# Pixie8888/R3DFSSeg

Hardware: AMD Instinct MI355X
Metric: episodes/sec S3DIS 2-way 5-shot 2048-pt (MPTI+attention, train step: forward+backward+grad all-reduce+Adam) (higher is better)
Workload: dtype f32 (index-free GEMMs -- self-attention, 1x1 convolutions, weight gradients, the EdgeConv backward's edge GEMMs -- as bf16x3 split products on the bf16 MFMA with fp32 accumulate; every index-deciding result: fp32)

## Files before the change

### include/r3d.h

```cpp
#ifndef R3D_H
#define R3D_H
#include <stdint.h>

#ifdef __cplusplus
extern "C" {
#endif

const char* r3d_last_error_string(void);
int r3d_abi_version(void);
int r3d_debug_poison_lds(unsigned pattern, unsigned* sink , void* stream);
int r3d_debug_set_cg_spmv_lds_min_blocks(int min_blocks);
int r3d_set_matrix_arith(int mode);
int r3d_get_matrix_arith(void);
int r3d_debug_set_gemm_bx3(int mask);

int r3d_cm_to_pm(const float* in , int B, int C, int N, float* out , long ld, void* stream);
int r3d_pm_to_cm(const float* in , long ld, int B, int C, int N, float* out , void* stream);
int r3d_pm_to_cm_pitched(const float* in, long ld, int B, int C, int N, float* out , long pitch, void* stream);
long r3d_cm_pitch(int N);
int r3d_copy_cols(const float* src, long ld_src, float* dst, long ld_dst, long M, int C, void* stream);

int r3d_sqnorm(const float* x, long ldx, long rows, int C, float* out, void* stream);
long r3d_knn_norm_ws_words(int B, int N);
int r3d_knn_topk(const float* x, long ldx, const float* x_cm, int B, int N, int C, int k, int mode,
                 const int32_t* n_valid_dev, float* norm_ws, float* cm_ws, int32_t* idx_out, float* score_out,
                 int32_t* status, void* stream);
long r3d_knn_ws_words(int B, int N, int C, int k, int flags);
int r3d_knn_topk_batched(const float* x, long ldx, const float* x_cm, int B, int N, int C, int k, int mode,
                         const int32_t* n_valid_dev, int n_valid_stride, float* ws, long ws_words, int32_t* idx_out,
                         float* score_out, int32_t* status, void* stream);
int r3d_debug_set_knn_bf16_threshold(int on);
int r3d_debug_set_knn_bf16_filter(int on);
int r3d_set_wpack_in_capture(int on);

int r3d_pointwise_conv(const float* X, long ldx, const float* W , long M, int K, int Co,
                       const float* scale, const float* shift, int act, float* Out, long ldo, void* stream);

int r3d_edgeconv_fwd(const float* PQ, const int32_t* idx, const float* W2, const float* s2, const float* t2,
                     float* out, long ldo, int B, int N, int K, int32_t* argmax_out, void* stream);

long r3d_attention_ws_words(int B, int N);
int r3d_attention_fwd(const float* qkv, long ld, int B, int N, float* out, long ldo, float* lse_out, float* ws,
                      void* stream);

int r3d_head_desc_words(void);
int r3d_head_max_k(void);
int r3d_fps_sample_count_table(int k, int n_max, int32_t* out, void* stream);
long r3d_head_proto_ws_words(int n_way, int k_shot, int N);
int r3d_head_proto_ws_offsets(int n_way, int k_shot, int N, long* out6 );
#define R3D_HEAD_FPS_ONE_LAUNCH 1
int r3d_head_prototypes(const int32_t* support_y , const int32_t* shot_keep ,
                        const float* feat , long ldf, const float* featT ,
                        const float* qfeat , long ldq, int n_way, int k_shot, int N, int D,
                        int n_query_pts, int k, float* nodes, long ldn, float* node_labels ,
                        int32_t* desc, int32_t* assign_out , int32_t* cluster_count ,
                        int32_t* ws, long ws_words, int flags, void* stream);

int r3d_head_prototypes_batched(int n_ep, int fps_group, const int32_t* support_y, long sy_stride, const int32_t* shot_keep,
                                long keep_stride, const float* feat, long ldf, long feat_ep_rows, const float* qfeat, long ldq,
                                long qfeat_ep_rows, int n_way, int k_shot, int N, int D, int n_query_pts, int k, float* nodes,
                                long ldn, long nodes_ep_rows, float* node_labels, int32_t* desc, long desc_stride,
                                int32_t* assign_out, long assign_stride, int32_t* cluster_count, long ccount_stride,
                                int32_t* ws, long ws_words, long ws_stride, int flags, void* stream);

long r3d_lp_ws_words(int n_cap, int kp1);
int r3d_lp_ws_offsets(int n_cap, int kp1, long* out6);
int r3d_label_propagate(const float* nodes, long ldn, int D, const int32_t* nbr, int kp1, const float* Y,
                        const int32_t* n_dev, const int32_t* n_proto_dev, int n_cap, float sigma, float alpha,
                        int max_iter, float tol, float* Z, int32_t* ws, long ws_words, int32_t* stats_out, void* stream);

int r3d_label_propagate_batched(int n_ep, const float* nodes, long ldn, int D, const int32_t* nbr, int kp1, const float* Y,
                                const int32_t* n_dev, const int32_t* n_proto_dev, long desc_stride, int n_cap, float sigma,
                                float alpha, int max_iter, float tol, float* Z, int32_t* ws, long ws_words, long ws_stride,
                                int32_t* stats_out, long stats_stride, void* stream);
long r3d_graph_weights_verify_words(int n_cap, int kp1);
int r3d_graph_weights_verify(int n_ep, const float* nodes, long ldn, int D, const int32_t* n_dev, long desc_stride, int n_cap,
                             int kp1, float sigma, int32_t* ws, long ws_words, long ws_stride, float* scratch,
                             int32_t* mismatch_out, void* stream);

int r3d_label_propagate_solve_batched(int n_ep, const float* Y, const int32_t* n_dev, long desc_stride, int n_cap, int kp1,
                                      float alpha, int max_iter, float tol, float* Z, int32_t* ws, long ws_words,
                                      long ws_stride, int32_t* stats_out, long stats_stride, void* stream);

int r3d_graph_set_lp_budget(void* graph, void* graph_exec, int budget, int* n_cg);

int r3d_query_logits_ce(const float* Z, const int32_t* n_proto_dev, int n_q, int N, int n_classes,
                        const int64_t* labels , float* logits ,
                        float* loss_out , int32_t* pred_out , void* stream);

int r3d_query_logits_ce_batched(int n_ep, const float* Z, long z_ep_rows, const int32_t* n_proto_dev, long desc_stride, int n_q,
                                int N, int n_classes, const int64_t* labels, float* logits, float* loss_out, int32_t* pred_out,
                                void* stream);

int r3d_pointwise_conv_acc(const float* X, long ldx, const float* W, long M, int K, int Co, const float* scale,
                           const float* shift, int act, float* Out, long ldo, void* stream);
long r3d_pointwise_conv_stats_ws_words(long M, int Co);
int r3d_pointwise_conv_stats(const float* X, long ldx, const float* W, long M, int K, int Co, float* Out, long ldo,
                             float* sums_out , float* ws, void* stream);
int r3d_pointwise_conv_stats2(const float* X, long ldx, const float* W, long M, int K, int Co, float* Out, long ldo,
                              long M_first, float* sums_a , float* sums_b , float* ws, void* stream);
int r3d_pointwise_conv_stats_seg(const float* X, long ldx, const float* W, long M, int K, int Co, float* Out, long ldo,
                                 long rows_a, long rows_b, float* sums_out, float* ws, void* stream);
int r3d_colreduce(const float* part , int chunks, int C, float* sums_out , void* stream);
int r3d_colreduce_seg(const float* part, int count_a, int count_b, int n_seg, int C, float* sums_out , void* stream);
long r3d_colstats_ws_words(long M, int C);
int r3d_colstats(const float* X, long ldx, const float* DY, long lddy, long M, int C, int mode, const float* scale,
                 const float* shift, const float* mean, const float* invstd, int act, float* sums_out ,
                 float* ws, void* stream);
int r3d_bn_fold(const float* sums, double count, int C, const float* gamma, const float* beta, float eps,
                float momentum, float* running_mean , float* running_var , float* mean, float* invstd,
                float* scale, float* shift, float* rec , const int32_t* rec_index_dev , long rec_stride,
                void* stream);
long r3d_colstats_seg_ws_words(long M, int C, long rows_a, long rows_b);
int r3d_colstats_seg(const float* X, long ldx, const float* DY, long lddy, long M, int C, long rows_a, long rows_b, int mode,
                     const float* scale, const float* shift, const float* mean, const float* invstd, long bn_stride, int act,
                     float* sums_out , float* ws, void* stream);
int r3d_bn_fold_seg(const float* sums , int n_seg, double count_a, double count_b, int C, const float* gamma,
                    const float* beta, float eps, float momentum, float* running_mean , float* running_var ,
                    float* mean, float* invstd, float* scale, float* shift, long bn_stride, float* rec ,
                    const int32_t* rec_index_dev , long rec_stride, void* stream);
int r3d_affine_act_seg(const float* Z, long ldz, long M, int C, long rows_a, long rows_b, const float* scale, const float* shift,
                       long bn_stride, int act, float* Y, long ldy, void* stream);
int r3d_bn_bwd_apply_seg(const float* Z, long ldz, const float* DY, long lddy, long M, int C, long rows_a, long rows_b,
                         const float* scale, const float* shift, const float* mean, const float* invstd, long bn_stride, int act,
                         const float* sums , double count_a, double count_b, float* DZ, long lddz, void* stream);
int r3d_bn_running_update(const float* rec, int n_records, long rec_stride, int C, float momentum,
                          const float* bias , float* running_mean,
                          float* running_var, void* stream);
int r3d_affine_act(const float* Z, long ldz, long M, int C, const float* scale, const float* shift, int act, float* Y,
                   long ldy, void* stream);
int r3d_bn_bwd_apply(const float* Z, long ldz, const float* DY, long lddy, long M, int C, const float* scale,
                     const float* shift, const float* mean, const float* invstd, int act, const float* sums,
                     double count, float* DZ, long lddz, void* stream);
long r3d_gemm_tn_ws_words(long M, int Ca, int Cb);
int r3d_gemm_tn(const float* A, long lda, const float* B, long ldb, long M, int Ca, int Cb, float alpha, float* out,
                int accumulate, float* ws, void* stream);
int r3d_add_cols(const float* src, long ld_src, float* dst, long ld_dst, long M, int C, void* stream);

long r3d_edgeconv_train_ws_words(int B, int N);
int r3d_edge_stats1(const float* PQ, const int32_t* idx, int B, int N, int K, int clouds_a, int clouds_b,
                    float* sums_out , float* esum , float* ws,
                    void* stream);
int r3d_edgeconv_train_fwd_minmax(const float* PQ, const int32_t* idx, const float* s1, const float* t1, long bn_stride,
                                  const float* W2, int B, int N, int K, int clouds_a, int clouds_b, float* zmax, float* zmin,
                                  int32_t* argmax, int32_t* argmin, float* sums_out , float* ws, void* stream);
int r3d_edge_select(float* zmax , const float* zmin, int32_t* argmax ,
                    const int32_t* argmin, const float* s2, const float* t2, long bn_stride, long M, long rows_a, long rows_b,
                    float* out, long ldo, void* stream);
long r3d_edge_reverse_ws_words(int B, int N, int K);
int r3d_edge_reverse(const int32_t* idx, int B, int N, int K, int32_t* rev_ws, long ws_words, void* stream);
int r3d_edgeconv_bwd(const float* PQ, const int32_t* idx, const float* s1, const float* t1, const float* mean1,
                     const float* invstd1, const float* W2, const float* s2, const float* t2, const float* mean2,
                     const float* invstd2, long bn_stride, const float* bn2_sums, const float* dout, long lddo,
                     const int32_t* argmax, const float* zwin , const float* esum , int B, int N, int K,
                     int clouds_a, int clouds_b, float* DY1 , float* BE ,
                     const int32_t* rev_ws , float* dW2, float* bn1_sums, float* dPQ,
                     float* ws, void* stream);

int r3d_attention_fwd_train(const float* qkv, long ld, int B, int N, float* out, long ldo, float* lse_out, float p_drop,
                            unsigned seed, const unsigned* seed_dev, float* ws , void* stream);
int r3d_attention_bwd(const float* qkv, long ld, int B, int N, const float* O, long ldo, const float* dO, long lddo,
                      const float* lse, float p_drop, unsigned seed, const unsigned* seed_dev, float q_scale, float* dqkv,
                      long ldd, float* ws , void* stream);
int r3d_attention_bwd_ws(const float* qkv, long ld, int B, int N, const float* O, long ldo, const float* dO, long lddo,
                         const float* lse, float p_drop, unsigned seed, const unsigned* seed_dev, float q_scale,
                         float* dqkv, long ldd, float* ws, int ws_holds_packed_qkv, void* stream);

long r3d_attention_ws_words_ep(int B, int N, int seed_group);
int r3d_attention_fwd_train_ep(const float* qkv, long ld, int B, int N, float* out, long ldo, float* lse_out, float p_drop,
                               unsigned seed, const unsigned* seed_dev, int seed_group, float* ws, void* stream);
int r3d_attention_bwd_ep(const float* qkv, long ld, int B, int N, const float* O, long ldo, const float* dO, long lddo,
                         const float* lse, float p_drop, unsigned seed, const unsigned* seed_dev, int seed_group, float q_scale,
                         float* dqkv, long ldd, float* ws, int ws_holds_packed_qkv, void* stream);

long r3d_attention_ws_words_ep_d(int B, int N, int seed_group, int D);
int r3d_attention_fwd_train_ep_d(const float* qkv, long ld, int B, int N, float* out, long ldo, float* lse_out, float p_drop,
                                 unsigned seed, const unsigned* seed_dev, int seed_group, int D, float* ws, void* stream);
int r3d_attention_bwd_ep_d(const float* qkv, long ld, int B, int N, const float* O, long ldo, const float* dO, long lddo,
                           const float* lse, float p_drop, unsigned seed, const unsigned* seed_dev, int seed_group, int D,
                           float q_scale, float* dqkv, long ldd, float* ws, int ws_holds_packed_qkv, void* stream);

int r3d_ce_grad(const float* Z, const int32_t* n_proto_dev, int n_cap, int n_query_pts, int n_classes,
                const int64_t* labels, const float* gscale_dev, float* G, void* stream);
int r3d_label_propagate_bwd(const float* nodes, long ldn, int D, int kp1, const float* Z, const float* G,
                            const int32_t* n_dev, int n_cap, float sigma, float alpha, int max_iter, float tol, float* lam,
                            float* dnodes, long ldd, int32_t* ws, long ws_words, int32_t* stats_out, void* stream);
int r3d_head_prototypes_bwd(const float* dnodes, long ldd, int n_way, int k_shot, int N, int D, int n_query_pts,
                            const int32_t* desc, const int32_t* assign, const int32_t* cluster_count, const int32_t* ws,
                            float* dsfeat, long lds_, float* dqfeat, long ldq, void* stream);

int r3d_ce_grad_batched(int n_ep, const float* Z, const int32_t* n_proto_dev, long desc_stride, int n_cap, int n_query_pts,
                        int n_classes, const int64_t* labels, const float* gscale_dev, float* G, void* stream);
int r3d_label_propagate_bwd_batched(int n_ep, const float* nodes, long ldn, int D, int kp1, const float* Z, const float* G,
                                    const int32_t* n_dev, long desc_stride, int n_cap, float sigma, float alpha, int max_iter,
                                    float tol, float* lam, float* dnodes, long ldd, int32_t* ws, long ws_words, long ws_stride,
                                    int32_t* stats_out, long stats_stride, void* stream);
int r3d_head_prototypes_bwd_batched(int n_ep, const float* dnodes, long ldd, long nodes_ep_rows, int n_way, int k_shot, int N,
                                    int D, int n_query_pts, const int32_t* desc, long desc_stride, const int32_t* assign,
                                    long assign_stride, const int32_t* cluster_count, long ccount_stride, const int32_t* ws,
                                    long ws_stride, float* dsfeat, long lds_, long dsfeat_ep_rows, float* dqfeat, long ldq,
                                    long dqfeat_ep_rows, void* stream);

long r3d_contrast_ws_words(int n_way, int k_shot, int N);
int r3d_contrast_fwd(const float* feat, long ldf, int D, const int32_t* support_y, const int32_t* support_flag, int n_way,
                     int k_shot, int N, const float* W, const float* bias, float temp, float* loss_out, float* ws,
                     long ws_words, void* stream);
int r3d_contrast_bwd(int D, int n_way, int k_shot, int N, const float* gscale_dev, float* dfeat, long ldd, float* dW,
                     float* db, float* ws, void* stream);
int r3d_contrast_fwd_batched(int n_ep, const float* feat, long ldf, long feat_ep_rows, int D, const int32_t* support_y,
                             const int32_t* support_flag, int n_way, int k_shot, int N, const float* W, const float* bias,
                             float temp, float* loss_out, float* ws, long ws_words, long ws_stride, void* stream);
int r3d_contrast_bwd_batched(int n_ep, int D, int n_way, int k_shot, int N, const float* gscale_dev, float* dfeat, long ldd,
                             long dfeat_ep_rows, float* dW, float* db, float* ws, long ws_stride, void* stream);
int r3d_train_metrics_batched(int n_ep, const int32_t* pred, const int64_t* query_y, const int64_t* gt_query_y, int n_query_pts,
                              const float* Z, long z_ep_rows, const int32_t* desc, long desc_stride, const int32_t* proto_ws,
                              long pws_stride, const int32_t* assign, long assign_stride, const int32_t* gt_support_y, int n_way,
                              int k_shot, int N, float* out4 , void* stream);
int r3d_train_metrics(const int32_t* pred, const int64_t* query_y, const int64_t* gt_query_y, int n_query_pts, const float* Z,
                      const int32_t* desc, const int32_t* proto_ws, const int32_t* assign, const int32_t* gt_support_y,
                      int n_way, int k_shot, int N, float* out4, void* stream);

long r3d_clean_ws_words(int n_way, int k_shot);
int r3d_clean_shot_detect(const float* feat , long ldf, int D, const float* support_x ,
                          int Cin, const int32_t* support_y, int n_way, int k_shot, int N, int32_t* shot_keep,
                          float* dbg_cos_sum , int32_t* ws, void* stream);

int r3d_clean_shot_detect_batched(int n_ep, const float* feat, long ldf, long feat_ep_rows, int D, const float* support_x,
                                  int Cin, const int32_t* support_y, int n_way, int k_shot, int N, int32_t* shot_keep,
                                  float* dbg_cos_sum, int32_t* ws, long ws_stride, void* stream);

int r3d_protonet_head(const float* sfeat, long ldf, const float* qfeat, long ldq, int D, const int32_t* support_y,
                      int n_way, int k_shot, int N, int n_query_pts, int method, float scaler, float* Z, float* ws,
                      void* stream);

long r3d_protonet_head_ws_words(int n_ep, int n_way, int k_shot);
int r3d_protonet_head_batched(int n_ep, const float* sfeat, long ldf, const float* qfeat, long ldq, long feat_ep_rows, int D,
                              const int32_t* support_y, int n_way, int k_shot, int N, int n_query_pts, int method,
                              float scaler, float* Z, float* ws, long ws_words, void* stream);
int r3d_count_correct_batched(int n_ep, const int32_t* pred, const int64_t* labels, long n_pts, int32_t* correct,
                              void* stream);

long r3d_protonet_head_train_ws_words(int n_ep, int n_way, int k_shot, int N, int n_query_pts, int D);
int r3d_protonet_head_train_fwd(int n_ep, const float* sfeat, long ldf, const float* qfeat, long ldq, long feat_ep_rows, int D,
                                const int32_t* support_y, int n_way, int k_shot, int N, int n_query_pts, int method,
                                float scaler, float* Z, float* ws, long ws_words, void* stream);
int r3d_protonet_head_bwd(int n_ep, const float* qfeat, long ldq, long feat_ep_rows, int D, const int32_t* support_y, int n_way,
                          int k_shot, int N, int n_query_pts, int method, float scaler, const float* dZ, float* dsfeat,
                          long ldds, float* dqfeat, long lddq, long dfeat_ep_rows, float* ws, long ws_words, void* stream);

int r3d_miou_accumulate(const int32_t* pred, const int64_t* gt, long n, const int32_t* lut, int n_lut, int n_classes,
                        uint64_t* hist, void* stream);

#ifdef __cplusplus
}
#endif
#endif
```

### r3dfsseg_amd/_lib.py

```python
import ctypes
import os
import re

_HERE = os.path.dirname(os.path.abspath(__file__))
LIB_PATH = os.environ.get("R3D_LIB") or os.path.join(_HERE, "libr3d_hip.so")
HEADER_PATH = os.path.join(os.path.dirname(_HERE), "include", "r3d.h")

c_f = ctypes.c_void_p
c_i = ctypes.c_int
c_l = ctypes.c_long
c_fl = ctypes.c_float
c_d = ctypes.c_double
c_u = ctypes.c_uint

_SIGS = {
    "r3d_last_error_string": (ctypes.c_char_p, []),
    "r3d_abi_version": (c_i, []),
    "r3d_cm_to_pm": (c_i, [c_f, c_i, c_i, c_i, c_f, c_l, c_f]),
    "r3d_pm_to_cm": (c_i, [c_f, c_l, c_i, c_i, c_i, c_f, c_f]),
    "r3d_pm_to_cm_pitched": (c_i, [c_f, c_l, c_i, c_i, c_i, c_f, c_l, c_f]),
    "r3d_cm_pitch": (c_l, [c_i]),
    "r3d_copy_cols": (c_i, [c_f, c_l, c_f, c_l, c_l, c_i, c_f]),
    "r3d_sqnorm": (c_i, [c_f, c_l, c_l, c_i, c_f, c_f]),
    "r3d_knn_topk": (c_i, [c_f, c_l, c_f, c_i, c_i, c_i, c_i, c_i, c_f, c_f, c_f, c_f, c_f, c_f, c_f]),
    "r3d_pointwise_conv": (c_i, [c_f, c_l, c_f, c_l, c_i, c_i, c_f, c_f, c_i, c_f, c_l, c_f]),
    "r3d_edgeconv_fwd": (c_i, [c_f, c_f, c_f, c_f, c_f, c_f, c_l, c_i, c_i, c_i, c_f, c_f]),
    "r3d_attention_ws_words": (c_l, [c_i, c_i]),
    "r3d_knn_norm_ws_words": (c_l, [c_i, c_i]),
    "r3d_attention_fwd": (c_i, [c_f, c_l, c_i, c_i, c_f, c_l, c_f, c_f, c_f]),
    "r3d_head_desc_words": (c_i, []),
    "r3d_debug_poison_lds": (c_i, [c_u, c_f, c_f]),
    "r3d_debug_set_cg_spmv_lds_min_blocks": (c_i, [c_i]),
    "r3d_debug_set_gemm_bx3": (c_i, [c_i]),
    "r3d_set_matrix_arith": (c_i, [c_i]),
    "r3d_get_matrix_arith": (c_i, []),
    "r3d_head_max_k": (c_i, []),
    "r3d_fps_sample_count_table": (c_i, [c_i, c_i, c_f, c_f]),
    "r3d_head_proto_ws_words": (c_l, [c_i, c_i, c_i]),
    "r3d_head_proto_ws_offsets": (c_i, [c_i, c_i, c_i, ctypes.POINTER(c_l)]),
    "r3d_head_prototypes": (c_i, [c_f, c_f, c_f, c_l, c_f, c_f, c_l, c_i, c_i, c_i, c_i, c_i, c_i, c_f, c_l,
                                  c_f, c_f, c_f, c_f, c_f, c_l, c_i, c_f]),
    "r3d_lp_ws_words": (c_l, [c_i, c_i]),
    "r3d_lp_ws_offsets": (c_i, [c_i, c_i, ctypes.POINTER(c_l)]),
    "r3d_label_propagate": (c_i, [c_f, c_l, c_i, c_f, c_i, c_f, c_f, c_f, c_i, c_fl, c_fl, c_i, c_fl, c_f, c_f,
                                  c_l, c_f, c_f]),
    "r3d_graph_set_lp_budget": (c_i, [c_f, c_f, c_i, ctypes.POINTER(c_i)]),
    "r3d_pointwise_conv_acc": (c_i, [c_f, c_l, c_f, c_l, c_i, c_i, c_f, c_f, c_i, c_f, c_l, c_f]),
    "r3d_edgeconv_train_fwd_minmax": (c_i, [c_f, c_f, c_f, c_f, c_l, c_f, c_i, c_i, c_i, c_i, c_i, c_f, c_f, c_f, c_f, c_f, c_f, c_f]),
    "r3d_edge_select": (c_i, [c_f, c_f, c_f, c_f, c_f, c_f, c_l, c_l, c_l, c_l, c_f, c_l, c_f]),
    "r3d_pointwise_conv_stats_ws_words": (c_l, [c_l, c_i]),
    "r3d_pointwise_conv_stats": (c_i, [c_f, c_l, c_f, c_l, c_i, c_i, c_f, c_l, c_f, c_f, c_f]),
    "r3d_pointwise_conv_stats2": (c_i, [c_f, c_l, c_f, c_l, c_i, c_i, c_f, c_l, c_l, c_f, c_f, c_f, c_f]),
    "r3d_colreduce": (c_i, [c_f, c_i, c_i, c_f, c_f]),
    "r3d_colstats_ws_words": (c_l, [c_l, c_i]),
    "r3d_colstats": (c_i, [c_f, c_l, c_f, c_l, c_l, c_i, c_i, c_f, c_f, c_f, c_f, c_i, c_f, c_f, c_f]),
    "r3d_bn_fold": (c_i, [c_f, c_d, c_i, c_f, c_f, c_fl, c_fl, c_f, c_f, c_f, c_f, c_f, c_f, c_f, c_f, c_l, c_f]),
    "r3d_bn_running_update": (c_i, [c_f, c_i, c_l, c_i, c_fl, c_f, c_f, c_f, c_f]),
    "r3d_affine_act": (c_i, [c_f, c_l, c_l, c_i, c_f, c_f, c_i, c_f, c_l, c_f]),
    "r3d_bn_bwd_apply": (c_i, [c_f, c_l, c_f, c_l, c_l, c_i, c_f, c_f, c_f, c_f, c_i, c_f, c_d, c_f, c_l, c_f]),
    "r3d_gemm_tn_ws_words": (c_l, [c_l, c_i, c_i]),
    "r3d_gemm_tn": (c_i, [c_f, c_l, c_f, c_l, c_l, c_i, c_i, c_fl, c_f, c_i, c_f, c_f]),
    "r3d_add_cols": (c_i, [c_f, c_l, c_f, c_l, c_l, c_i, c_f]),
    "r3d_edgeconv_train_ws_words": (c_l, [c_i, c_i]),
    "r3d_edge_stats1": (c_i, [c_f, c_f, c_i, c_i, c_i, c_i, c_i, c_f, c_f, c_f, c_f]),
    "r3d_edge_reverse_ws_words": (c_l, [c_i, c_i, c_i]),
    "r3d_edge_reverse": (c_i, [c_f, c_i, c_i, c_i, c_f, c_l, c_f]),
    "r3d_edgeconv_bwd": (c_i, [c_f] * 11 + [c_l, c_f, c_f, c_l, c_f, c_f, c_f, c_i, c_i, c_i, c_i, c_i, c_f, c_f, c_f, c_f, c_f, c_f, c_f, c_f]),
    "r3d_attention_fwd_train": (c_i, [c_f, c_l, c_i, c_i, c_f, c_l, c_f, c_fl, c_u, c_f, c_f, c_f]),
    "r3d_attention_bwd": (c_i, [c_f, c_l, c_i, c_i, c_f, c_l, c_f, c_l, c_f, c_fl, c_u, c_f, c_fl, c_f, c_l, c_f, c_f]),
    "r3d_attention_bwd_ws": (c_i, [c_f, c_l, c_i, c_i, c_f, c_l, c_f, c_l, c_f, c_fl, c_u, c_f, c_fl, c_f, c_l, c_f, c_i, c_f]),
    "r3d_ce_grad": (c_i, [c_f, c_f, c_i, c_i, c_i, c_f, c_f, c_f, c_f]),
    "r3d_label_propagate_bwd": (c_i, [c_f, c_l, c_i, c_i, c_f, c_f, c_f, c_i, c_fl, c_fl, c_i, c_fl, c_f, c_f, c_l, c_f, c_l, c_f, c_f]),
    "r3d_head_prototypes_bwd": (c_i, [c_f, c_l, c_i, c_i, c_i, c_i, c_i, c_f, c_f, c_f, c_f, c_f, c_l, c_f, c_l, c_f]),
    "r3d_contrast_ws_words": (c_l, [c_i, c_i, c_i]),
    "r3d_contrast_fwd": (c_i, [c_f, c_l, c_i, c_f, c_f, c_i, c_i, c_i, c_f, c_f, c_fl, c_f, c_f, c_l, c_f]),
    "r3d_contrast_bwd": (c_i, [c_i, c_i, c_i, c_i, c_f, c_f, c_l, c_f, c_f, c_f, c_f]),
    "r3d_train_metrics": (c_i, [c_f, c_f, c_f, c_i, c_f, c_f, c_f, c_f, c_f, c_i, c_i, c_i, c_f, c_f]),
    "r3d_clean_ws_words": (c_l, [c_i, c_i]),
    "r3d_clean_shot_detect": (c_i, [c_f, c_l, c_i, c_f, c_i, c_f, c_i, c_i, c_i, c_f, c_f, c_f, c_f]),
    "r3d_protonet_head": (c_i, [c_f, c_l, c_f, c_l, c_i, c_f, c_i, c_i, c_i, c_i, c_i, c_fl, c_f, c_f, c_f]),
    "r3d_protonet_head_ws_words": (c_l, [c_i, c_i, c_i]),
    "r3d_protonet_head_batched": (c_i, [c_i, c_f, c_l, c_f, c_l, c_l, c_i, c_f, c_i, c_i, c_i, c_i, c_i, c_fl, c_f, c_f, c_l, c_f]),
    "r3d_count_correct_batched": (c_i, [c_i, c_f, c_f, c_l, c_f, c_f]),
    "r3d_protonet_head_train_ws_words": (c_l, [c_i, c_i, c_i, c_i, c_i, c_i]),
    "r3d_protonet_head_train_fwd": (c_i, [c_i, c_f, c_l, c_f, c_l, c_l, c_i, c_f, c_i, c_i, c_i, c_i, c_i, c_fl, c_f, c_f, c_l, c_f]),
    "r3d_protonet_head_bwd": (c_i, [c_i, c_f, c_l, c_l, c_i, c_f, c_i, c_i, c_i, c_i, c_i, c_fl, c_f, c_f, c_l, c_f, c_l, c_l, c_f,
                                    c_l, c_f]),
    "r3d_miou_accumulate": (c_i, [c_f, c_f, c_l, c_f, c_i, c_i, c_f, c_f]),
    "r3d_query_logits_ce": (c_i, [c_f, c_f, c_i, c_i, c_i, c_f, c_f, c_f, c_f, c_f]),
    "r3d_knn_topk_batched": (c_i, [c_f, c_l, c_f, c_i, c_i, c_i, c_i, c_i, c_f, c_i, c_f, c_l, c_f, c_f, c_f, c_f]),
    "r3d_knn_ws_words": (c_l, [c_i, c_i, c_i, c_i, c_i]),
    "r3d_debug_set_knn_bf16_threshold": (c_i, [c_i]),
    "r3d_debug_set_knn_bf16_filter": (c_i, [c_i]),
    "r3d_set_wpack_in_capture": (c_i, [c_i]),
    "r3d_pointwise_conv_stats_seg": (c_i, [c_f, c_l, c_f, c_l, c_i, c_i, c_f, c_l, c_l, c_l, c_f, c_f, c_f]),
    "r3d_colreduce_seg": (c_i, [c_f, c_i, c_i, c_i, c_i, c_f, c_f]),
    "r3d_colstats_seg_ws_words": (c_l, [c_l, c_i, c_l, c_l]),
    "r3d_colstats_seg": (c_i, [c_f, c_l, c_f, c_l, c_l, c_i, c_l, c_l, c_i, c_f, c_f, c_f, c_f, c_l, c_i, c_f, c_f, c_f]),
    "r3d_bn_fold_seg": (c_i, [c_f, c_i, c_d, c_d, c_i, c_f, c_f, c_fl, c_fl, c_f, c_f, c_f, c_f, c_f, c_f, c_l, c_f, c_f, c_l, c_f]),
    "r3d_affine_act_seg": (c_i, [c_f, c_l, c_l, c_i, c_l, c_l, c_f, c_f, c_l, c_i, c_f, c_l, c_f]),
    "r3d_bn_bwd_apply_seg": (c_i, [c_f, c_l, c_f, c_l, c_l, c_i, c_l, c_l, c_f, c_f, c_f, c_f, c_l, c_i, c_f, c_d, c_d, c_f, c_l, c_f]),
    "r3d_attention_ws_words_ep": (c_l, [c_i, c_i, c_i]),
    "r3d_attention_fwd_train_ep": (c_i, [c_f, c_l, c_i, c_i, c_f, c_l, c_f, c_fl, c_u, c_f, c_i, c_f, c_f]),
    "r3d_attention_bwd_ep": (c_i, [c_f, c_l, c_i, c_i, c_f, c_l, c_f, c_l, c_f, c_fl, c_u, c_f, c_i, c_fl, c_f, c_l, c_f, c_i, c_f]),
    "r3d_attention_ws_words_ep_d": (c_l, [c_i, c_i, c_i, c_i]),
    "r3d_attention_fwd_train_ep_d": (c_i, [c_f, c_l, c_i, c_i, c_f, c_l, c_f, c_fl, c_u, c_f, c_i, c_i, c_f, c_f]),
    "r3d_attention_bwd_ep_d": (c_i, [c_f, c_l, c_i, c_i, c_f, c_l, c_f, c_l, c_f, c_fl, c_u, c_f, c_i, c_i, c_fl, c_f, c_l, c_f, c_i,
                                     c_f]),
    "r3d_head_prototypes_batched": (c_i, [c_i, c_i, c_f, c_l, c_f, c_l, c_f, c_l, c_l, c_f, c_l, c_l, c_i, c_i, c_i, c_i, c_i, c_i,
                                          c_f, c_l, c_l, c_f, c_f, c_l, c_f, c_l, c_f, c_l, c_f, c_l, c_l, c_i, c_f]),
    "r3d_head_prototypes_bwd_batched": (c_i, [c_i, c_f, c_l, c_l, c_i, c_i, c_i, c_i, c_i, c_f, c_l, c_f, c_l, c_f, c_l, c_f, c_l,
                                              c_f, c_l, c_l, c_f, c_l, c_l, c_f]),
    "r3d_graph_weights_verify_words": (c_l, [c_i, c_i]),
    "r3d_graph_weights_verify": (c_i, [c_i, c_f, c_l, c_i, c_f, c_l, c_i, c_i, c_fl, c_f, c_l, c_l, c_f, c_f, c_f]),
    "r3d_label_propagate_solve_batched": (c_i, [c_i, c_f, c_f, c_l, c_i, c_i, c_fl, c_i, c_fl, c_f, c_f, c_l, c_l, c_f, c_l, c_f]),
    "r3d_label_propagate_batched": (c_i, [c_i, c_f, c_l, c_i, c_f, c_i, c_f, c_f, c_f, c_l, c_i, c_fl, c_fl, c_i, c_fl, c_f, c_f,
                                          c_l, c_l, c_f, c_l, c_f]),
    "r3d_label_propagate_bwd_batched": (c_i, [c_i, c_f, c_l, c_i, c_i, c_f, c_f, c_f, c_l, c_i, c_fl, c_fl, c_i, c_fl, c_f, c_f,
                                              c_l, c_f, c_l, c_l, c_f, c_l, c_f]),
    "r3d_ce_grad_batched": (c_i, [c_i, c_f, c_f, c_l, c_i, c_i, c_i, c_f, c_f, c_f, c_f]),
    "r3d_query_logits_ce_batched": (c_i, [c_i, c_f, c_l, c_f, c_l, c_i, c_i, c_i, c_f, c_f, c_f, c_f, c_f]),
    "r3d_contrast_fwd_batched": (c_i, [c_i, c_f, c_l, c_l, c_i, c_f, c_f, c_i, c_i, c_i, c_f, c_f, c_fl, c_f, c_f, c_l, c_l, c_f]),
    "r3d_contrast_bwd_batched": (c_i, [c_i, c_i, c_i, c_i, c_i, c_f, c_f, c_l, c_l, c_f, c_f, c_f, c_l, c_f]),
    "r3d_train_metrics_batched": (c_i, [c_i, c_f, c_f, c_f, c_i, c_f, c_l, c_f, c_l, c_f, c_l, c_f, c_l, c_f, c_i, c_i, c_i, c_f, c_f]),
    "r3d_clean_shot_detect_batched": (c_i, [c_i, c_f, c_l, c_l, c_i, c_f, c_i, c_f, c_i, c_i, c_i, c_f, c_f, c_f, c_l, c_f]),
}

_lib = None


def header_symbols():
    txt = open(HEADER_PATH).read()
    txt = re.sub(r"/\*.*?\*/", "", txt, flags=re.S)
    return sorted(set(re.findall(r"\b(r3d_[a-z0-9_]+)\s*\(", txt)))


ABI_VERSION = 5


def load():
    global _lib
    if _lib is not None:
        return _lib
    import torch
    if not os.path.exists(LIB_PATH):
        raise RuntimeError(
            "r3dfsseg_amd: %s not found -- build it with `python -m r3dfsseg_amd.build` "
            "(hipcc, gfx950). There is no CPU fallback." % LIB_PATH)
    cdll = ctypes.CDLL(LIB_PATH)
    lib = _Bound()
    lib._cdll = cdll
    for name, (res, args) in _SIGS.items():
        try:
            fn = getattr(cdll, name)
        except AttributeError:
            raise RuntimeError("r3dfsseg_amd: symbol %s missing from %s" % (name, LIB_PATH))
        fn.restype = res
        fn.argtypes = args
        setattr(lib, name, fn)
    if lib.r3d_abi_version() != ABI_VERSION:
        raise RuntimeError("r3dfsseg_amd: %s has C ABI version %d, this package binds version %d -- rebuild it "
                           "(`python -m r3dfsseg_amd.build --force`)" % (LIB_PATH, lib.r3d_abi_version(), ABI_VERSION))
    _lib = lib
    mode = os.environ.get("R3D_MATRIX_ARITH")
    if mode is not None:
        if mode not in ("fp32", "bf16x3"):
            raise RuntimeError("R3D_MATRIX_ARITH=%r: expected fp32 or bf16x3" % mode)
        check(lib.r3d_set_matrix_arith(1 if mode == "bf16x3" else 0))
    mask = os.environ.get("R3D_GEMM_BX3")
    if mask is not None:
        check(lib.r3d_debug_set_gemm_bx3(int(mask)))
    return lib


class _Bound:
    """The bound entry points as plain attributes (one per symbol of include/r3d.h)."""


_call_log = None


def record_calls(on):
    lib = load()
    for name in _SIGS:
        raw = getattr(lib._cdll, name)
        if not on:
            setattr(lib, name, raw)
            continue

        def wrapper(*args, _raw=raw):
            rc = _raw(*args)
            if _call_log is not None:
                _call_log.append((_raw, args))
            return rc
        setattr(lib, name, wrapper)


def check(rc):
    if rc != 0:
        raise RuntimeError("r3d: " + load().r3d_last_error_string().decode())
```

### r3dfsseg_amd/csrc/common.h

```cpp
#pragma once
#include <hip/hip_runtime.h>
#include <stdint.h>
#include <stdio.h>

#define R3D_OK 0
#define R3D_ERR_ARG 1
#define R3D_ERR_LAUNCH 2
#define R3D_ERR_UNSUPPORTED 3

void r3d_set_error(const char* fmt, ...);

#define R3D_REQUIRE(cond, ...)          \
  do {                                  \
    if (!(cond)) {                      \
      r3d_set_error(__VA_ARGS__);       \
      return R3D_ERR_ARG;               \
    }                                   \
  } while (0)

#define R3D_LAUNCH_CHECK(name)                                              \
  do {                                                                      \
    hipError_t e_ = hipGetLastError();                                      \
    if (e_ != hipSuccess) {                                                 \
      r3d_set_error("%s: launch failed: %s", name, hipGetErrorString(e_));  \
      return R3D_ERR_LAUNCH;                                                \
    }                                                                       \
  } while (0)

typedef float f32x16 __attribute__((ext_vector_type(16)));
typedef float f32x4 __attribute__((ext_vector_type(4)));

#define R3D_WAVE 64

static __device__ __forceinline__ int r3d_lane() { return threadIdx.x & 63; }

static __device__ __forceinline__ int r3d_acc_row(int r, int lane) {
  return (r & 3) + 8 * (r >> 2) + 4 * (lane >> 5);
}

static __device__ __forceinline__ float r3d_readlane_f(float v, int src) {
  return __int_as_float(__builtin_amdgcn_readlane(__float_as_int(v), src));
}

static __device__ __forceinline__ float r3d_sum8_dpp(float v) {
  int x = __float_as_int(v);
  v += __int_as_float(__builtin_amdgcn_mov_dpp(x, 0xB1, 0xF, 0xF, true));
  x = __float_as_int(v);
  v += __int_as_float(__builtin_amdgcn_mov_dpp(x, 0x4E, 0xF, 0xF, true));
  x = __float_as_int(v);
  v += __int_as_float(__builtin_amdgcn_mov_dpp(x, 0x141, 0xF, 0xF, true));
  return v;
}

static __device__ __forceinline__ int r3d_wave_incl_scan(int v) {
  v += __builtin_amdgcn_update_dpp(0, v, 0x111, 0xF, 0xF, true);
  v += __builtin_amdgcn_update_dpp(0, v, 0x112, 0xF, 0xF, true);
  v += __builtin_amdgcn_update_dpp(0, v, 0x114, 0xF, 0xF, true);
  v += __builtin_amdgcn_update_dpp(0, v, 0x118, 0xF, 0xF, true);
  v += __builtin_amdgcn_update_dpp(0, v, 0x142, 0xA, 0xF, false);
  v += __builtin_amdgcn_update_dpp(0, v, 0x143, 0xC, 0xF, false);
  return v;
}

static __device__ __forceinline__ float r3d_wave_sum(float v) {
#pragma unroll
  for (int o = 32; o > 0; o >>= 1) v += __shfl_xor(v, o);
  return v;
}
static __device__ __forceinline__ float r3d_wave_max(float v) {
#pragma unroll
  for (int o = 32; o > 0; o >>= 1) v = fmaxf(v, __shfl_xor(v, o));
  return v;
}

static __device__ __forceinline__ float r3d_keep(float v, bool keep) {
  return __uint_as_float(__float_as_uint(v) & (keep ? 0xffffffffu : 0u));
}

typedef unsigned r3d_u32x4 __attribute__((ext_vector_type(4)));
typedef __bf16 r3d_bf16x8 __attribute__((ext_vector_type(8)));
extern int g_r3d_matrix_arith;

static __device__ __forceinline__ void r3d_bx3_split2(float x0, float x1, unsigned& h, unsigned& m, unsigned& l) {
  const unsigned u0 = __float_as_uint(x0), u1 = __float_as_uint(x1);
  const float r0 = x0 - __uint_as_float(u0 & 0xffff0000u), r1 = x1 - __uint_as_float(u1 & 0xffff0000u);
  const unsigned v0 = __float_as_uint(r0), v1 = __float_as_uint(r1);
  const float t0 = r0 - __uint_as_float(v0 & 0xffff0000u), t1 = r1 - __uint_as_float(v1 & 0xffff0000u);
  h = __builtin_amdgcn_perm(u1, u0, 0x07060302u);
  m = __builtin_amdgcn_perm(v1, v0, 0x07060302u);
  l = __builtin_amdgcn_perm(__float_as_uint(t1), __float_as_uint(t0), 0x07060302u);
}
struct r3d_bx3 {
  r3d_u32x4 h, m, l;
};
static __device__ __forceinline__ r3d_bx3 r3d_bx3_split8(const float* x) {
  r3d_bx3 f;
#pragma unroll
  for (int i = 0; i < 4; ++i) {
    unsigned h, m, l;
    r3d_bx3_split2(x[2 * i], x[2 * i + 1], h, m, l);
    f.h[i] = h; f.m[i] = m; f.l[i] = l;
  }
  return f;
}
static __device__ __forceinline__ f32x16 r3d_mfma_bf16(r3d_u32x4 a, r3d_u32x4 b, f32x16 c) {
#if defined(ATT_ABL) && (ATT_ABL & 4)
  c[0] += __uint_as_float(a[0] ^ b[1]);
  return c;
#endif
  return __builtin_amdgcn_mfma_f32_32x32x16_bf16(__builtin_bit_cast(r3d_bf16x8, a), __builtin_bit_cast(r3d_bf16x8, b), c, 0,
                                                 0, 0);
}
static __device__ __forceinline__ f32x16 r3d_bx3_mma(const r3d_bx3& a, const r3d_bx3& b, f32x16 c) {
  c = r3d_mfma_bf16(a.l, b.h, c);
  c = r3d_mfma_bf16(a.h, b.l, c);
  c = r3d_mfma_bf16(a.m, b.m, c);
  c = r3d_mfma_bf16(a.m, b.h, c);
  c = r3d_mfma_bf16(a.h, b.m, c);
  c = r3d_mfma_bf16(a.h, b.h, c);
  return c;
}

extern int g_r3d_gemm_bx3;

static inline int r3d_cdiv(long a, long b) { return (int)((a + b - 1) / b); }

static __device__ __forceinline__ int r3d_xcd_swizzle(int id, int n) {
  const int q = n >> 3, r = n & 7, x = id & 7;
  return (x < r ? x * (q + 1) : r * (q + 1) + (x - r) * q) + (id >> 3);
}

struct r3d_segmap {
  long a, b;
  __host__ __device__ bool odd(int seg) const { return b > 0 && (seg & 1); }
  __host__ __device__ long seg_rows(int seg) const { return odd(seg) ? b : a; }
  __host__ __device__ long seg_row0(int seg) const {
    return b > 0 ? (long)(seg >> 1) * (a + b) + (odd(seg) ? a : 0) : (long)seg * a;
  }
  __host__ __device__ int seg_of_row(long r) const {
    if (b == 0) return (int)(r / a);
    const long p = r / (a + b);
    return (int)(2 * p + ((r - p * (a + b)) >= a ? 1 : 0));
  }
  __device__ int seg_of_row32(int r) const {
    const int A = (int)a, B = (int)b;
    if (B == 0) return r / A;
    const int p = r / (A + B);
    return 2 * p + ((r - p * (A + B)) >= A ? 1 : 0);
  }
  __host__ __device__ int n_seg(long total) const { return (int)(b > 0 ? 2 * (total / (a + b)) : total / a); }
  __host__ __device__ bool covers(long total) const {
    return a > 0 && b >= 0 && total > 0 && total < 0x7fffffffL && total % (a + b) == 0;
  }
};

static __global__ void r3d_fill_words_kernel(unsigned* __restrict__ p, unsigned v, long n) {
  for (long i = (long)blockIdx.x * blockDim.x + threadIdx.x; i < n; i += (long)gridDim.x * blockDim.x) p[i] = v;
}
static __global__ void r3d_copy_words_kernel(unsigned* __restrict__ dst, const unsigned* __restrict__ src, long n) {
  for (long i = (long)blockIdx.x * blockDim.x + threadIdx.x; i < n; i += (long)gridDim.x * blockDim.x) dst[i] = src[i];
}
static __global__ void r3d_fill_words_ep_kernel(unsigned* __restrict__ p, unsigned v, long n, long stride_words) {
  p += (long)blockIdx.y * stride_words;
  for (long i = (long)blockIdx.x * blockDim.x + threadIdx.x; i < n; i += (long)gridDim.x * blockDim.x) p[i] = v;
}
static inline void r3d_fill_words_ep(void* p, unsigned v, long n_words, int n_ep, long stride_words, hipStream_t st) {
  const int g = (int)(n_words < 256L * 2048 ? (n_words + 255) / 256 : 2048);
  hipLaunchKernelGGL(r3d_fill_words_ep_kernel, dim3(g > 0 ? g : 1, n_ep), dim3(256), 0, st, (unsigned*)p, v, n_words, stride_words);
}
static inline void r3d_zero_words(void* p, long n_words, hipStream_t st) {
  const int g = (int)(n_words < 256L * 2048 ? (n_words + 255) / 256 : 2048);
  hipLaunchKernelGGL(r3d_fill_words_kernel, dim3(g > 0 ? g : 1), dim3(256), 0, st, (unsigned*)p, 0u, n_words);
}
static inline void r3d_copy_words(void* dst, const void* src, long n_words, hipStream_t st) {
  const int g = (int)(n_words < 256L * 2048 ? (n_words + 255) / 256 : 2048);
  hipLaunchKernelGGL(r3d_copy_words_kernel, dim3(g > 0 ? g : 1), dim3(256), 0, st, (unsigned*)dst, (const unsigned*)src,
                     n_words);
}
```

### r3dfsseg_amd/csrc/gemm.hip

```cpp
#include "common.h"

#define G_BM 64
#define G_BN 64
#define G_BK 32
#define G_LD (G_BK + 1)

enum { R3D_ACT_NONE = 0, R3D_ACT_RELU = 1, R3D_ACT_LRELU02 = 2 };

__global__ __launch_bounds__(256) void r3d_pointwise_gemm_kernel(
    const float* __restrict__ X, long ldx, const float* __restrict__ W, int M, int K, int Co,
    const float* __restrict__ scale, const float* __restrict__ shift, int act,
    float* __restrict__ Out, long ldo, int accumulate, float* __restrict__ stats_part ) {
  __shared__ float Xs[2][G_BM * G_LD];
  __shared__ float Ws[2][G_BN * G_LD];
  const int tid = threadIdx.x, lane = tid & 63, w = tid >> 6;
  const int wm = w >> 1, wn = w & 1;
  const int tiles_n = (Co + G_BN - 1) / G_BN;
  const int tile = r3d_xcd_swizzle((int)blockIdx.x, (int)gridDim.x);
  const int tile_m = tile / tiles_n;
  const long m0 = (long)tile_m * G_BM;
  const int n0 = (tile - tile_m * tiles_n) * G_BN;
  f32x16 acc;
#pragma unroll
  for (int r = 0; r < 16; ++r) acc[r] = 0.f;
  const int srow = tid >> 5, scol = tid & 31;
  float xv[G_BM / 8], wv[G_BN / 8];
  const float* xrow[G_BM / 8];
  const float* wrow[G_BN / 8];
#pragma unroll
  for (int p = 0; p < G_BM / 8; ++p) {
    xrow[p] = X + min(m0 + srow + 8 * p, (long)M - 1) * ldx;
    wrow[p] = W + (long)min(n0 + srow + 8 * p, Co - 1) * K;
  }
  auto load_step = [&](int k0) {
    const int gk = k0 + scol;
    if (k0 + G_BK <= K) {
#pragma unroll
      for (int p = 0; p < G_BM / 8; ++p) {
        xv[p] = xrow[p][gk];
        wv[p] = wrow[p][gk];
      }
    } else {
      const int gkc = min(gk, K - 1);
#pragma unroll
      for (int p = 0; p < G_BM / 8; ++p) {
        xv[p] = r3d_keep(xrow[p][gkc], gk < K);
        wv[p] = r3d_keep(wrow[p][gkc], gk < K);
      }
    }
  };
  auto store_step = [&](int buf) {
#pragma unroll
    for (int p = 0; p < G_BM / 8; ++p) {
      const int row = srow + 8 * p;
      Xs[buf][row * G_LD + scol] = xv[p];
      Ws[buf][row * G_LD + scol] = wv[p];
    }
  };
  load_step(0);
  store_step(0);
  __syncthreads();
  int buf = 0;
  for (int k0 = 0; k0 < K; k0 += G_BK, buf ^= 1) {
    const bool more = k0 + G_BK < K;
    if (more) load_step(k0 + G_BK);
    __builtin_amdgcn_sched_barrier(0);
    const float* ap = Xs[buf] + (32 * wm + (lane & 31)) * G_LD + (lane >> 5);
    const float* bp = Ws[buf] + (32 * wn + (lane & 31)) * G_LD + (lane >> 5);
#pragma unroll
    for (int kk = 0; kk < G_BK; kk += 2)
      acc = __builtin_amdgcn_mfma_f32_32x32x2f32(ap[kk], bp[kk], acc, 0, 0, 0);
    if (more) store_step(buf ^ 1);
    __syncthreads();
  }
  const int j = n0 + 32 * wn + (lane & 31);
  const bool jok = j < Co;
  const float sc = (scale && jok) ? scale[j] : 1.f;
  const float sh = (shift && jok) ? shift[j] : 0.f;
  float s1 = 0.f, s2 = 0.f;
#pragma unroll
  for (int r = 0; r < 16; ++r) {
    const long m = m0 + 32 * wm + r3d_acc_row(r, lane);
    if (m >= M || !jok) continue;
    float v = sc * acc[r] + sh;
    if (act == R3D_ACT_RELU) v = fmaxf(v, 0.f);
    else if (act == R3D_ACT_LRELU02) v = v > 0.f ? v : 0.2f * v;
    Out[m * ldo + j] = accumulate ? Out[m * ldo + j] + v : v;
    s1 += v;
    s2 += v * v;
  }
  if (stats_part) {
    s1 += __shfl_xor(s1, 32);
    s2 += __shfl_xor(s2, 32);
    __syncthreads();
    float* red = Xs[0];
    if (lane < 32) {
      red[((wm * 2 + wn) * 2 + 0) * 32 + lane] = s1;
      red[((wm * 2 + wn) * 2 + 1) * 32 + lane] = s2;
    }
    __syncthreads();
    if (tid < 128) {
      const int which = tid >> 6, cc = tid & 63, wn2 = cc >> 5, l2 = cc & 31;
      const int jj = n0 + cc;
      if (jj < Co)
        stats_part[((long)tile_m * 2 + which) * Co + jj] =
            red[((0 * 2 + wn2) * 2 + which) * 32 + l2] + red[((1 * 2 + wn2) * 2 + which) * 32 + l2];
    }
  }
}

static int pointwise_launch(const float* X, long ldx, const float* W, long M, int K, int Co, const float* scale,
                            const float* shift, int act, float* Out, long ldo, int accumulate, float* stats_part,
                            void* stream);
bool r3d_pointwise_bx3_ok(const float* X, long ldx, const float* W, long M, int K, int Co);
int r3d_pointwise_bx3_launch(const float* X, long ldx, const float* W, long M, int K, int Co, const float* scale,
                             const float* shift, int act, float* Out, long ldo, int accumulate, float* stats_part,
                             hipStream_t st);

extern "C" int r3d_pointwise_conv(const float* X, long ldx, const float* W, long M, int K, int Co,
                                  const float* scale, const float* shift, int act, float* Out,
                                  long ldo, void* stream) {
  return pointwise_launch(X, ldx, W, M, K, Co, scale, shift, act, Out, ldo, 0, nullptr, stream);
}

extern "C" int r3d_colreduce(const float* part, int chunks, int C, float* sums_out, void* stream);
extern "C" long r3d_pointwise_conv_stats_ws_words(long M, int Co) { return (long)r3d_cdiv(M, G_BM) * 2 * Co; }
extern "C" int r3d_pointwise_conv_stats(const float* X, long ldx, const float* W, long M, int K, int Co, float* Out,
                                        long ldo, float* sums_out, float* ws, void* stream) {
  R3D_REQUIRE(sums_out && ws, "r3d_pointwise_conv_stats: null pointer");
  int rc = pointwise_launch(X, ldx, W, M, K, Co, nullptr, nullptr, R3D_ACT_NONE, Out, ldo, 0, ws, stream);
  if (rc) return rc;
  return r3d_colreduce(ws, r3d_cdiv(M, G_BM), Co, sums_out, stream);
}

extern "C" int r3d_pointwise_conv_stats2(const float* X, long ldx, const float* W, long M, int K, int Co, float* Out,
                                         long ldo, long M_first, float* sums_a, float* sums_b, float* ws, void* stream) {
  R3D_REQUIRE(sums_a && sums_b && ws, "r3d_pointwise_conv_stats2: null pointer");
  R3D_REQUIRE(M_first > 0 && M_first < M && M_first % G_BM == 0,
              "r3d_pointwise_conv_stats2: first segment of %ld rows (of %ld) must be a positive multiple of %d", M_first, M,
              G_BM);
  int rc = pointwise_launch(X, ldx, W, M, K, Co, nullptr, nullptr, R3D_ACT_NONE, Out, ldo, 0, ws, stream);
  if (rc) return rc;
  const int tiles_a = (int)(M_first / G_BM);
  rc = r3d_colreduce(ws, tiles_a, Co, sums_a, stream);
  if (rc) return rc;
  return r3d_colreduce(ws + (long)tiles_a * 2 * Co, r3d_cdiv(M, G_BM) - tiles_a, Co, sums_b, stream);
}

extern "C" int r3d_colreduce_seg(const float* part, int count_a, int count_b, int n_seg, int C, float* sums_out, void* stream);
extern "C" int r3d_pointwise_conv_stats_seg(const float* X, long ldx, const float* W, long M, int K, int Co, float* Out,
                                            long ldo, long rows_a, long rows_b, float* sums_out, float* ws, void* stream) {
  R3D_REQUIRE(sums_out && ws, "r3d_pointwise_conv_stats_seg: null pointer");
  const r3d_segmap sm{rows_a, rows_b};
  R3D_REQUIRE(sm.covers(M) && (sm.n_seg(M) == 1 || (rows_a % G_BM == 0 && rows_b % G_BM == 0)),
              "r3d_pointwise_conv_stats_seg: %ld rows in segments of %ld + %ld rows (multiples of %d needed)", M, rows_a, rows_b,
              G_BM);
  int rc = pointwise_launch(X, ldx, W, M, K, Co, nullptr, nullptr, R3D_ACT_NONE, Out, ldo, 0, ws, stream);
  if (rc) return rc;
  return r3d_colreduce_seg(ws, r3d_cdiv(rows_a, G_BM), r3d_cdiv(rows_b, G_BM), sm.n_seg(M), Co, sums_out, stream);
}

extern "C" int r3d_pointwise_conv_acc(const float* X, long ldx, const float* W, long M, int K, int Co,
                                      const float* scale, const float* shift, int act, float* Out,
                                      long ldo, void* stream) {
  return pointwise_launch(X, ldx, W, M, K, Co, scale, shift, act, Out, ldo, 1, nullptr, stream);
}

static int pointwise_launch(const float* X, long ldx, const float* W, long M, int K, int Co, const float* scale,
                            const float* shift, int act, float* Out, long ldo, int accumulate, float* stats_part,
                            void* stream) {
  R3D_REQUIRE(X && W && Out, "r3d_pointwise_conv: null pointer");
  R3D_REQUIRE(M > 0 && K > 0 && Co > 0 && ldx >= K && ldo >= Co,
              "r3d_pointwise_conv: bad shape M=%ld K=%d Co=%d ldx=%ld ldo=%ld", M, K, Co, ldx, ldo);
  R3D_REQUIRE(act >= 0 && act <= 2, "r3d_pointwise_conv: unknown activation %d", act);
  if (r3d_pointwise_bx3_ok(X, ldx, W, M, K, Co)) {
    const int rc = r3d_pointwise_bx3_launch(X, ldx, W, M, K, Co, scale, shift, act, Out, ldo, accumulate, stats_part,
                                            (hipStream_t)stream);
    if (rc > 0) return rc;
    if (rc == 0) {
      R3D_LAUNCH_CHECK("r3d_pointwise_conv");
      return R3D_OK;
    }
  }
  const long tiles = (long)r3d_cdiv(M, G_BM) * r3d_cdiv(Co, G_BN);
  R3D_REQUIRE(tiles < 0x7fffffffL, "r3d_pointwise_conv: too many tiles");
  dim3 grid((unsigned)tiles);
  hipLaunchKernelGGL(r3d_pointwise_gemm_kernel, grid, dim3(256), 0, (hipStream_t)stream, X, ldx, W,
                     (int)M, K, Co, scale, shift, act, Out, ldo, accumulate, stats_part);
  R3D_LAUNCH_CHECK("r3d_pointwise_conv");
  return R3D_OK;
}

__global__ void r3d_cm_to_pm_kernel(const float* __restrict__ in, int C, int N, float* __restrict__ out,
                                    long ld) {
  __shared__ float t[32][33];
  const int b = blockIdx.z;
  const int n0 = blockIdx.x * 32, c0 = blockIdx.y * 32;
  const int tx = threadIdx.x & 31, ty = threadIdx.x >> 5;
  for (int i = ty; i < 32; i += 8) {
    const int c = c0 + i, n = n0 + tx;
    t[i][tx] = (c < C && n < N) ? in[((long)b * C + c) * N + n] : 0.f;
  }
  __syncthreads();
  for (int i = ty; i < 32; i += 8) {
    const int n = n0 + i, c = c0 + tx;
    if (n < N && c < C) out[((long)b * N + n) * ld + c] = t[tx][i];
  }
}

__global__ void r3d_pm_to_cm_kernel(const float* __restrict__ in, long ld, int C, int N,
                                    float* __restrict__ out, long pitch) {
  __shared__ float t[32][33];
  const int b = blockIdx.z;
  const int n0 = blockIdx.x * 32, c0 = blockIdx.y * 32;
  const int tx = threadIdx.x & 31, ty = threadIdx.x >> 5;
  for (int i = ty; i < 32; i += 8) {
    const int n = n0 + i, c = c0 + tx;
    t[i][tx] = (c < C && n < N) ? in[((long)b * N + n) * ld + c] : 0.f;
  }
  __syncthreads();
  for (int i = ty; i < 32; i += 8) {
    const int c = c0 + i, n = n0 + tx;
    if (c < C && n < N) out[((long)b * C + c) * pitch + n] = t[tx][i];
  }
}

extern "C" int r3d_cm_to_pm(const float* in, int B, int C, int N, float* out, long ld, void* stream) {
  R3D_REQUIRE(in && out && B > 0 && C > 0 && N > 0 && ld >= C, "r3d_cm_to_pm: bad arguments");
  dim3 grid(r3d_cdiv(N, 32), r3d_cdiv(C, 32), B);
  hipLaunchKernelGGL(r3d_cm_to_pm_kernel, grid, dim3(256), 0, (hipStream_t)stream, in, C, N, out, ld);
  R3D_LAUNCH_CHECK("r3d_cm_to_pm");
  return R3D_OK;
}

extern "C" int r3d_pm_to_cm(const float* in, long ld, int B, int C, int N, float* out, void* stream) {
  R3D_REQUIRE(in && out && B > 0 && C > 0 && N > 0 && ld >= C, "r3d_pm_to_cm: bad arguments");
  dim3 grid(r3d_cdiv(N, 32), r3d_cdiv(C, 32), B);
  hipLaunchKernelGGL(r3d_pm_to_cm_kernel, grid, dim3(256), 0, (hipStream_t)stream, in, ld, C, N, out, (long)N);
  R3D_LAUNCH_CHECK("r3d_pm_to_cm");
  return R3D_OK;
}

extern "C" int r3d_pm_to_cm_pitched(const float* in, long ld, int B, int C, int N, float* out, long pitch,
                                    void* stream) {
  R3D_REQUIRE(in && out && B > 0 && C > 0 && N > 0 && ld >= C && pitch >= N, "r3d_pm_to_cm_pitched: bad arguments");
  dim3 grid(r3d_cdiv(N, 32), r3d_cdiv(C, 32), B);
  hipLaunchKernelGGL(r3d_pm_to_cm_kernel, grid, dim3(256), 0, (hipStream_t)stream, in, ld, C, N, out, pitch);
  R3D_LAUNCH_CHECK("r3d_pm_to_cm_pitched");
  return R3D_OK;
}

__global__ __launch_bounds__(256) void r3d_copy_cols_kernel(const float* __restrict__ src, long lds_, float* __restrict__ dst,
                                                            long ldd, long M, int C) {
  const int lane = threadIdx.x & 63;
  const long r0 = ((long)blockIdx.x * 4 + (threadIdx.x >> 6)) * 4;
  for (int c = lane; c < C; c += 64) {
    float a[4];
#pragma unroll
    for (int u = 0; u < 4; ++u) a[u] = src[(r0 + u < M ? r0 + u : M - 1) * lds_ + c];
#pragma unroll
    for (int u = 0; u < 4; ++u)
      if (r0 + u < M) dst[(r0 + u) * ldd + c] = a[u];
  }
}

extern "C" int r3d_copy_cols(const float* src, long ld_src, float* dst, long ld_dst, long M, int C,
                             void* stream) {
  R3D_REQUIRE(src && dst && M > 0 && C > 0, "r3d_copy_cols: bad arguments");
  hipLaunchKernelGGL(r3d_copy_cols_kernel, dim3(r3d_cdiv(M, 16)), dim3(256), 0,
                     (hipStream_t)stream, src, ld_src, dst, ld_dst, M, C);
  R3D_LAUNCH_CHECK("r3d_copy_cols");
  return R3D_OK;
}
```

### r3dfsseg_amd/csrc/gemm_bx3.hip

```cpp
#if defined(GB_ABL) && (GB_ABL & 4)
#define ATT_ABL 4
#endif
#include "common.h"
#include <mutex>
#include <type_traits>
#include <vector>
#ifndef GB_ABL
#define GB_ABL 0
#endif

#define GB_RS 40

enum { GB_ACT_NONE = 0, GB_ACT_RELU = 1, GB_ACT_LRELU02 = 2 };

static __device__ __forceinline__ void gb_store_chunk(unsigned short* __restrict__ planes, int rows, int row, int kc,
                                                      const float (&v)[8]) {
#if GB_ABL & 2
  r3d_bx3 f;
  for (int i = 0; i < 4; ++i) { f.h[i] = __float_as_uint(v[i]); f.m[i] = __float_as_uint(v[4 + i]); f.l[i] = f.h[i] ^ f.m[i]; }
#else
  const r3d_bx3 f = r3d_bx3_split8(v);
#endif
  unsigned short* p = planes + row * GB_RS + 8 * kc;
  *reinterpret_cast<r3d_u32x4*>(p) = f.h;
  *reinterpret_cast<r3d_u32x4*>(p + rows * GB_RS) = f.m;
  *reinterpret_cast<r3d_u32x4*>(p + 2 * rows * GB_RS) = f.l;
}
static __device__ __forceinline__ r3d_bx3 gb_load_frag(const unsigned short* __restrict__ planes, int rows, int row, int ks,
                                                       int g) {
  const unsigned short* p = planes + row * GB_RS + 16 * ks + 8 * g;
  r3d_bx3 f;
  f.h = *reinterpret_cast<const r3d_u32x4*>(p);
  f.m = *reinterpret_cast<const r3d_u32x4*>(p + rows * GB_RS);
  f.l = *reinterpret_cast<const r3d_u32x4*>(p + 2 * rows * GB_RS);
  return f;
}

static __device__ __forceinline__ void gb_wave_mma(const unsigned short* __restrict__ As, int a_rows, int a_row0,
                                                   const unsigned short* __restrict__ Bs, int b_rows, int b_row0, int lane,
                                                   f32x16 (&acc)[2][2]) {
  const int j = lane & 31, g = lane >> 5;
#pragma unroll
  for (int ks = 0; ks < 2; ++ks) {
    r3d_bx3 a[2], b[2];
#pragma unroll
    for (int t = 0; t < 2; ++t) {
      a[t] = gb_load_frag(As, a_rows, a_row0 + 32 * t + j, ks, g);
      b[t] = gb_load_frag(Bs, b_rows, b_row0 + 32 * t + j, ks, g);
    }
#pragma unroll
    for (int tm = 0; tm < 2; ++tm)
#pragma unroll
      for (int tn = 0; tn < 2; ++tn) acc[tm][tn] = r3d_bx3_mma(a[tm], b[tn], acc[tm][tn]);
  }
}

template <int NT>
__global__ __launch_bounds__(256) __attribute__((amdgpu_waves_per_eu(2))) void r3d_pointwise_gemm_bx3_kernel(
    const float* __restrict__ X, long ldx, const float* __restrict__ W, int M, int K, int Co,
    const float* __restrict__ scale, const float* __restrict__ shift, int act, float* __restrict__ Out, long ldo,
    int accumulate, float* __restrict__ stats_part) {
  constexpr int BM = 256, BN = 32 * NT;
  __shared__ __attribute__((aligned(16))) unsigned short Bs[2][2][NT][3][64 * 8];
  const int tid = threadIdx.x, lane = tid & 63, w = tid >> 6;
  const int j = lane & 31, g = lane >> 5;
  const int tiles_n = (Co + BN - 1) / BN;
  const int tile = r3d_xcd_swizzle((int)blockIdx.x, (int)gridDim.x);
  const int tile_m = tile / tiles_n;
  const long mw = (long)tile_m * BM + 64 * w;
  const int n0 = (tile - tile_m * tiles_n) * BN;
  const long m0 = (long)tile_m * BM;
  const long arows = min((long)BM, (long)M - m0);
  const __amdgpu_buffer_rsrc_t ra = __builtin_amdgcn_make_buffer_rsrc(
      (void*)(X + m0 * ldx), 0, (int)(((arows - 1) * ldx + K) * 4), 0x00020000);
  const int wrows = min(BN, Co - n0);
  const __amdgpu_buffer_rsrc_t rw =
      __builtin_amdgcn_make_buffer_rsrc((void*)(W + (long)n0 * K), 0, wrows * K * 4, 0x00020000);
  int oa[2];
#pragma unroll
  for (int tm = 0; tm < 2; ++tm) oa[tm] = (int)(((64 * w + 32 * tm + j) * ldx + 16 * g) * 4);
  constexpr int WU = BN / 64;
  const int wc = tid & 3;
  int ow[WU];
  unsigned short* wdst[WU];
#pragma unroll
  for (int u = 0; u < WU; ++u) {
    const int wrow = (tid >> 2) + 64 * u;
    ow[u] = (wrow * K + 8 * wc) * 4;
    wdst[u] = &Bs[0][wc & 1][wrow >> 5][0][((wrow & 31) + 32 * (wc >> 1)) * 8];
  }
  constexpr int BUF = 2 * NT * 3 * 64 * 8;
  float araw[2][2][8], wraw[WU][8];
  auto ld8 = [&](const __amdgpu_buffer_rsrc_t r, int voff, int soff, float (&d)[8]) {
    const r3d_u32x4 a = __builtin_amdgcn_raw_buffer_load_b128(r, voff, soff, 0);
    const r3d_u32x4 b = __builtin_amdgcn_raw_buffer_load_b128(r, voff + 16, soff, 0);
#pragma unroll
    for (int i = 0; i < 4; ++i) { d[i] = __uint_as_float(a[i]); d[4 + i] = __uint_as_float(b[i]); }
  };
  auto aload = [&](int k, int s) {
#pragma unroll
    for (int tm = 0; tm < 2; ++tm) ld8(ra, oa[tm] + 32 * s, k * 4, araw[s][tm]);
  };
  auto asplit = [&](int s, r3d_bx3 (&fa)[2]) {
#pragma unroll
    for (int tm = 0; tm < 2; ++tm) {
#if GB_ABL & 2
      for (int i = 0; i < 4; ++i) { fa[tm].h[i] = __float_as_uint(araw[s][tm][i]); fa[tm].m[i] = __float_as_uint(araw[s][tm][4 + i]); fa[tm].l[i] = fa[tm].h[i] ^ fa[tm].m[i]; }
#else
      fa[tm] = r3d_bx3_split8(araw[s][tm]);
#endif
    }
  };
  auto wload = [&](int k) {
#pragma unroll
    for (int u = 0; u < WU; ++u) ld8(rw, ow[u], k * 4, wraw[u]);
  };
  auto wstore = [&](int buf) {
#pragma unroll
    for (int u = 0; u < WU; ++u) {
#if GB_ABL & 2
      r3d_bx3 f;
      for (int i = 0; i < 4; ++i) { f.h[i] = __float_as_uint(wraw[u][i]); f.m[i] = __float_as_uint(wraw[u][4 + i]); f.l[i] = f.h[i] ^ f.m[i]; }
#else
      const r3d_bx3 f = r3d_bx3_split8(wraw[u]);
#endif
      unsigned short* d = wdst[u] + buf * BUF;
      *reinterpret_cast<r3d_u32x4*>(d) = f.h;
      *reinterpret_cast<r3d_u32x4*>(d + 64 * 8) = f.m;
      *reinterpret_cast<r3d_u32x4*>(d + 2 * 64 * 8) = f.l;
    }
  };
  auto mma = [&](int buf, int s, const r3d_bx3 (&fa)[2], f32x16 (&acc)[2][NT]) {
#pragma unroll
    for (int tn = 0; tn < NT; ++tn) {
      r3d_bx3 fb;
      const unsigned short* bsrc = &Bs[buf][s][tn][0][lane * 8];
      fb.h = *reinterpret_cast<const r3d_u32x4*>(bsrc);
      fb.m = *reinterpret_cast<const r3d_u32x4*>(bsrc + 64 * 8);
      fb.l = *reinterpret_cast<const r3d_u32x4*>(bsrc + 2 * 64 * 8);
#pragma unroll
      for (int tm = 0; tm < 2; ++tm) acc[tm][tn] = r3d_bx3_mma(fa[tm], fb, acc[tm][tn]);
    }
  };
  f32x16 acc[2][NT];
#pragma unroll
  for (int a = 0; a < 2; ++a)
#pragma unroll
    for (int b = 0; b < NT; ++b)
#pragma unroll
      for (int r = 0; r < 16; ++r) acc[a][b][r] = 0.f;
  wload(0);
  aload(0, 0);
  aload(0, 1);
  wstore(0);
  __syncthreads();
  for (int k = 0, it = 0; k < K; k += 32, ++it) {
    const int cur = it & 1;
    const int kn = (GB_ABL & 8) ? 0 : min(k + 32, K - 32);
    r3d_bx3 fa0[2], fa1[2];
    asplit(0, fa0);
    wload(kn);
    aload(kn, 0);
    __builtin_amdgcn_sched_barrier(0);
    mma(cur, 0, fa0, acc);
    asplit(1, fa1);
    aload(kn, 1);
    __builtin_amdgcn_sched_barrier(0);
    mma(cur, 1, fa1, acc);
    wstore(cur ^ 1);
    __syncthreads();
  }
  constexpr int ER = BN + 4;
  float* es = reinterpret_cast<float*>(&Bs[0][0][0][0][0]) + w * 8 * ER;
  constexpr int LPR = BN / 4;
  constexpr int RPI = 64 / LPR;
  const int erow = lane / LPR, ecol = 4 * (lane % LPR);
  const bool cok = n0 + ecol < Co;
  float sc[NT], sh[NT], s1[2][NT], s2[2][NT];
#pragma unroll
  for (int tn = 0; tn < NT; ++tn) {
    const int jc = n0 + 32 * tn + j;
    sc[tn] = (scale && jc < Co) ? scale[jc] : 1.f;
    sh[tn] = (shift && jc < Co) ? shift[jc] : 0.f;
    s1[0][tn] = s2[0][tn] = s1[1][tn] = s2[1][tn] = 0.f;
  }
#pragma unroll
  for (int tm = 0; tm < 2; ++tm) {
#pragma unroll
    for (int q = 0; q < 4; ++q) {
      const long mrow0 = mw + 32 * tm + 8 * q;
#pragma unroll
      for (int tn = 0; tn < NT; ++tn) {
#pragma unroll
        for (int i = 0; i < 4; ++i) {
          float v = sc[tn] * acc[tm][tn][4 * q + i] + sh[tn];
          if (act == GB_ACT_RELU) v = fmaxf(v, 0.f);
          else if (act == GB_ACT_LRELU02) v = fmaxf(v, 0.2f * v);
          es[(4 * g + i) * ER + 32 * tn + j] = v;
          {
            const float u = r3d_keep(v, mrow0 + 4 * g + i < M);
            s1[tm][tn] += u;
            s2[tm][tn] += u * u;
          }
        }
      }
#pragma unroll
      for (int i = 0; i < 8 / RPI; ++i) {
        const int row = erow + RPI * i;
        const long m = mrow0 + row;
        const float4 v = *reinterpret_cast<const float4*>(&es[row * ER + ecol]);
        if (m < M && cok && !(GB_ABL & 1)) {
          float4* dst = reinterpret_cast<float4*>(&Out[m * ldo + n0 + ecol]);
          if (accumulate) {
            const float4 o = *dst;
            *dst = make_float4(o.x + v.x, o.y + v.y, o.z + v.z, o.w + v.w);
          } else {
            *dst = v;
          }
        }
      }
    }
  }
  if (stats_part && mw < M) {
    const long t64 = mw >> 6;
#pragma unroll
    for (int tn = 0; tn < NT; ++tn) {
      const int jc = n0 + 32 * tn + j;
      const float a1 = (s1[0][tn] + __shfl_xor(s1[0][tn], 32)) + (s1[1][tn] + __shfl_xor(s1[1][tn], 32));
      const float a2 = (s2[0][tn] + __shfl_xor(s2[0][tn], 32)) + (s2[1][tn] + __shfl_xor(s2[1][tn], 32));
      if (lane < 32 && jc < Co) {
        stats_part[(t64 * 2 + 0) * Co + jc] = a1;
        stats_part[(t64 * 2 + 1) * Co + jc] = a2;
      }
    }
  }
}

__global__ void r3d_w_pack_bx3_kernel(const float* __restrict__ W, int K, int Co, int BN ,
                                      unsigned short* __restrict__ out) {
  const int NT = BN / 32, ksteps = K / 32;
  const long i = (long)blockIdx.x * blockDim.x + threadIdx.x;
  const int Cop = (Co + BN - 1) / BN * BN;
  if (i >= (long)Cop * (K / 8)) return;
  const int n = (int)(i / (K / 8)), c8 = (int)(i - (long)n * (K / 8));
  const int ks = c8 >> 2, c = c8 & 3;
  float v[8];
#pragma unroll
  for (int u = 0; u < 8; ++u) v[u] = r3d_keep(W[(long)min(n, Co - 1) * K + 32 * ks + 8 * c + u], n < Co);
  const r3d_bx3 f = r3d_bx3_split8(v);
  const int ct = n / BN, tn = (n % BN) >> 5, lane = (n & 31) + 32 * (c >> 1), sx = c & 1;
  unsigned short* d = out + ((((long)(ct * ksteps + ks) * 2 + sx) * NT + tn) * 3) * 512 + lane * 8;
  *reinterpret_cast<r3d_u32x4*>(d) = f.h;
  *reinterpret_cast<r3d_u32x4*>(d + 512) = f.m;
  *reinterpret_cast<r3d_u32x4*>(d + 1024) = f.l;
}

template <int NT>
__global__ __launch_bounds__(256) __attribute__((amdgpu_waves_per_eu(3))) void r3d_pointwise_gemm_bx3p_kernel(
    const float* __restrict__ X, long ldx, const unsigned short* __restrict__ Wp, int M, int K, int Co,
    const float* __restrict__ scale, const float* __restrict__ shift, int act, float* __restrict__ Out, long ldo,
    int accumulate, float* __restrict__ stats_part) {
  constexpr int BM = 128, BN = 32 * NT;
  constexpr int TILE = 2 * NT * 3 * 512;
  constexpr int CPT = TILE / 8 / 256;
  __shared__ __attribute__((aligned(16))) unsigned short Bs[2][TILE];
  __shared__ float st_s[2][2][BN];
  const int tid = threadIdx.x, lane = tid & 63, w = tid >> 6;
  const int j = lane & 31, g = lane >> 5;
  const int tiles_n = (Co + BN - 1) / BN, ksteps = K / 32;
  const int tile = r3d_xcd_swizzle((int)blockIdx.x, (int)gridDim.x);
  const int tile_m = tile / tiles_n, ct = tile - tile_m * tiles_n;
  const long m0 = (long)tile_m * BM, mw = m0 + 32 * w;
  const int n0 = ct * BN;
  const long arows = min((long)BM, (long)M - m0);
  const __amdgpu_buffer_rsrc_t ra = __builtin_amdgcn_make_buffer_rsrc(
      (void*)(X + m0 * ldx), 0, (int)(((arows - 1) * ldx + K) * 4), 0x00020000);
  const __amdgpu_buffer_rsrc_t rw = __builtin_amdgcn_make_buffer_rsrc(
      (void*)(Wp + (long)ct * ksteps * TILE), 0, ksteps * TILE * 2, 0x00020000);
  const int oa = (int)(((32 * w + j) * ldx + 16 * g) * 4);
  float araw[16];
  auto aload = [&](int k) {
#pragma unroll
    for (int q = 0; q < 4; ++q) {
      const r3d_u32x4 v = __builtin_amdgcn_raw_buffer_load_b128(ra, oa + 16 * q, k * 4, 0);
#pragma unroll
      for (int i = 0; i < 4; ++i) araw[4 * q + i] = __uint_as_float(v[i]);
    }
  };
  constexpr int H0 = (CPT + 1) / 2;
  r3d_u32x4 wst[CPT];
  auto wload = [&](int ks, int half) {
#pragma unroll
    for (int u = 0; u < CPT; ++u)
      if ((u < H0) == (half == 0)) wst[u] = __builtin_amdgcn_raw_buffer_load_b128(rw, (tid + 256 * u) * 16, ks * TILE * 2, 0);
  };
  auto wstore = [&](int buf, int half) {
#pragma unroll
    for (int u = 0; u < CPT; ++u)
      if ((u < H0) == (half == 0)) *reinterpret_cast<r3d_u32x4*>(&Bs[buf][(tid + 256 * u) * 8]) = wst[u];
  };
  f32x16 acc[NT];
#pragma unroll
  for (int b = 0; b < NT; ++b)
#pragma unroll
    for (int r = 0; r < 16; ++r) acc[b][r] = 0.f;
  auto mma = [&](int buf, int sx, const r3d_bx3& fa) {
#pragma unroll
    for (int tn = 0; tn < NT; ++tn) {
      r3d_bx3 fb;
      const unsigned short* bsrc = &Bs[buf][((sx * NT + tn) * 3) * 512 + lane * 8];
      fb.h = *reinterpret_cast<const r3d_u32x4*>(bsrc);
      fb.m = *reinterpret_cast<const r3d_u32x4*>(bsrc + 512);
      fb.l = *reinterpret_cast<const r3d_u32x4*>(bsrc + 1024);
      acc[tn] = r3d_bx3_mma(fa, fb, acc[tn]);
    }
  };
  wload(0, 0);
  wload(0, 1);
  aload(0);
  wstore(0, 0);
  wstore(0, 1);
  __syncthreads();
  for (int ks = 0; ks < ksteps; ++ks) {
    const int cur = ks & 1, kn = min(ks + 1, ksteps - 1);
    const r3d_bx3 fa0 = r3d_bx3_split8(&araw[0]), fa1 = r3d_bx3_split8(&araw[8]);
    aload(32 * kn);
    wload(kn, 0);
    __builtin_amdgcn_sched_barrier(0);
    mma(cur, 0, fa0);
    wstore(cur ^ 1, 0);
    wload(kn, 1);
    __builtin_amdgcn_sched_barrier(0);
    mma(cur, 1, fa1);
    wstore(cur ^ 1, 1);
    __syncthreads();
  }
  constexpr int ER = BN + 4;
  float* es = reinterpret_cast<float*>(&Bs[0][0]) + w * 8 * ER;
  constexpr int LPR = BN / 4, RPI = 64 / LPR;
  const int erow = lane / LPR, ecol = 4 * (lane % LPR);
  float s1[NT], s2[NT];
#pragma unroll
  for (int tn = 0; tn < NT; ++tn) s1[tn] = s2[tn] = 0.f;
  auto epilogue = [&](auto PLAIN_, auto STATS_, auto FULL_) {
    constexpr bool PLAIN = decltype(PLAIN_)::value, STATS = decltype(STATS_)::value, FULL = decltype(FULL_)::value;
    const bool cok = FULL || n0 + ecol < Co;
    float sc[NT], sh[NT];
    if (!PLAIN) {
#pragma unroll
      for (int tn = 0; tn < NT; ++tn) {
        const int jc = n0 + 32 * tn + j;
        sc[tn] = (scale && (FULL || jc < Co)) ? scale[jc] : 1.f;
        sh[tn] = (shift && (FULL || jc < Co)) ? shift[jc] : 0.f;
      }
    }
#pragma unroll
    for (int q = 0; q < 4; ++q) {
      const int rleft = FULL ? 8 : (int)min((long)8, (long)M - (mw + 8 * q));
#pragma unroll
      for (int tn = 0; tn < NT; ++tn) {
#pragma unroll
        for (int i = 0; i < 4; ++i) {
          float v = acc[tn][4 * q + i];
          if (!PLAIN) {
            v = sc[tn] * v + sh[tn];
            if (act == GB_ACT_RELU) v = fmaxf(v, 0.f);
            else if (act == GB_ACT_LRELU02) v = fmaxf(v, 0.2f * v);
          }
          es[(4 * g + i) * ER + 32 * tn + j] = v;
          if (STATS) {
            const float u = FULL ? v : r3d_keep(v, 4 * g + i < rleft);
            s1[tn] += u;
            s2[tn] += u * u;
          }
        }
      }
#pragma unroll
      for (int i = 0; i < 8 / RPI; ++i) {
        const int row = erow + RPI * i;
        const float4 v = *reinterpret_cast<const float4*>(&es[row * ER + ecol]);
        if ((FULL || row < rleft) && cok) {
          float4* dst = reinterpret_cast<float4*>(&Out[(mw + 8 * q + row) * ldo + n0 + ecol]);
          if (accumulate) {
            const float4 o = *dst;
            *dst = make_float4(o.x + v.x, o.y + v.y, o.z + v.z, o.w + v.w);
          } else {
            *dst = v;
          }
        }
      }
    }
  };
  {
    using T_ = std::integral_constant<bool, true>;
    using F_ = std::integral_constant<bool, false>;
    const bool plain = !scale && !shift && act == GB_ACT_NONE, full = mw + 32 <= M && n0 + BN <= Co, stats = stats_part != nullptr;
    if (plain) {
      if (stats) { if (full) epilogue(T_{}, T_{}, T_{}); else epilogue(T_{}, T_{}, F_{}); }
      else       { if (full) epilogue(T_{}, F_{}, T_{}); else epilogue(T_{}, F_{}, F_{}); }
    } else {
      if (stats) epilogue(F_{}, T_{}, F_{});
      else       { if (full) epilogue(F_{}, F_{}, T_{}); else epilogue(F_{}, F_{}, F_{}); }
    }
  }
  if (stats_part) {
#pragma unroll
    for (int tn = 0; tn < NT; ++tn) {
      const float a1 = s1[tn] + __shfl_xor(s1[tn], 32), a2 = s2[tn] + __shfl_xor(s2[tn], 32);
      if ((w & 1) && lane < 32) { st_s[w >> 1][0][32 * tn + j] = a1; st_s[w >> 1][1][32 * tn + j] = a2; }
      s1[tn] = a1;
      s2[tn] = a2;
    }
    __syncthreads();
    if (!(w & 1) && lane < 32 && mw < M) {
      const long t64 = mw >> 6;
#pragma unroll
      for (int tn = 0; tn < NT; ++tn) {
        const int jc = n0 + 32 * tn + j;
        if (jc < Co) {
          stats_part[(t64 * 2 + 0) * Co + jc] = s1[tn] + st_s[w >> 1][0][32 * tn + j];
          stats_part[(t64 * 2 + 1) * Co + jc] = s2[tn] + st_s[w >> 1][1][32 * tn + j];
        }
      }
    }
  }
}

template <int WM, int WN>
__global__ __launch_bounds__(256) __attribute__((amdgpu_waves_per_eu(2))) void r3d_gemm_tn_bx3_kernel(
    const float* __restrict__ A, long lda, const float* __restrict__ B, long ldb, long M, int Ca, int Cb, int tn_rows,
    float* __restrict__ part ) {
  constexpr int BM = 64 * WM, BN = 64 * WN;
  constexpr int XU = BM / 64, WU = BN / 64;
  extern __shared__ __attribute__((aligned(16))) unsigned short gb_smem[];
  unsigned short* As = gb_smem;
  unsigned short* Bs = gb_smem + 3 * BM * GB_RS;
  const int tid = threadIdx.x, lane = tid & 63, w = tid >> 6;
  const int wm = w / WN, wn = w - wm * WN;
  const int nti = (Ca + BM - 1) / BM, ntj = (Cb + BN - 1) / BN;
  const int tile = r3d_xcd_swizzle((int)blockIdx.x, (int)gridDim.x);
  const int chunk = tile / (nti * ntj), tij = tile - chunk * (nti * ntj);
  const int i0 = (tij % nti) * BM, j0 = (tij / nti) * BN;
  const long m_beg = (long)chunk * tn_rows, m_end = min(M, m_beg + tn_rows);
  const int crows = (int)(m_end - m_beg);
  const __amdgpu_buffer_rsrc_t ra =
      __builtin_amdgcn_make_buffer_rsrc((void*)(A + m_beg * lda), 0, (int)(((long)(crows - 1) * lda + Ca) * 4), 0x00020000);
  const __amdgpu_buffer_rsrc_t rb =
      __builtin_amdgcn_make_buffer_rsrc((void*)(B + m_beg * ldb), 0, (int)(((long)(crows - 1) * ldb + Cb) * 4), 0x00020000);
  const int lda4 = (int)lda * 4, ldb4 = (int)ldb * 4;
  int ao[XU], bo[WU], amc[XU], bmc[WU];
#pragma unroll
  for (int u = 0; u < XU; ++u) {
    const int c = tid + 256 * u;
    amc[u] = c / BM;
    ao[u] = 8 * amc[u] * lda4 + 4 * min(i0 + c % BM, Ca - 1);
  }
#pragma unroll
  for (int u = 0; u < WU; ++u) {
    const int c = tid + 256 * u;
    bmc[u] = c / BN;
    bo[u] = 8 * bmc[u] * ldb4 + 4 * min(j0 + c % BN, Cb - 1);
  }
  float ar[XU][8], br[WU][8];
  auto gload = [&](int mk) {
#pragma unroll
    for (int u = 0; u < XU; ++u)
#pragma unroll
      for (int t = 0; t < 8; ++t) ar[u][t] = __uint_as_float(__builtin_amdgcn_raw_buffer_load_b32(ra, ao[u] + (mk + t) * lda4, 0, 0));
#pragma unroll
    for (int u = 0; u < WU; ++u)
#pragma unroll
      for (int t = 0; t < 8; ++t) br[u][t] = __uint_as_float(__builtin_amdgcn_raw_buffer_load_b32(rb, bo[u] + (mk + t) * ldb4, 0, 0));
  };
  f32x16 acc[2][2];
#pragma unroll
  for (int a = 0; a < 2; ++a)
#pragma unroll
    for (int b = 0; b < 2; ++b)
#pragma unroll
      for (int r = 0; r < 16; ++r) acc[a][b][r] = 0.f;
  gload(0);
  for (int mk = 0; mk < crows; mk += 32) {
#pragma unroll
    for (int u = 0; u < XU; ++u) { const int c = tid + 256 * u; gb_store_chunk(As, BM, c % BM, amc[u], ar[u]); }
#pragma unroll
    for (int u = 0; u < WU; ++u) { const int c = tid + 256 * u; gb_store_chunk(Bs, BN, c % BN, bmc[u], br[u]); }
    __syncthreads();
    gload(mk + 32);
    __builtin_amdgcn_sched_barrier(0);
    gb_wave_mma(As, BM, 64 * wm, Bs, BN, 64 * wn, lane, acc);
    __syncthreads();
  }
  float* out = part + (long)chunk * Ca * Cb;
#pragma unroll
  for (int tm = 0; tm < 2; ++tm)
#pragma unroll
    for (int tn = 0; tn < 2; ++tn) {
      const int j = j0 + 64 * wn + 32 * tn + (lane & 31);
#pragma unroll
      for (int r = 0; r < 16; ++r) {
        const int i = i0 + 64 * wm + 32 * tm + r3d_acc_row(r, lane);
        if (i < Ca && j < Cb) out[(long)i * Cb + j] = acc[tm][tn][r];
      }
    }
}

static const size_t GB_LDS_22 = sizeof(unsigned short) * 3 * (128 + 128) * GB_RS;
static const size_t GB_LDS_41 = sizeof(unsigned short) * 3 * (256 + 64) * GB_RS;

template <typename KernelT>
static int gb_lds_attr(KernelT k, size_t bytes) {
  return hipFuncSetAttribute((const void*)k, hipFuncAttributeMaxDynamicSharedMemorySize, (int)bytes) == hipSuccess ? 0 : 1;
}

bool r3d_pointwise_bx3_ok(const float* X, long ldx, const float* W, long M, int K, int Co) {
  return g_r3d_matrix_arith == 1 && (g_r3d_gemm_bx3 & 1) && K >= 32 && K % 32 == 0 && (ldx & 3) == 0 &&
         ((uintptr_t)X & 15) == 0 && ((uintptr_t)W & 15) == 0 && Co >= 32 && Co % 4 == 0 && M >= 64;
}

static int g_wpack_in_capture = 0;
extern "C" int r3d_set_wpack_in_capture(int on) {
  const int old = g_wpack_in_capture;
  g_wpack_in_capture = on ? 1 : 0;
  return old;
}
struct WPackBuf { int dev; hipStream_t st; void* p; size_t cap; };
static unsigned short* wpack_scratch(hipStream_t st, size_t bytes) {
  static std::mutex mu;
  static std::vector<WPackBuf> pool;
  hipStreamCaptureStatus cs = hipStreamCaptureStatusNone;
  if (hipStreamIsCapturing(st, &cs) != hipSuccess) return nullptr;
  const bool capturing = cs != hipStreamCaptureStatusNone;
  if (capturing && !g_wpack_in_capture) return nullptr;
  int dev = 0;
  if (hipGetDevice(&dev) != hipSuccess) return nullptr;
  std::lock_guard<std::mutex> lock(mu);
  for (auto& b : pool)
    if (b.dev == dev && b.st == st) {
      if (b.cap >= bytes) return (unsigned short*)b.p;
      if (capturing) return nullptr;
      void* p = nullptr;
      if (hipMalloc(&p, bytes) != hipSuccess) return nullptr;
      b.p = p; b.cap = bytes;
      return (unsigned short*)p;
    }
  if (capturing) return nullptr;
  void* p = nullptr;
  const size_t cap = bytes < (4u << 20) ? (4u << 20) : bytes;
  if (hipMalloc(&p, cap) != hipSuccess) return nullptr;
  pool.push_back(WPackBuf{dev, st, p, cap});
  return (unsigned short*)p;
}

int r3d_pointwise_bx3_launch(const float* X, long ldx, const float* W, long M, int K, int Co, const float* scale,
                             const float* shift, int act, float* Out, long ldo, int accumulate, float* stats_part,
                             hipStream_t st) {
  if ((ldo & 3) != 0 || ((uintptr_t)Out & 15) != 0) return -1;
  if (!(GB_ABL & 128) && (g_r3d_gemm_bx3 & 4) && M >= 256) {
    const int bnp = Co > 64 ? 128 : 64;
    const int Cop = r3d_cdiv(Co, bnp) * bnp;
    unsigned short* wp = wpack_scratch(st, (size_t)Cop * K * 6);
    if (wp) {
      hipLaunchKernelGGL(r3d_w_pack_bx3_kernel, dim3(r3d_cdiv((long)Cop * (K / 8), 256)), dim3(256), 0, st, W, K, Co, bnp, wp);
      const long tiles = (long)r3d_cdiv(M, 128) * (Cop / bnp);
      R3D_REQUIRE(tiles < 0x7fffffffL, "r3d_pointwise_conv: too many tiles");
      if (bnp == 128)
        hipLaunchKernelGGL((r3d_pointwise_gemm_bx3p_kernel<4>), dim3((unsigned)tiles), dim3(256), 0, st, X, ldx, wp, (int)M, K, Co,
                           scale, shift, act, Out, ldo, accumulate, stats_part);
      else
        hipLaunchKernelGGL((r3d_pointwise_gemm_bx3p_kernel<2>), dim3((unsigned)tiles), dim3(256), 0, st, X, ldx, wp, (int)M, K, Co,
                           scale, shift, act, Out, ldo, accumulate, stats_part);
      return R3D_OK;
    }
  }
  const int bn = (Co > 64 && !(GB_ABL & 64)) ? 128 : 64;
  const long tiles = (long)r3d_cdiv(M, 256) * r3d_cdiv(Co, bn);
  R3D_REQUIRE(tiles < 0x7fffffffL, "r3d_pointwise_conv: too many tiles");
  if (bn == 128)
    hipLaunchKernelGGL((r3d_pointwise_gemm_bx3_kernel<4>), dim3((unsigned)tiles), dim3(256), 0, st, X, ldx, W, (int)M, K, Co, scale,
                       shift, act, Out, ldo, accumulate, stats_part);
  else
    hipLaunchKernelGGL((r3d_pointwise_gemm_bx3_kernel<2>), dim3((unsigned)tiles), dim3(256), 0, st, X, ldx, W, (int)M, K, Co, scale,
                       shift, act, Out, ldo, accumulate, stats_part);
  return R3D_OK;
}

bool r3d_gemm_tn_bx3_ok(int Ca, int Cb) { return g_r3d_matrix_arith == 1 && (g_r3d_gemm_bx3 & 2) && Ca >= 32 && Cb >= 32; }

int r3d_gemm_tn_bx3_tiles(int Ca, int Cb) {
  return Cb > 64 ? r3d_cdiv(Ca, 128) * r3d_cdiv(Cb, 128) : r3d_cdiv(Ca, 256) * r3d_cdiv(Cb, 64);
}

template <int WM, int WN>
static int gemm_tn_bx3_go(size_t lds, int blocks, hipStream_t st, const float* A, long lda, const float* B, long ldb, long M,
                          int Ca, int Cb, int rows, float* part) {
  static bool attr = false;
  if (!attr) {
    R3D_REQUIRE(gb_lds_attr(r3d_gemm_tn_bx3_kernel<WM, WN>, lds) == 0, "r3d_gemm_tn: cannot reserve %zu B of LDS", lds);
    attr = true;
  }
  hipLaunchKernelGGL((r3d_gemm_tn_bx3_kernel<WM, WN>), dim3(blocks), dim3(256), lds, st, A, lda, B, ldb, M, Ca, Cb, rows, part);
  return R3D_OK;
}

int r3d_gemm_tn_bx3_launch(const float* A, long lda, const float* B, long ldb, long M, int Ca, int Cb, int rows, int chunks,
                           float* part, hipStream_t st) {
  const int blocks = r3d_gemm_tn_bx3_tiles(Ca, Cb) * chunks;
  if (Cb > 64) return gemm_tn_bx3_go<2, 2>(GB_LDS_22, blocks, st, A, lda, B, ldb, M, Ca, Cb, rows, part);
  return gemm_tn_bx3_go<4, 1>(GB_LDS_41, blocks, st, A, lda, B, ldb, M, Ca, Cb, rows, part);
}
```

### r3dfsseg_amd/csrc/train_ops.hip

```cpp
#include "common.h"

#define TS_ROWS 512
#define TS_MAXC 1024

__global__ __launch_bounds__(256) void r3d_colpartial_kernel(
    const float* __restrict__ X, long ldx, const float* __restrict__ DY, long lddy, r3d_segmap sm, int C, int mode,
    const float* __restrict__ scale, const float* __restrict__ shift, const float* __restrict__ mean,
    const float* __restrict__ invstd, long bn_stride, int act, int rows_per_chunk_a, int rows_per_chunk_b, int cmax,
    float* __restrict__ part ) {
  __shared__ float sa[4][64], sb[4][64];
  const int lane = threadIdx.x & 63, w = threadIdx.x >> 6;
  const int c = blockIdx.x * 64 + lane;
  const int seg = blockIdx.z;
  const long srows = sm.seg_rows(seg);
  const int rows_per_chunk = sm.odd(seg) ? rows_per_chunk_b : rows_per_chunk_a;
  const long s0 = (long)blockIdx.y * rows_per_chunk;
  if (s0 >= srows) return;
  const long base = sm.seg_row0(seg);
  const long r0 = base + s0;
  const long r1 = base + min(srows, s0 + rows_per_chunk);
  float a = 0.f, b = 0.f;
  if (c < C) {
    float sc = 1.f, sh = 0.f, mu = 0.f, is = 1.f;
    if (mode == 1) {
      const long o = (long)seg * bn_stride + c;
      sc = scale[o]; sh = shift[o]; mu = mean[o]; is = invstd[o];
    }
    for (long rb = r0 + w; rb < r1; rb += 32) {
      float xv[8], gv[8];
#pragma unroll
      for (int u = 0; u < 8; ++u) {
        const long r = min(rb + 4 * u, r1 - 1);
        xv[u] = X[r * ldx + c];
        gv[u] = mode == 1 ? DY[r * lddy + c] : 0.f;
      }
#pragma unroll
      for (int u = 0; u < 8; ++u) {
        if (rb + 4 * u < r1) {
          const float x = xv[u];
          if (mode == 0) {
            a += x;
            b += x * x;
          } else {
            const float uu = sc * x + sh;
            float g = gv[u];
            if (act == 1) g = uu > 0.f ? g : 0.f;
            else if (act == 2) g = uu > 0.f ? g : 0.2f * g;
            a += g;
            b += g * ((x - mu) * is);
          }
        }
      }
    }
  }
  sa[w][lane] = a;
  sb[w][lane] = b;
  __syncthreads();
  if (w == 0 && c < C) {
    const long slot = (long)seg * cmax + blockIdx.y;
    part[(slot * 2 + 0) * C + c] = ((sa[0][lane] + sa[1][lane]) + sa[2][lane]) + sa[3][lane];
    part[(slot * 2 + 1) * C + c] = ((sb[0][lane] + sb[1][lane]) + sb[2][lane]) + sb[3][lane];
  }
}

__global__ __launch_bounds__(256) void r3d_colpartial_v4_kernel(
    const float* __restrict__ X, long ldx, const float* __restrict__ DY, long lddy, r3d_segmap sm, int C, int mode,
    const float* __restrict__ scale, const float* __restrict__ shift, const float* __restrict__ mean,
    const float* __restrict__ invstd, long bn_stride, int act, int rows_per_chunk_a, int rows_per_chunk_b, int cmax,
    float* __restrict__ part ) {
  __shared__ float4 sa[4][64], sb[4][64];
  const int lane = threadIdx.x & 63, w = threadIdx.x >> 6;
  const int c = blockIdx.x * 256 + 4 * lane;
  const int seg = blockIdx.z;
  const long srows = sm.seg_rows(seg);
  const int rows_per_chunk = sm.odd(seg) ? rows_per_chunk_b : rows_per_chunk_a;
  const long s0 = (long)blockIdx.y * rows_per_chunk;
  if (s0 >= srows) return;
  const long base = sm.seg_row0(seg);
  const long r0 = base + s0;
  const long r1 = base + min(srows, s0 + rows_per_chunk);
  float4 a = make_float4(0.f, 0.f, 0.f, 0.f), b = a;
  float4 sc = make_float4(1.f, 1.f, 1.f, 1.f), sh = make_float4(0.f, 0.f, 0.f, 0.f), mu = sh, is = sc;
  if (mode == 1) {
    const long o = (long)seg * bn_stride + c;
    sc = *reinterpret_cast<const float4*>(scale + o); sh = *reinterpret_cast<const float4*>(shift + o);
    mu = *reinterpret_cast<const float4*>(mean + o); is = *reinterpret_cast<const float4*>(invstd + o);
  }
  auto acc = [&](float x, float g0, float sc_, float sh_, float mu_, float is_, float& a_, float& b_) {
    if (mode == 0) {
      a_ += x;
      b_ += x * x;
    } else {
      const float uu = sc_ * x + sh_;
      float g = g0;
      if (act == 1) g = uu > 0.f ? g : 0.f;
      else if (act == 2) g = uu > 0.f ? g : 0.2f * g;
      a_ += g;
      b_ += g * ((x - mu_) * is_);
    }
  };
  for (long rb = r0 + w; rb < r1; rb += 32) {
    float4 xv[8], gv[8];
#pragma unroll
    for (int u = 0; u < 8; ++u) {
      const long r = min(rb + 4 * u, r1 - 1);
      xv[u] = *reinterpret_cast<const float4*>(X + r * ldx + c);
      gv[u] = mode == 1 ? *reinterpret_cast<const float4*>(DY + r * lddy + c) : make_float4(0.f, 0.f, 0.f, 0.f);
    }
#pragma unroll
    for (int u = 0; u < 8; ++u) {
      if (rb + 4 * u < r1) {
        acc(xv[u].x, gv[u].x, sc.x, sh.x, mu.x, is.x, a.x, b.x);
        acc(xv[u].y, gv[u].y, sc.y, sh.y, mu.y, is.y, a.y, b.y);
        acc(xv[u].z, gv[u].z, sc.z, sh.z, mu.z, is.z, a.z, b.z);
        acc(xv[u].w, gv[u].w, sc.w, sh.w, mu.w, is.w, a.w, b.w);
      }
    }
  }
  sa[w][lane] = a;
  sb[w][lane] = b;
  __syncthreads();
  if (w == 0) {
    const long slot = (long)seg * cmax + blockIdx.y;
    float4 ta, tb;
    ta.x = ((sa[0][lane].x + sa[1][lane].x) + sa[2][lane].x) + sa[3][lane].x; ta.y = ((sa[0][lane].y + sa[1][lane].y) + sa[2][lane].y) + sa[3][lane].y;
    ta.z = ((sa[0][lane].z + sa[1][lane].z) + sa[2][lane].z) + sa[3][lane].z; ta.w = ((sa[0][lane].w + sa[1][lane].w) + sa[2][lane].w) + sa[3][lane].w;
    tb.x = ((sb[0][lane].x + sb[1][lane].x) + sb[2][lane].x) + sb[3][lane].x; tb.y = ((sb[0][lane].y + sb[1][lane].y) + sb[2][lane].y) + sb[3][lane].y;
    tb.z = ((sb[0][lane].z + sb[1][lane].z) + sb[2][lane].z) + sb[3][lane].z; tb.w = ((sb[0][lane].w + sb[1][lane].w) + sb[2][lane].w) + sb[3][lane].w;
    *reinterpret_cast<float4*>(part + (slot * 2 + 0) * C + c) = ta;
    *reinterpret_cast<float4*>(part + (slot * 2 + 1) * C + c) = tb;
  }
}

__global__ __launch_bounds__(256) void r3d_colreduce_kernel(const float* __restrict__ part, int count_a, int count_b,
                                                            int cmax, int C, float* __restrict__ out ) {
  __shared__ double sa[4][64], sb[4][64];
  const int lane = threadIdx.x & 63, w = threadIdx.x >> 6;
  const int c = blockIdx.x * 64 + lane;
  const int seg = blockIdx.y;
  const bool odd = count_b > 0 && (seg & 1);
  const int chunks = odd ? count_b : count_a;
  const long first = cmax > 0 ? (long)seg * cmax
                              : (count_b > 0 ? (long)(seg >> 1) * (count_a + count_b) + (odd ? count_a : 0) : (long)seg * count_a);
  part += first * 2 * C;
  out += (long)seg * 2 * C;
  double a = 0.0, b = 0.0;
  if (c < C) {
    int k = w;
    for (; k + 12 < chunks; k += 16) {
      float va[4], vb[4];
#pragma unroll
      for (int u = 0; u < 4; ++u) {
        va[u] = part[((long)(k + 4 * u) * 2 + 0) * C + c];
        vb[u] = part[((long)(k + 4 * u) * 2 + 1) * C + c];
      }
#pragma unroll
      for (int u = 0; u < 4; ++u) { a += (double)va[u]; b += (double)vb[u]; }
    }
    for (; k < chunks; k += 4) {
      a += (double)part[((long)k * 2 + 0) * C + c];
      b += (double)part[((long)k * 2 + 1) * C + c];
    }
  }
  sa[w][lane] = a;
  sb[w][lane] = b;
  __syncthreads();
  if (w == 0 && c < C) {
    out[c] = (float)(((sa[0][lane] + sa[1][lane]) + sa[2][lane]) + sa[3][lane]);
    out[C + c] = (float)(((sb[0][lane] + sb[1][lane]) + sb[2][lane]) + sb[3][lane]);
  }
}

__global__ void r3d_bn_fold_kernel(const float* __restrict__ sums , int n_seg, double count_a,
                                   double count_b, int C, const float* __restrict__ gamma,
                                   const float* __restrict__ beta, float eps, float momentum,
                                   float* __restrict__ running_mean, float* __restrict__ running_var,
                                   float* __restrict__ mean, float* __restrict__ invstd, float* __restrict__ scale,
                                   float* __restrict__ shift, long bn_stride, float* __restrict__ rec,
                                   const int* __restrict__ rec_index, long rec_stride) {
  const int c = blockIdx.x * blockDim.x + threadIdx.x;
  if (c >= C) return;
  const float g = gamma[c], bt = beta[c];
  float rm = running_mean ? running_mean[c] : 0.f, rv = running_var ? running_var[c] : 0.f;
  const long rec0 = rec_index ? *rec_index : 0;
  for (int s0 = 0; s0 < n_seg; s0 += 8) {
    float sv[8], qv[8];
#pragma unroll
    for (int u = 0; u < 8; ++u) {
      const long o = (long)min(s0 + u, n_seg - 1) * 2 * C;
      sv[u] = sums[o + c];
      qv[u] = sums[o + C + c];
    }
#pragma unroll
    for (int u = 0; u < 8; ++u) {
      const int seg = s0 + u;
      if (seg >= n_seg) break;
      const double count = (count_b > 0.0 && (seg & 1)) ? count_b : count_a;
      const double m = (double)sv[u] / count;
      double var = (double)qv[u] / count - m * m;
      if (var < 0.0) var = 0.0;
      const float is = (float)(1.0 / sqrt(var + (double)eps));
      const long o = (long)seg * bn_stride + c;
      mean[o] = (float)m;
      invstd[o] = is;
      const float sc = g * is;
      scale[o] = sc;
      shift[o] = bt - (float)m * sc;
      const double unb = count > 1.0 ? var * count / (count - 1.0) : var;
      if (rec) {
        float* r = rec + (rec0 + seg) * rec_stride;
        r[c] = (float)m;
        r[C + c] = (float)unb;
      } else if (running_mean) {
        rm = (1.f - momentum) * rm + momentum * (float)m;
        rv = (1.f - momentum) * rv + momentum * (float)unb;
      }
    }
  }
  if (!rec && running_mean) {
    running_mean[c] = rm;
    running_var[c] = rv;
  }
}

__global__ void r3d_bn_running_update_kernel(const float* __restrict__ rec, int n_records, long rec_stride, int C, float momentum,
                                             const float* __restrict__ bias, float* __restrict__ running_mean,
                                             float* __restrict__ running_var) {
  const int c = blockIdx.x * blockDim.x + threadIdx.x;
  if (c >= C) return;
  float rm = running_mean[c], rv = running_var[c];
  const float mb = bias ? momentum * bias[c] : 0.f;
  for (int k0 = 0; k0 < n_records; k0 += 8) {
    float mv[8], vv[8];
#pragma unroll
    for (int u = 0; u < 8; ++u) {
      const long o = (long)min(k0 + u, n_records - 1) * rec_stride;
      mv[u] = rec[o + c];
      vv[u] = rec[o + C + c];
    }
#pragma unroll
    for (int u = 0; u < 8; ++u) {
      if (k0 + u < n_records) {
        rm = (1.f - momentum) * rm + momentum * mv[u];
        if (bias) rm = rm + mb;
        rv = (1.f - momentum) * rv + momentum * vv[u];
      }
    }
  }
  running_mean[c] = rm;
  running_var[c] = rv;
}


#define EW_ROWS 32
__global__ __launch_bounds__(256) void r3d_affine_act_kernel(const float* __restrict__ Z, long ldz, int M, int C, r3d_segmap sm,
                                                             const float* __restrict__ scale, const float* __restrict__ shift,
                                                             long bn_stride, int act, float* __restrict__ Y, long ldy) {
  const int lane = threadIdx.x & 63, w = threadIdx.x >> 6;
  const int r0 = blockIdx.x * EW_ROWS + w;
  long zo[EW_ROWS / 4], yo[EW_ROWS / 4], bo[EW_ROWS / 4];
#pragma unroll
  for (int u = 0; u < EW_ROWS / 4; ++u) {
    const int r = min(r0 + 4 * u, M - 1);
    zo[u] = (long)r * ldz; yo[u] = (long)r * ldy;
    bo[u] = (long)sm.seg_of_row32(r) * bn_stride;
  }
  for (int c = lane; c < C; c += 64) {
    float zv[EW_ROWS / 4], sc[EW_ROWS / 4], sh[EW_ROWS / 4];
#pragma unroll
    for (int u = 0; u < EW_ROWS / 4; ++u) { zv[u] = Z[zo[u] + c]; sc[u] = scale[bo[u] + c]; sh[u] = shift[bo[u] + c]; }
#pragma unroll
    for (int u = 0; u < EW_ROWS / 4; ++u) {
      float v = sc[u] * zv[u] + sh[u];
      if (act == 1) v = fmaxf(v, 0.f);
      else if (act == 2) v = v > 0.f ? v : 0.2f * v;
      if (r0 + 4 * u < M) Y[yo[u] + c] = v;
    }
  }
}

__global__ __launch_bounds__(256) void r3d_bn_bwd_apply_kernel(
    const float* __restrict__ Z, long ldz, const float* __restrict__ DY, long lddy, int M, int C, r3d_segmap sm,
    const float* __restrict__ scale, const float* __restrict__ shift, const float* __restrict__ mean,
    const float* __restrict__ invstd, long bn_stride, int act, const float* __restrict__ sums ,
    double count_a, double count_b, float* __restrict__ DZ, long lddz) {
  const int lane = threadIdx.x & 63, w = threadIdx.x >> 6;
  const int r0 = blockIdx.x * EW_ROWS + w;
  constexpr int U = 4;
  for (int rr = 0; rr < EW_ROWS / 4; rr += U) {
    long zo[U], go[U], oo[U], bo[U], so[U];
    double cnt[U];
    bool same = true;
#pragma unroll
    for (int u = 0; u < U; ++u) {
      const int r = min(r0 + 4 * (rr + u), M - 1);
      const int seg = sm.seg_of_row32(r);
      zo[u] = (long)r * ldz; go[u] = (long)r * lddy; oo[u] = (long)r * lddz;
      bo[u] = (long)seg * bn_stride; so[u] = (long)seg * 2 * C;
      cnt[u] = sm.odd(seg) ? count_b : count_a;
      same = same && so[u] == so[0];
    }
    for (int c = lane; c < C; c += 64) {
      float z[U], g[U], sc[U], sh[U], mu[U], is[U], m1[U], m2[U];
#pragma unroll
      for (int u = 0; u < U; ++u) {
        z[u] = Z[zo[u] + c]; g[u] = DY[go[u] + c];
        sc[u] = scale[bo[u] + c]; sh[u] = shift[bo[u] + c]; mu[u] = mean[bo[u] + c]; is[u] = invstd[bo[u] + c];
      }
      if (same) {
        const float a1 = (float)((double)sums[so[0] + c] / cnt[0]), a2 = (float)((double)sums[so[0] + C + c] / cnt[0]);
#pragma unroll
        for (int u = 0; u < U; ++u) { m1[u] = a1; m2[u] = a2; }
      } else {
#pragma unroll
        for (int u = 0; u < U; ++u) {
          m1[u] = (float)((double)sums[so[u] + c] / cnt[u]);
          m2[u] = (float)((double)sums[so[u] + C + c] / cnt[u]);
        }
      }
#pragma unroll
      for (int u = 0; u < U; ++u) {
        const float uu = sc[u] * z[u] + sh[u];
        float gg = g[u];
        if (act == 1) gg = uu > 0.f ? gg : 0.f;
        else if (act == 2) gg = uu > 0.f ? gg : 0.2f * gg;
        const float zh = (z[u] - mu[u]) * is[u];
        if (r0 + 4 * (rr + u) < M) DZ[oo[u] + c] = sc[u] * (gg - m1[u] - zh * m2[u]);
      }
    }
  }
}

#define BA_ROWS 64
template <int NK >
__global__ __launch_bounds__(256) void r3d_bn_bwd_apply_v4_kernel(
    const float* __restrict__ Z, long ldz, const float* __restrict__ DY, long lddy, int M, int C, r3d_segmap sm,
    const float* __restrict__ scale, const float* __restrict__ shift, const float* __restrict__ mean,
    const float* __restrict__ invstd, long bn_stride, int act, const float* __restrict__ sums, double count_a, double count_b,
    float* __restrict__ DZ, long lddz) {
  const int lane = threadIdx.x & 63, w = threadIdx.x >> 6;
  const int lpr = NK > 1 ? 64 : C >> 2;
  const int rpw = 64 / lpr;
  const int col0 = 4 * (lane & (lpr - 1));
  const int rsub = lane / lpr;
  const int rb0 = blockIdx.x * BA_ROWS;
  const int rb1 = min(rb0 + BA_ROWS, M) - 1;
  const int seg_first = sm.seg_of_row32(rb0), seg_last = sm.seg_of_row32(rb1);
  float4 sc[NK], sh[NK], mu[NK], is[NK], m1[NK], m2[NK];
  int cur = -1;
  auto load_consts = [&](int seg) {
    const long bo = (long)seg * bn_stride, so = (long)seg * 2 * C;
    const double cnt = sm.odd(seg) ? count_b : count_a;
#pragma unroll
    for (int kk = 0; kk < NK; ++kk) {
      const int c = col0 + 256 * kk;
      sc[kk] = *reinterpret_cast<const float4*>(scale + bo + c); sh[kk] = *reinterpret_cast<const float4*>(shift + bo + c);
      mu[kk] = *reinterpret_cast<const float4*>(mean + bo + c); is[kk] = *reinterpret_cast<const float4*>(invstd + bo + c);
      const float4 s1 = *reinterpret_cast<const float4*>(sums + so + c), s2 = *reinterpret_cast<const float4*>(sums + so + C + c);
      m1[kk] = make_float4((float)((double)s1.x / cnt), (float)((double)s1.y / cnt), (float)((double)s1.z / cnt), (float)((double)s1.w / cnt));
      m2[kk] = make_float4((float)((double)s2.x / cnt), (float)((double)s2.y / cnt), (float)((double)s2.z / cnt), (float)((double)s2.w / cnt));
    }
    cur = seg;
  };
  load_consts(seg_first);
  const bool one_seg = seg_first == seg_last;
  auto elem = [&](float z, float g, float sc_, float sh_, float mu_, float is_, float m1_, float m2_) {
    const float uu = sc_ * z + sh_;
    float gg = g;
    if (act == 1) gg = uu > 0.f ? gg : 0.f;
    else if (act == 2) gg = uu > 0.f ? gg : 0.2f * gg;
    const float zh = (z - mu_) * is_;
    return sc_ * (gg - m1_ - zh * m2_);
  };
  constexpr int U = NK > 1 ? 2 : 4;
  const int step = 4 * rpw;
  for (int it = 0; it < BA_ROWS; it += U * step) {
    float4 z[U][NK], g[U][NK];
    int row[U];
#pragma unroll
    for (int u = 0; u < U; ++u) {
      row[u] = rb0 + it + u * step + rpw * w + rsub;
      const int r = min(row[u], M - 1);
#pragma unroll
      for (int kk = 0; kk < NK; ++kk) {
        z[u][kk] = *reinterpret_cast<const float4*>(Z + (long)r * ldz + col0 + 256 * kk);
        g[u][kk] = *reinterpret_cast<const float4*>(DY + (long)r * lddy + col0 + 256 * kk);
      }
    }
#pragma unroll
    for (int u = 0; u < U; ++u) {
      if (!one_seg) {
        const int seg = sm.seg_of_row32(min(row[u], M - 1));
        if (seg != cur) load_consts(seg);
      }
      if (row[u] < M && row[u] <= rb1) {
#pragma unroll
        for (int kk = 0; kk < NK; ++kk) {
          float4 o;
          o.x = elem(z[u][kk].x, g[u][kk].x, sc[kk].x, sh[kk].x, mu[kk].x, is[kk].x, m1[kk].x, m2[kk].x);
          o.y = elem(z[u][kk].y, g[u][kk].y, sc[kk].y, sh[kk].y, mu[kk].y, is[kk].y, m1[kk].y, m2[kk].y);
          o.z = elem(z[u][kk].z, g[u][kk].z, sc[kk].z, sh[kk].z, mu[kk].z, is[kk].z, m1[kk].z, m2[kk].z);
          o.w = elem(z[u][kk].w, g[u][kk].w, sc[kk].w, sh[kk].w, mu[kk].w, is[kk].w, m1[kk].w, m2[kk].w);
          *reinterpret_cast<float4*>(DZ + (long)row[u] * lddz + col0 + 256 * kk) = o;
        }
      }
    }
  }
}

#define TN_ROWS_MAX 4096
bool r3d_gemm_tn_bx3_ok(int Ca, int Cb);
int r3d_gemm_tn_bx3_tiles(int Ca, int Cb);
int r3d_gemm_tn_bx3_launch(const float* A, long lda, const float* B, long ldb, long M, int Ca, int Cb, int rows, int chunks,
                           float* part, hipStream_t st);
static int tn_rows(long M, int Ca, int Cb, bool bx3) {
  const long tiles = bx3 ? r3d_gemm_tn_bx3_tiles(Ca, Cb) : (long)((Ca + 63) / 64) * ((Cb + 63) / 64);
  long chunks = (bx3 ? 512 : 1024) / tiles;
  if (chunks < 1) chunks = 1;
  long rows = (M + chunks - 1) / chunks;
  rows = ((rows + 31) / 32) * 32;
  if (rows < 128) rows = 128;
  if (rows > TN_ROWS_MAX) rows = TN_ROWS_MAX;
  return (int)rows;
}
__global__ __launch_bounds__(256) void r3d_gemm_tn_kernel(const float* __restrict__ A, long lda, const float* __restrict__ B,
                                                          long ldb, long M, int Ca, int Cb, int TN_ROWS,
                                                          float* __restrict__ part ) {
  __shared__ float As[2][32 * 65];
  __shared__ float Bs[2][32 * 65];
  const int tid = threadIdx.x, lane = tid & 63, w = tid >> 6;
  const int wi = w >> 1, wj = w & 1;
  const int nti = (Ca + 63) / 64, ntj = (Cb + 63) / 64;
  const int tile = r3d_xcd_swizzle((int)blockIdx.x, (int)gridDim.x);
  const int chunk = tile / (nti * ntj), tij = tile - chunk * (nti * ntj);
  const int i0 = (tij % nti) * 64, j0 = (tij / nti) * 64;
  const long m_beg = (long)chunk * TN_ROWS, m_end = min(M, m_beg + TN_ROWS);
  f32x16 acc;
#pragma unroll
  for (int r = 0; r < 16; ++r) acc[r] = 0.f;
  const int srow = tid >> 6, scol = tid & 63;
  float av[8], bv[8];
  const float* acol = A + min(i0 + scol, Ca - 1);
  const float* bcol = B + min(j0 + scol, Cb - 1);
  auto load_stage = [&](long m0) {
    if (m0 + 32 <= m_end) {
#pragma unroll
      for (int p = 0; p < 8; ++p) {
        const long m = m0 + srow + 4 * p;
        av[p] = acol[m * lda];
        bv[p] = bcol[m * ldb];
      }
    } else {
#pragma unroll
      for (int p = 0; p < 8; ++p) {
        const long m = m0 + srow + 4 * p;
        const long mc = min(m, M - 1);
        av[p] = r3d_keep(acol[mc * lda], m < m_end);
        bv[p] = r3d_keep(bcol[mc * ldb], m < m_end);
      }
    }
  };
  auto store_stage = [&](int buf) {
#pragma unroll
    for (int p = 0; p < 8; ++p) {
      As[buf][(srow + 4 * p) * 65 + scol] = av[p];
      Bs[buf][(srow + 4 * p) * 65 + scol] = bv[p];
    }
  };
  load_stage(m_beg);
  store_stage(0);
  __syncthreads();
  int buf = 0;
  for (long m0 = m_beg; m0 < m_end; m0 += 32, buf ^= 1) {
    const bool more = m0 + 32 < m_end;
    if (more) load_stage(m0 + 32);
    __builtin_amdgcn_sched_barrier(0);
#pragma unroll
    for (int s2 = 0; s2 < 16; ++s2) {
      const int m = 2 * s2 + (lane >> 5);
      acc = __builtin_amdgcn_mfma_f32_32x32x2f32(As[buf][m * 65 + 32 * wi + (lane & 31)], Bs[buf][m * 65 + 32 * wj + (lane & 31)],
                                                 acc, 0, 0, 0);
    }
    if (more) store_stage(buf ^ 1);
    __syncthreads();
  }
  const int j = j0 + 32 * wj + (lane & 31);
#pragma unroll
  for (int r = 0; r < 16; ++r) {
    const int i = i0 + 32 * wi + r3d_acc_row(r, lane);
    if (i < Ca && j < Cb) part[((long)chunk * Ca + i) * Cb + j] = acc[r];
  }
}

__global__ void r3d_chunk_reduce_kernel(const float* __restrict__ part, int chunks, long n, float alpha,
                                        float* __restrict__ out, int accumulate) {
  const long i = (long)blockIdx.x * blockDim.x + threadIdx.x;
  if (i >= n) return;
  float s = 0.f;
  int k = 0;
  for (; k + 8 <= chunks; k += 8) {
    float v[8];
#pragma unroll
    for (int u = 0; u < 8; ++u) v[u] = part[(long)(k + u) * n + i];
#pragma unroll
    for (int u = 0; u < 8; ++u) s += v[u];
  }
  for (; k < chunks; ++k) s += part[(long)k * n + i];
  out[i] = accumulate ? out[i] + alpha * s : alpha * s;
}

__global__ __launch_bounds__(256) void r3d_add_cols_kernel(const float* __restrict__ src, long lds_, float* __restrict__ dst,
                                                           long ldd, long M, int C) {
  const int lane = threadIdx.x & 63;
  const long r0 = ((long)blockIdx.x * 4 + (threadIdx.x >> 6)) * 4;
  for (int c = lane; c < C; c += 64) {
    float a[4], b[4];
#pragma unroll
    for (int u = 0; u < 4; ++u) {
      const long r = r0 + u < M ? r0 + u : M - 1;
      a[u] = src[r * lds_ + c]; b[u] = dst[r * ldd + c];
    }
#pragma unroll
    for (int u = 0; u < 4; ++u)
      if (r0 + u < M) dst[(r0 + u) * ldd + c] = b[u] + a[u];
  }
}

static int ts_rows(long M, int C) {
  const long groups = (C + 63) / 64;
  long chunks = 1024 / groups;
  if (chunks > M / 64) chunks = M / 64;
  if (chunks < 1) chunks = 1;
  long rows = (M + chunks - 1) / chunks;
  rows = ((rows + 31) / 32) * 32;
  if (rows > TS_ROWS) rows = TS_ROWS;
  return (int)rows;
}
static int ts_chunks(long rows, int C) { return rows > 0 ? r3d_cdiv(rows, ts_rows(rows, C)) : 0; }
extern "C" long r3d_colstats_seg_ws_words(long M, int C, long rows_a, long rows_b) {
  const r3d_segmap sm{rows_a, rows_b};
  if (!sm.covers(M)) return 0;
  const int ca = ts_chunks(rows_a, C), cb = ts_chunks(rows_b, C);
  return (long)sm.n_seg(M) * (ca > cb ? ca : cb) * 2L * C + 16;
}
extern "C" long r3d_colstats_ws_words(long M, int C) { return r3d_colstats_seg_ws_words(M, C, M, 0); }

extern "C" int r3d_colstats_seg(const float* X, long ldx, const float* DY, long lddy, long M, int C, long rows_a,
                                long rows_b, int mode, const float* scale, const float* shift, const float* mean,
                                const float* invstd, long bn_stride, int act, float* sums_out, float* ws, void* stream) {
  R3D_REQUIRE(X && sums_out && ws && M > 0 && C > 0 && C <= TS_MAXC, "r3d_colstats: bad arguments");
  R3D_REQUIRE(mode == 0 || (DY && scale && shift && mean && invstd), "r3d_colstats: mode 1 needs dy and the BN vectors");
  const r3d_segmap sm{rows_a, rows_b};
  R3D_REQUIRE(sm.covers(M), "r3d_colstats: %ld rows are not whole segments of %ld + %ld rows", M, rows_a, rows_b);
  const int ra = ts_rows(rows_a, C), rb = rows_b > 0 ? ts_rows(rows_b, C) : ra;
  const int ca = ts_chunks(rows_a, C), cb = ts_chunks(rows_b, C);
  const int cmax = ca > cb ? ca : cb, n_seg = sm.n_seg(M);
  R3D_REQUIRE(n_seg <= 65535 && cmax <= 65535, "r3d_colstats: too many segments");
  hipStream_t st = (hipStream_t)stream;
  const bool v4 = C % 256 == 0 && ((ldx | (DY ? lddy : 0) | bn_stride) & 3) == 0 &&
                  (((uintptr_t)X | (uintptr_t)DY | (uintptr_t)scale | (uintptr_t)shift | (uintptr_t)mean | (uintptr_t)invstd |
                    (uintptr_t)ws) & 15) == 0;
  if (v4)
    hipLaunchKernelGGL(r3d_colpartial_v4_kernel, dim3(C / 256, cmax, n_seg), dim3(256), 0, st, X, ldx, DY, lddy, sm, C, mode,
                       scale, shift, mean, invstd, bn_stride, act, ra, rb, cmax, ws);
  else
  hipLaunchKernelGGL(r3d_colpartial_kernel, dim3(r3d_cdiv(C, 64), cmax, n_seg), dim3(256), 0, st, X, ldx, DY, lddy, sm, C, mode,
                     scale, shift, mean, invstd, bn_stride, act, ra, rb, cmax, ws);
  hipLaunchKernelGGL(r3d_colreduce_kernel, dim3(r3d_cdiv(C, 64), n_seg), dim3(256), 0, st, ws, ca, cb, cmax, C, sums_out);
  R3D_LAUNCH_CHECK("r3d_colstats");
  return R3D_OK;
}
extern "C" int r3d_colstats(const float* X, long ldx, const float* DY, long lddy, long M, int C, int mode,
                            const float* scale, const float* shift, const float* mean, const float* invstd, int act,
                            float* sums_out, float* ws, void* stream) {
  return r3d_colstats_seg(X, ldx, DY, lddy, M, C, M, 0, mode, scale, shift, mean, invstd, 0, act, sums_out, ws, stream);
}

extern "C" int r3d_colreduce_seg(const float* part, int count_a, int count_b, int n_seg, int C, float* sums_out, void* stream) {
  R3D_REQUIRE(part && sums_out && count_a > 0 && count_b >= 0 && n_seg > 0 && n_seg <= 65535 && C > 0,
              "r3d_colreduce: bad arguments");
  hipLaunchKernelGGL(r3d_colreduce_kernel, dim3(r3d_cdiv(C, 64), n_seg), dim3(256), 0, (hipStream_t)stream, part, count_a, count_b,
                     0, C, sums_out);
  R3D_LAUNCH_CHECK("r3d_colreduce");
  return R3D_OK;
}
extern "C" int r3d_colreduce(const float* part, int chunks, int C, float* sums_out, void* stream) {
  return r3d_colreduce_seg(part, chunks, 0, 1, C, sums_out, stream);
}

extern "C" int r3d_bn_fold_seg(const float* sums, int n_seg, double count_a, double count_b, int C, const float* gamma,
                               const float* beta, float eps, float momentum, float* running_mean, float* running_var,
                               float* mean, float* invstd, float* scale, float* shift, long bn_stride, float* rec,
                               const int32_t* rec_index_dev, long rec_stride, void* stream) {
  R3D_REQUIRE(sums && gamma && beta && mean && invstd && scale && shift && C > 0 && count_a > 0 && count_b >= 0 && n_seg > 0,
              "r3d_bn_fold: bad arguments");
  R3D_REQUIRE(n_seg == 1 || bn_stride >= C, "r3d_bn_fold: %d segments need a vector stride of at least C", n_seg);
  R3D_REQUIRE(!rec || rec_stride >= 2L * C, "r3d_bn_fold: a record holds 2 C floats");
  hipLaunchKernelGGL(r3d_bn_fold_kernel, dim3(r3d_cdiv(C, 64)), dim3(64), 0, (hipStream_t)stream, sums, n_seg, count_a, count_b,
                     C, gamma, beta, eps, momentum, running_mean, running_var, mean, invstd, scale, shift, bn_stride, rec,
                     rec_index_dev, rec_stride);
  R3D_LAUNCH_CHECK("r3d_bn_fold");
  return R3D_OK;
}
extern "C" int r3d_bn_fold(const float* sums, double count, int C, const float* gamma, const float* beta, float eps,
                           float momentum, float* running_mean, float* running_var, float* mean, float* invstd,
                           float* scale, float* shift, float* rec, const int32_t* rec_index_dev, long rec_stride,
                           void* stream) {
  return r3d_bn_fold_seg(sums, 1, count, 0.0, C, gamma, beta, eps, momentum, running_mean, running_var, mean, invstd, scale,
                         shift, 0, rec, rec_index_dev, rec_stride, stream);
}

extern "C" int r3d_bn_running_update(const float* rec, int n_records, long rec_stride, int C, float momentum, const float* bias,
                                     float* running_mean, float* running_var, void* stream) {
  R3D_REQUIRE(rec && running_mean && running_var && n_records > 0 && C > 0 && rec_stride >= 2L * C,
              "r3d_bn_running_update: bad arguments");
  hipLaunchKernelGGL(r3d_bn_running_update_kernel, dim3(r3d_cdiv(C, 256)), dim3(256), 0, (hipStream_t)stream, rec, n_records,
                     rec_stride, C, momentum, bias, running_mean, running_var);
  R3D_LAUNCH_CHECK("r3d_bn_running_update");
  return R3D_OK;
}

extern "C" int r3d_affine_act_seg(const float* Z, long ldz, long M, int C, long rows_a, long rows_b, const float* scale,
                                  const float* shift, long bn_stride, int act, float* Y, long ldy, void* stream) {
  R3D_REQUIRE(Z && Y && scale && shift && M > 0 && C > 0, "r3d_affine_act: bad arguments");
  const r3d_segmap sm{rows_a, rows_b};
  R3D_REQUIRE(sm.covers(M), "r3d_affine_act: %ld rows are not whole segments of %ld + %ld rows", M, rows_a, rows_b);
  hipLaunchKernelGGL(r3d_affine_act_kernel, dim3(r3d_cdiv(M, EW_ROWS)), dim3(256), 0, (hipStream_t)stream, Z, ldz, (int)M, C, sm,
                     scale, shift, bn_stride, act, Y, ldy);
  R3D_LAUNCH_CHECK("r3d_affine_act");
  return R3D_OK;
}
extern "C" int r3d_affine_act(const float* Z, long ldz, long M, int C, const float* scale, const float* shift, int act,
                              float* Y, long ldy, void* stream) {
  return r3d_affine_act_seg(Z, ldz, M, C, M, 0, scale, shift, 0, act, Y, ldy, stream);
}

extern "C" int r3d_bn_bwd_apply_seg(const float* Z, long ldz, const float* DY, long lddy, long M, int C, long rows_a,
                                    long rows_b, const float* scale, const float* shift, const float* mean,
                                    const float* invstd, long bn_stride, int act, const float* sums, double count_a,
                                    double count_b, float* DZ, long lddz, void* stream) {
  R3D_REQUIRE(Z && DY && DZ && scale && shift && mean && invstd && sums, "r3d_bn_bwd_apply: null pointer");
  const r3d_segmap sm{rows_a, rows_b};
  R3D_REQUIRE(sm.covers(M) && count_a > 0, "r3d_bn_bwd_apply: %ld rows are not whole segments of %ld + %ld rows", M, rows_a,
              rows_b);
  const bool pow2 = C >= 16 && C <= 1024 && (C & (C - 1)) == 0;
  const bool al16 = ((ldz | lddy | lddz | bn_stride) & 3) == 0 &&
                    (((uintptr_t)Z | (uintptr_t)DY | (uintptr_t)DZ | (uintptr_t)scale | (uintptr_t)shift | (uintptr_t)mean |
                      (uintptr_t)invstd | (uintptr_t)sums) & 15) == 0;
  if (pow2 && al16) {
#define BA_GO(NK)                                                                                                             \
  hipLaunchKernelGGL(r3d_bn_bwd_apply_v4_kernel<NK>, dim3(r3d_cdiv(M, BA_ROWS)), dim3(256), 0, (hipStream_t)stream, Z, ldz, DY, \
                     lddy, (int)M, C, sm, scale, shift, mean, invstd, bn_stride, act, sums, count_a, count_b, DZ, lddz)
    if (C <= 256) BA_GO(1);
    else if (C == 512) BA_GO(2);
    else BA_GO(4);
#undef BA_GO
  } else
  hipLaunchKernelGGL(r3d_bn_bwd_apply_kernel, dim3(r3d_cdiv(M, EW_ROWS)), dim3(256), 0, (hipStream_t)stream, Z, ldz, DY,
                     lddy, (int)M, C, sm, scale, shift, mean, invstd, bn_stride, act, sums, count_a, count_b, DZ, lddz);
  R3D_LAUNCH_CHECK("r3d_bn_bwd_apply");
  return R3D_OK;
}
extern "C" int r3d_bn_bwd_apply(const float* Z, long ldz, const float* DY, long lddy, long M, int C, const float* scale,
                                const float* shift, const float* mean, const float* invstd, int act, const float* sums,
                                double count, float* DZ, long lddz, void* stream) {
  return r3d_bn_bwd_apply_seg(Z, ldz, DY, lddy, M, C, M, 0, scale, shift, mean, invstd, 0, act, sums, count, 0.0, DZ, lddz,
                              stream);
}

extern "C" long r3d_gemm_tn_ws_words(long M, int Ca, int Cb) {
  const int r0 = tn_rows(M, Ca, Cb, false), r1 = tn_rows(M, Ca, Cb, true);
  const int rows = r0 < r1 ? r0 : r1;
  return ((M + rows - 1) / rows) * (long)Ca * Cb + 16;
}

extern "C" int r3d_gemm_tn(const float* A, long lda, const float* B, long ldb, long M, int Ca, int Cb, float alpha,
                           float* out, int accumulate, float* ws, void* stream) {
  R3D_REQUIRE(A && B && out && ws && M > 0 && Ca > 0 && Cb > 0 && lda >= Ca && ldb >= Cb, "r3d_gemm_tn: bad arguments");
  const bool bx3 = r3d_gemm_tn_bx3_ok(Ca, Cb);
  const int rows = tn_rows(M, Ca, Cb, bx3);
  const int chunks = r3d_cdiv(M, rows);
  hipStream_t st = (hipStream_t)stream;
  if (bx3) {
    const int rc = r3d_gemm_tn_bx3_launch(A, lda, B, ldb, M, Ca, Cb, rows, chunks, ws, st);
    if (rc) return rc;
  } else {
    hipLaunchKernelGGL(r3d_gemm_tn_kernel, dim3(r3d_cdiv(Ca, 64) * r3d_cdiv(Cb, 64) * chunks), dim3(256), 0, st, A, lda, B,
                       ldb, M, Ca, Cb, rows, ws);
  }
  hipLaunchKernelGGL(r3d_chunk_reduce_kernel, dim3(r3d_cdiv((long)Ca * Cb, 256)), dim3(256), 0, st, ws, chunks,
                     (long)Ca * Cb, alpha, out, accumulate);
  R3D_LAUNCH_CHECK("r3d_gemm_tn");
  return R3D_OK;
}

extern "C" int r3d_add_cols(const float* src, long ld_src, float* dst, long ld_dst, long M, int C, void* stream) {
  R3D_REQUIRE(src && dst && M > 0 && C > 0, "r3d_add_cols: bad arguments");
  hipLaunchKernelGGL(r3d_add_cols_kernel, dim3(r3d_cdiv(M, 16)), dim3(256), 0, (hipStream_t)stream, src, ld_src, dst,
                     ld_dst, M, C);
  R3D_LAUNCH_CHECK("r3d_add_cols");
  return R3D_OK;
}
```

### r3dfsseg_amd/train_ops.py

```python
import contextlib
import ctypes
from collections import namedtuple

import torch

from . import _lib, ops
from .ops import SegLayout, _p, _rows, _st, _timed

BN_EPS, BN_MOM = 1e-5, 0.1
update_running_stats = True


class BNRecorder:

    def __init__(self, max_episodes, device):
        self.max_records = 2 * max_episodes
        self.device = device
        self.tables = {}
        self.index_dev = None

    def slot_for(self, bnmod, bias):
        if bnmod not in self.tables:
            rec = torch.zeros(self.max_records, 2, bnmod.num_features, device=self.device, dtype=torch.float32)
            self.tables[bnmod] = (rec, bias.detach() if bias is not None else None)
        return self.tables[bnmod][0]

    def apply(self, n_episodes):
        lib = _lib.load()
        assert 2 * n_episodes <= self.max_records
        with torch.no_grad():
            for bnmod, (rec, bias) in self.tables.items():
                C = bnmod.num_features
                _lib.check(lib.r3d_bn_running_update(_p(rec), 2 * n_episodes, 2 * C, C, BN_MOM, _p(bias),
                                                     _p(bnmod.running_mean), _p(bnmod.running_var), _st()))
                bnmod.num_batches_tracked += 2 * n_episodes


bn_recorder = None


@contextlib.contextmanager
def recording(rec):
    global bn_recorder
    saved, bn_recorder = bn_recorder, rec
    try:
        yield rec
    finally:
        bn_recorder = saved


def deferred_running_stats(model):
    rec = model.__dict__.get("_bn_rec1")
    if rec is None:
        rec = model.__dict__["_bn_rec1"] = BNRecorder(1, next(model.parameters()).device)
    return recording(rec)


def _f(n, dev):
    return torch.empty(n, device=dev, dtype=torch.float32)


class BNVec:

    def __init__(self, n_seg, C, dev):
        self.t = torch.empty(n_seg, 4, C, device=dev, dtype=torch.float32)
        self.stride = 4 * C

    @property
    def scale(self): return self.t[:, 0]
    @property
    def shift(self): return self.t[:, 1]
    @property
    def mean(self): return self.t[:, 2]
    @property
    def invstd(self): return self.t[:, 3]

    def ptrs(self):
        return _p(self.t[0, 0]), _p(self.t[0, 1]), _p(self.t[0, 2]), _p(self.t[0, 3])


def colstats(X, C, seg, mode=0, DY=None, bn=None, act=0):
    M, ldx = _rows(X)
    dev = X.device
    lib = _lib.load()
    sums = _f(seg.n_seg * 2 * C, dev).view(seg.n_seg, 2, C)
    ws = _f(lib.r3d_colstats_seg_ws_words(M, C, seg.rows_a, seg.rows_b), dev)
    lddy = DY.stride(0) if DY is not None else 0
    sc, sh, mu, is_ = bn.ptrs() if bn is not None else (None, None, None, None)
    with _timed("bn_stats"):
        _lib.check(lib.r3d_colstats_seg(_p(X), ldx, _p(DY), lddy, M, C, seg.rows_a, seg.rows_b, mode, sc, sh, mu, is_,
                                        bn.stride if bn is not None else 0, act, _p(sums), _p(ws), _st()))
    return sums


def bn_fold(sums, counts, bnmod, bias=None):
    n_seg, _, C = sums.shape
    dev = sums.device
    lib = _lib.load()
    bn = BNVec(n_seg, C, dev)
    rec = bn_recorder
    if rec is not None:
        table, idx_dev = rec.slot_for(bnmod, bias), rec.index_dev
    elif update_running_stats:
        table, idx_dev = torch.empty(n_seg, 2, C, device=dev, dtype=torch.float32), None
    else:
        table, idx_dev = None, None
    sc, sh, mu, is_ = bn.ptrs()
    _lib.check(lib.r3d_bn_fold_seg(_p(sums), n_seg, counts[0], counts[1], C, _p(bnmod.weight), _p(bnmod.bias), BN_EPS, BN_MOM,
                                   None, None, mu, is_, sc, sh, bn.stride, _p(table), _p(idx_dev), 2 * C, _st()))
    if rec is None and table is not None:
        with torch.no_grad():
            _lib.check(lib.r3d_bn_running_update(_p(table), n_seg, 2 * C, C, BN_MOM, _p(bias.detach()) if bias is not None else None,
                                                 _p(bnmod.running_mean), _p(bnmod.running_var), _st()))
            bnmod.num_batches_tracked += n_seg
    return bn


def affine_act(Z, bn, act, seg, out=None):
    M, ldz = _rows(Z)
    C = Z.shape[1]
    if out is None:
        out = torch.empty(M, C, device=Z.device, dtype=torch.float32)
    sc, sh, _, _ = bn.ptrs()
    _lib.check(_lib.load().r3d_affine_act_seg(_p(Z), ldz, M, C, seg.rows_a, seg.rows_b, sc, sh, bn.stride, act, _p(out),
                                              out.stride(0), _st()))
    return out


def bn_bwd_apply(Z, DY, bn, act, sums, counts, seg, out=None):
    M, ldz = _rows(Z)
    C = Z.shape[1]
    DZ = torch.empty(M, C, device=Z.device, dtype=torch.float32) if out is None else out
    sc, sh, mu, is_ = bn.ptrs()
    _lib.check(_lib.load().r3d_bn_bwd_apply_seg(_p(Z), ldz, _p(DY), DY.stride(0), M, C, seg.rows_a, seg.rows_b, sc, sh, mu, is_,
                                                bn.stride, act, _p(sums), counts[0], counts[1], _p(DZ), DZ.stride(0), _st()))
    return DZ


def gemm_tn(A, B):
    M, lda = _rows(A)
    M2, ldb = _rows(B)
    assert M == M2
    Ca, Cb = A.shape[1], B.shape[1]
    lib = _lib.load()
    out = torch.empty(Ca, Cb, device=A.device, dtype=torch.float32)
    ws = _f(lib.r3d_gemm_tn_ws_words(M, Ca, Cb), A.device)
    with _timed("gemm_tn"):
        _lib.check(lib.r3d_gemm_tn(_p(A), lda, _p(B), ldb, M, Ca, Cb, 1.0, _p(out), 0, _p(ws), _st()))
    return out


def conv_acc(X, W, out):
    M, ldx = _rows(X)
    with _timed("pointwise_conv"):
        _lib.check(_lib.load().r3d_pointwise_conv_acc(_p(X), ldx, _p(W), M, X.shape[1], W.shape[0], None, None, 0, _p(out),
                                                      out.stride(0), _st()))


def add_cols(src, dst):
    M, lds = _rows(src)
    _lib.check(_lib.load().r3d_add_cols(_p(src), lds, _p(dst), dst.stride(0), M, src.shape[1], _st()))


def _one_segment(M):
    return SegLayout(1, 1, 0, M)


def conv_bn_fwd(X, W2d, bnmod, act, bias=None, out=None, seg=None):
    M, ldx = _rows(X)
    C = W2d.shape[0]
    lib = _lib.load()
    seg = _one_segment(M) if seg is None else seg
    assert seg.M == M
    z = torch.empty(M, C, device=X.device, dtype=torch.float32)
    if seg.aligned(64):
        sums = _f(seg.n_seg * 2 * C, X.device).view(seg.n_seg, 2, C)
        ws = _f(lib.r3d_pointwise_conv_stats_ws_words(M, C), X.device)
        with _timed("pointwise_conv"):
            _lib.check(lib.r3d_pointwise_conv_stats_seg(_p(X), ldx, _p(W2d), M, X.shape[1], C, _p(z), C, seg.rows_a, seg.rows_b,
                                                        _p(sums), _p(ws), _st()))
    else:
        ops.pointwise_conv(X, W2d, out=z)
        sums = colstats(z, C, seg, mode=0)
    bn = bn_fold(sums, seg.counts(), bnmod, bias)
    y = affine_act(z, bn, act, seg, out=out)
    return y, (X, W2d, z, bn, act, seg)


def conv_bn_bwd(saved, dY, want_dx=True, dx_acc=None):
    X, W2d, z, bn, act, seg = saved
    C = W2d.shape[0]
    M = z.shape[0]
    sums = colstats(z, C, seg, mode=1, DY=dY, bn=bn, act=act)
    dz = bn_bwd_apply(z, dY, bn, act, sums, seg.counts(), seg)
    dW = gemm_tn(dz, X)
    tot = sums.sum(0) if seg.n_seg > 1 else sums[0]
    dbias = torch.zeros(C, device=z.device, dtype=torch.float32)
    dX = None
    if want_dx:
        Wt = W2d.t().contiguous()
        if dx_acc is not None:
            conv_acc(dz, Wt, dx_acc)
        else:
            dX = ops.pointwise_conv(dz, Wt)
    return dW, tot[1], tot[0], dbias, dX


def edgeconv_train_fwd(inp, idx, ec, B, N, out, seg=None):
    lib = _lib.load()
    dev = inp.device
    seg = SegLayout(1, B, 0, N) if seg is None else seg
    assert seg.B == B and seg.N == N
    W1 = ec.layer[0].weight.reshape(64, -1)
    C = W1.shape[1] // 2
    Wpq = torch.cat((W1[:, :C], W1[:, C:] - W1[:, :C]), 0).contiguous()
    PQ = ops.pointwise_conv(inp, Wpq)
    K = idx.shape[-1]
    ws = _f(lib.r3d_edgeconv_train_ws_words(B, N), dev)
    W2 = ec.layer[3].weight.reshape(64, 64).contiguous()
    M = B * N
    argmax = torch.empty(M, 64, device=dev, dtype=torch.int32)
    argmin = torch.empty(M, 64, device=dev, dtype=torch.int32)
    zmax = torch.empty(M, 64, device=dev, dtype=torch.float32)
    zmin = torch.empty(M, 64, device=dev, dtype=torch.float32)
    idx3 = idx.view(B, N, K)
    sums1 = _f(seg.n_seg * 128, dev).view(seg.n_seg, 2, 64)
    sums2 = _f(seg.n_seg * 128, dev).view(seg.n_seg, 2, 64)
    counts = seg.counts(per_row=K)
    esum = torch.empty(M, 64, device=dev, dtype=torch.float32)
    with _timed("edgeconv"):
        _lib.check(lib.r3d_edge_stats1(_p(PQ), _p(idx3), B, N, K, seg.S, seg.Q, _p(sums1), _p(esum), _p(ws), _st()))
    bn1 = bn_fold(sums1, counts, ec.layer[1])
    sc1, sh1, _, _ = bn1.ptrs()
    with _timed("edgeconv"):
        _lib.check(lib.r3d_edgeconv_train_fwd_minmax(_p(PQ), _p(idx3), sc1, sh1, bn1.stride, _p(W2), B, N, K, seg.S, seg.Q,
                                                     _p(zmax), _p(zmin), _p(argmax), _p(argmin), _p(sums2), _p(ws), _st()))
    bn2 = bn_fold(sums2, counts, ec.layer[4])
    sc2, sh2, _, _ = bn2.ptrs()
    with _timed("edgeconv"):
        _lib.check(lib.r3d_edge_select(_p(zmax), _p(zmin), _p(argmax), _p(argmin), sc2, sh2, bn2.stride, M, seg.rows_a,
                                       seg.rows_b, _p(out), out.stride(0), _st()))
    return (inp, idx3, Wpq, PQ, W2, bn1, bn2, argmax, zmax, C, seg, esum)


def edgeconv_train_bwd(saved, dout, B, N, dx_acc):
    inp, idx3, Wpq, PQ, W2, bn1, bn2, argmax, zmax, C, seg, esum = saved
    lib = _lib.load()
    dev = PQ.device
    K = idx3.shape[-1]
    M = B * N
    dPQ = _f(M * 128, dev).view(M, 128)
    ws = _f(lib.r3d_edgeconv_train_ws_words(B, N), dev)
    rev = torch.empty(lib.r3d_edge_reverse_ws_words(B, N, K), device=dev, dtype=torch.int32)
    with _timed("edgeconv_bwd"):
        _lib.check(lib.r3d_edge_reverse(_p(idx3), B, N, K, _p(rev), rev.numel(), _st()))
    bn2_sums = colstats(zmax, 64, seg, mode=1, DY=dout, bn=bn2, act=ops.ACT_LRELU)
    DY1, BE = _f(M * K * 64, dev), _f(M * 128, dev)
    dW2, bn1_sums = _f(64 * 64, dev), _f(seg.n_seg * 128, dev).view(seg.n_seg, 2, 64)
    s1, t1, m1, i1 = bn1.ptrs()
    s2, t2, m2, i2 = bn2.ptrs()
    with _timed("edgeconv_bwd"):
        _lib.check(lib.r3d_edgeconv_bwd(_p(PQ), _p(idx3), s1, t1, m1, i1, _p(W2), s2, t2, m2, i2, bn1.stride, _p(bn2_sums),
                                        _p(dout), dout.stride(0), _p(argmax), _p(zmax), _p(esum), B, N, K, seg.S, seg.Q, _p(DY1),
                                        _p(BE), _p(rev),
                                        _p(dW2), _p(bn1_sums), _p(dPQ), _p(ws), _st()))
    t1s = bn1_sums.sum(0) if seg.n_seg > 1 else bn1_sums[0]
    t2s = bn2_sums.sum(0) if seg.n_seg > 1 else bn2_sums[0]
    dWpq = gemm_tn(dPQ, inp)
    dW1 = torch.cat((dWpq[:64] - dWpq[64:], dWpq[64:]), 1).reshape(64, 2 * C, 1, 1)
    if dx_acc is not None:
        conv_acc(dPQ, Wpq.t().contiguous(), dx_acc)
    return dW1, t1s[1], t1s[0], dW2.view(64, 64, 1, 1), t2s[1], t2s[0]


EncoderSaved = namedtuple("EncoderSaved", "model seg seed p_drop seed_dev ec mlp base cat level2 qkv lse feat aws")


def encoder_forward(model, x, seed, seg=None):
    enc, base, att = model.encoder, model.base_learner, model.att_learner
    lib = _lib.load()
    B, _, N = x.shape
    M = B * N
    dev = x.device
    if seg is None:
        seg = SegLayout(1, B, 0, N)
    assert seg.B == B and seg.N == N
    x_pm, x_cm = ops.input_layouts(x)
    cat = torch.empty(M, 64 * enc.n_edgeconv, device=dev, dtype=torch.float32)
    inp, ec_saved = x_pm, []
    for l in range(enc.n_edgeconv):
        idx = ops.knn(inp, B, N, enc.k, x_cm=x_cm if l == 0 else None)
        if enc.idx_patch is not None:
            idx = enc.idx_patch(l, idx.view(B, N, enc.k)).view(idx.shape)
        out = cat[:, 64 * l:64 * (l + 1)]
        ec_saved.append(edgeconv_train_fwd(inp, idx, enc.edge_convs[l], B, N, out, seg))
        inp = out
    h, mlp_saved = cat, []
    for jn in range(len(enc.conv.layer_dims)):
        W = enc.conv.layer[3 * jn].weight
        h, sv = conv_bn_fwd(h, W.reshape(W.shape[0], -1).contiguous(), enc.conv.layer[3 * jn + 1], ops.ACT_LRELU, seg=seg)
        mlp_saved.append(sv)
    level2 = h
    feat = torch.empty(M, model.feat_dim, device=dev, dtype=torch.float32)
    od = att.out_channel
    ops.copy_cols(cat[:, :64], feat[:, :64])
    hb, base_saved = level2, []
    for i, seq in enumerate(base.convs):
        last = i == base.num_convs - 1
        W = seq[0].weight
        hb, sv = conv_bn_fwd(hb, W.reshape(W.shape[0], -1).contiguous(), seq[1], ops.ACT_NONE if last else ops.ACT_RELU,
                             bias=seq[0].bias, out=feat[:, 64 + od:] if last else None, seg=seg)
        base_saved.append(sv)
    Wqkv, qscale = att._fold()
    qkv = ops.pointwise_conv(level2, Wqkv, qscale, None, ops.ACT_NONE)
    lse = torch.empty(M, device=dev, dtype=torch.float32)
    p_drop = float(att.dropout.p)
    aws = _f(lib.r3d_attention_ws_words_ep_d(B, N, seg.clouds, od), dev)
    with _timed("attention"):
        _lib.check(lib.r3d_attention_fwd_train_ep_d(_p(qkv), 3 * od, B, N, _p(feat[:, 64:64 + od]), feat.stride(0), _p(lse),
                                                    p_drop, ctypes.c_uint(seed & 0xffffffff), _p(model._slot.seed_dev),
                                                    seg.clouds, od, _p(aws), _st()))
    model._dbg_idx = [sv[1] for sv in ec_saved]
    if getattr(model, "_trace", None) is not None:
        for e in range(seg.E):
            for b0, Bs in ((e * seg.clouds, seg.S), (e * seg.clouds + seg.S, seg.Q)):
                if Bs:
                    model._trace.setdefault("idx", []).append([sv[1][b0:b0 + Bs] for sv in ec_saved])
                    model._trace.setdefault("argmax", []).append([sv[7][b0 * N:(b0 + Bs) * N] for sv in ec_saved])
    return feat, EncoderSaved(model, seg, seed, p_drop, model._slot.seed_dev, ec_saved, mlp_saved, base_saved, cat, level2,
                              qkv, lse, feat, aws)


def encoder_backward(saved, dfeat):
    model, seg = saved.model, saved.seg
    enc, base, att = model.encoder, model.base_learner, model.att_learner
    B, N, M = seg.B, seg.N, seg.M
    ec_saved, mlp_saved, base_saved = saved.ec, saved.mlp, saved.base
    cat, level2, qkv, lse, feat, aws = saved.cat, saved.level2, saved.qkv, saved.lse, saved.feat, saved.aws
    lib = _lib.load()
    dev = dfeat.device
    dfeat = dfeat.contiguous()
    g = {}
    dlevel2 = torch.zeros(M, level2.shape[1], device=dev, dtype=torch.float32)
    od = att.out_channel
    d = dfeat[:, 64 + od:]
    for i in reversed(range(base.num_convs)):
        seq = base.convs[i]
        dW, dg, db, dbias, dX = conv_bn_bwd(base_saved[i], d, want_dx=True, dx_acc=dlevel2 if i == 0 else None)
        g[seq[0].weight] = dW.view_as(seq[0].weight)
        g[seq[0].bias] = dbias
        g[seq[1].weight], g[seq[1].bias] = dg, db
        d = dX
    dqkv = torch.empty(M, 3 * od, device=dev, dtype=torch.float32)
    with _timed("attention_bwd"):
        _lib.check(lib.r3d_attention_bwd_ep_d(_p(qkv), 3 * od, B, N, _p(feat[:, 64:64 + od]), feat.stride(0),
                                              _p(dfeat[:, 64:64 + od]), dfeat.stride(0), _p(lse), saved.p_drop,
                                              ctypes.c_uint(saved.seed & 0xffffffff), _p(saved.seed_dev), seg.clouds, od,
                                              1.0 / att.temperature, _p(dqkv), 3 * od, _p(aws), 1, _st()))
    dWqkv = gemm_tn(dqkv, level2)
    for k, m in enumerate((att.q_map, att.k_map, att.v_map)):
        g[m.weight] = dWqkv[od * k:od * (k + 1)].reshape(m.weight.shape)
    Wraw = torch.cat([m.weight.reshape(od, -1) for m in (att.q_map, att.k_map, att.v_map)], 0)
    conv_acc(dqkv, Wraw.t().contiguous(), dlevel2)
    dcat = torch.zeros(M, cat.shape[1], device=dev, dtype=torch.float32)
    add_cols(dfeat[:, :64], dcat[:, :64])
    d = dlevel2
    for jn in reversed(range(len(mlp_saved))):
        conv, bnm = enc.conv.layer[3 * jn], enc.conv.layer[3 * jn + 1]
        dW, dg, db, _, dX = conv_bn_bwd(mlp_saved[jn], d, want_dx=True, dx_acc=dcat if jn == 0 else None)
        g[conv.weight] = dW.view_as(conv.weight)
        g[bnm.weight], g[bnm.bias] = dg, db
        d = dX
    for l in reversed(range(enc.n_edgeconv)):
        ec = enc.edge_convs[l]
        dx_acc = dcat[:, 64 * (l - 1):64 * l] if l > 0 else None
        dW1, dg1, db1, dW2, dg2, db2 = edgeconv_train_bwd(ec_saved[l], dcat[:, 64 * l:64 * (l + 1)], B, N, dx_acc)
        g[ec.layer[0].weight], g[ec.layer[1].weight], g[ec.layer[1].bias] = dW1, dg1, db1
        g[ec.layer[3].weight], g[ec.layer[4].weight], g[ec.layer[4].bias] = dW2, dg2, db2
    return [g.get(p) for p in encoder_params(model)]


def encoder_params(model):
    return list(model.encoder.parameters()) + list(model.base_learner.parameters()) + list(model.att_learner.parameters())


def _adjacent_rows(a, b):
    base = a._base
    if base is None or base is not b._base or base.dim() != 2 or not base.is_contiguous():
        return None
    if not (a.is_contiguous() and b.is_contiguous() and a.dim() == 2 and b.dim() == 2 and a.shape[1] == b.shape[1] == base.shape[1]):
        return None
    if base.shape[0] != a.shape[0] + b.shape[0] or a.data_ptr() != base.data_ptr():
        return None
    if b.data_ptr() != base.data_ptr() + a.numel() * a.element_size():
        return None
    return base


def next_dropout_seed(model):
    slot = model._slot
    if slot.seed_dev is not None:
        slot.seed_dev.add_(2)
        return 0
    model._drop_seed = getattr(model, "_drop_seed", 0) + 2
    return model._drop_seed


def next_dropout_seeds(model, E):
    slot = model._slot
    if slot.seed_dev is not None:
        slot.seed_dev.add_(2 * E)
        return 2 - 2 * E
    seed = getattr(model, "_drop_seed", 0) + 2
    model._drop_seed = seed + 2 * (E - 1)
    return seed


class EncoderTrainFn(torch.autograd.Function):

    @staticmethod
    def forward(ctx, x, model, seed, seg, *params):
        feat, ctx.saved = encoder_forward(model, x, seed, seg)
        if seg is None or seg.Q == 0:
            return feat
        assert seg.E == 1
        return feat[:seg.rows_a], feat[seg.rows_a:]

    @staticmethod
    def backward(ctx, *dfeats):
        saved, ctx.saved = ctx.saved, None
        if len(dfeats) == 2:
            rows, feat = (saved.seg.rows_a, saved.seg.rows_b), saved.feat
            dfeats = [d if d is not None else torch.zeros(r, feat.shape[1], device=feat.device, dtype=torch.float32)
                      for d, r in zip(dfeats, rows)]
            dfeat = _adjacent_rows(*dfeats)
            if dfeat is None:
                dfeat = torch.cat(dfeats, 0)
        else:
            dfeat = dfeats[0]
        return (None, None, None, None) + tuple(encoder_backward(saved, dfeat))


def get_features_train(model, x, seed, seg=None):
    return EncoderTrainFn.apply(x, model, seed, seg, *encoder_params(model))


def explicit_encoder_step(model, batch, grad_sink, head):
    E = batch.E
    S, N = model.n_way * model.k_shot, model.n_points
    Q = batch.query_x.shape[1]
    with torch.no_grad():
        seed = next_dropout_seeds(model, E)
        seg = SegLayout(E, S, Q, N)
        feat, saved = encoder_forward(model, batch.x_all.view(E * (S + Q), model.in_channels, N), seed, seg)
        outputs, dfeat, extra = head(feat, seg)
        assert dfeat.shape[0] == feat.shape[0]
        grads = encoder_backward(saved, dfeat)
        index = {id(p): i for i, p in enumerate(q for q in model.parameters() if q.requires_grad)}
        dst, src = [], []
        for p, g in list(zip(encoder_params(model), grads)) + extra:
            if g is not None:
                dst.append(grad_sink[index[id(p)]])
                src.append(g.reshape(p.shape))
        torch._foreach_add_(dst, src)
    return outputs
```

Baseline: 389.9.

## Emit pre-split bf16x3 dz from BN backward and consume it in weight and input GEMMs

New measurement: 383.9. -1.5%, worse.

```diff
diff --git a/include/r3d.h b/include/r3d.h
--- a/include/r3d.h
+++ b/include/r3d.h
@@ -137,6 +137,21 @@
                 int accumulate, float* ws, void* stream);
 int r3d_add_cols(const float* src, long ld_src, float* dst, long ld_dst, long M, int C, void* stream);
 
+int r3d_affine_act_seg_cut(const float* Z, long ldz, long M, int C, long rows_a, long rows_b, const float* scale,
+                           const float* shift, long bn_stride, int act, float* Y , long ldy, void* Yc, long ldc, int pw,
+                           void* stream);
+int r3d_bn_bwd_apply_seg_cut(const float* Z, long ldz, const float* DY, long lddy, long M, int C, long rows_a, long rows_b,
+                             const float* scale, const float* shift, const float* mean, const float* invstd, long bn_stride,
+                             int act, const float* sums, double count_a, double count_b, float* DZ , long lddz,
+                             void* DZc, long ldc, int pw, void* stream);
+int r3d_pointwise_conv_cut_ok(long M, int K, int Co, void* stream);
+int r3d_pointwise_conv_cut(const void* Xc, long ldc, int pw, const float* W, long M, int K, int Co, const float* scale,
+                           const float* shift, int act, float* Out, long ldo, int accumulate, float* stats_part ,
+                           void* stream);
+int r3d_gemm_tn_cut_supported(int Ca, int Cb, int a_cut, int b_cut);
+int r3d_gemm_tn_cut(const void* A, long lda, int apw, const void* B, long ldb, int bpw, long M, int Ca, int Cb, float alpha,
+                    float* out, int accumulate, float* ws, void* stream);
+
 long r3d_edgeconv_train_ws_words(int B, int N);
 int r3d_edge_stats1(const float* PQ, const int32_t* idx, int B, int N, int K, int clouds_a, int clouds_b,
                     float* sums_out , float* esum , float* ws,
diff --git a/r3dfsseg_amd/_lib.py b/r3dfsseg_amd/_lib.py
--- a/r3dfsseg_amd/_lib.py
+++ b/r3dfsseg_amd/_lib.py
@@ -100,6 +100,13 @@
     "r3d_bn_fold_seg": (c_i, [c_f, c_i, c_d, c_d, c_i, c_f, c_f, c_fl, c_fl, c_f, c_f, c_f, c_f, c_f, c_f, c_l, c_f, c_f, c_l, c_f]),
     "r3d_affine_act_seg": (c_i, [c_f, c_l, c_l, c_i, c_l, c_l, c_f, c_f, c_l, c_i, c_f, c_l, c_f]),
     "r3d_bn_bwd_apply_seg": (c_i, [c_f, c_l, c_f, c_l, c_l, c_i, c_l, c_l, c_f, c_f, c_f, c_f, c_l, c_i, c_f, c_d, c_d, c_f, c_l, c_f]),
+    "r3d_affine_act_seg_cut": (c_i, [c_f, c_l, c_l, c_i, c_l, c_l, c_f, c_f, c_l, c_i, c_f, c_l, c_f, c_l, c_i, c_f]),
+    "r3d_bn_bwd_apply_seg_cut": (c_i, [c_f, c_l, c_f, c_l, c_l, c_i, c_l, c_l, c_f, c_f, c_f, c_f, c_l, c_i, c_f, c_d, c_d, c_f, c_l,
+                                       c_f, c_l, c_i, c_f]),
+    "r3d_pointwise_conv_cut_ok": (c_i, [c_l, c_i, c_i, c_f]),
+    "r3d_pointwise_conv_cut": (c_i, [c_f, c_l, c_i, c_f, c_l, c_i, c_i, c_f, c_f, c_i, c_f, c_l, c_i, c_f, c_f]),
+    "r3d_gemm_tn_cut_supported": (c_i, [c_i, c_i, c_i, c_i]),
+    "r3d_gemm_tn_cut": (c_i, [c_f, c_l, c_i, c_f, c_l, c_i, c_l, c_i, c_i, c_fl, c_f, c_i, c_f, c_f]),
     "r3d_attention_ws_words_ep": (c_l, [c_i, c_i, c_i]),
     "r3d_attention_fwd_train_ep": (c_i, [c_f, c_l, c_i, c_i, c_f, c_l, c_f, c_fl, c_u, c_f, c_i, c_f, c_f]),
     "r3d_attention_bwd_ep": (c_i, [c_f, c_l, c_i, c_i, c_f, c_l, c_f, c_l, c_f, c_fl, c_u, c_f, c_i, c_fl, c_f, c_l, c_f, c_i, c_f]),
diff --git a/r3dfsseg_amd/csrc/common.h b/r3dfsseg_amd/csrc/common.h
--- a/r3dfsseg_amd/csrc/common.h
+++ b/r3dfsseg_amd/csrc/common.h
@@ -121,6 +121,31 @@
   return c;
 }
 
+struct r3d_cut {
+  unsigned short* p;
+  long ld;
+  int pw;
+};
+static __device__ __forceinline__ void r3d_cut_store4(const r3d_cut& t, long row, int col, float x0, float x1, float x2, float x3) {
+  const float v[8] = {x0, x1, x2, x3, 0.f, 0.f, 0.f, 0.f};
+  const r3d_bx3 f = r3d_bx3_split8(v);
+  unsigned short* d = t.p + row * t.ld + col;
+  *reinterpret_cast<uint2*>(d) = make_uint2(f.h[0], f.h[1]);
+  *reinterpret_cast<uint2*>(d + t.pw) = make_uint2(f.m[0], f.m[1]);
+  *reinterpret_cast<uint2*>(d + 2 * t.pw) = make_uint2(f.l[0], f.l[1]);
+}
+static __device__ __forceinline__ void r3d_cut_store1(const r3d_cut& t, long row, int col, float x) {
+  const float v[8] = {x, 0.f, 0.f, 0.f, 0.f, 0.f, 0.f, 0.f};
+  const r3d_bx3 f = r3d_bx3_split8(v);
+  unsigned short* d = t.p + row * t.ld + col;
+  d[0] = (unsigned short)f.h[0];
+  d[t.pw] = (unsigned short)f.m[0];
+  d[2 * t.pw] = (unsigned short)f.l[0];
+}
+static inline bool r3d_cut_valid(const void* p, long ld, int pw, int C) {
+  return p && ((uintptr_t)p & 15) == 0 && pw > 0 && pw % 8 == 0 && ld % 8 == 0 && pw >= C && ld >= 2L * pw + C;
+}
+
 extern int g_r3d_gemm_bx3;
 
 static inline int r3d_cdiv(long a, long b) { return (int)((a + b - 1) / b); }
diff --git a/r3dfsseg_amd/csrc/gemm.hip b/r3dfsseg_amd/csrc/gemm.hip
--- a/r3dfsseg_amd/csrc/gemm.hip
+++ b/r3dfsseg_amd/csrc/gemm.hip
@@ -166,6 +166,26 @@
   return pointwise_launch(X, ldx, W, M, K, Co, scale, shift, act, Out, ldo, 1, nullptr, stream);
 }
 
+bool r3d_pointwise_cut_ok(long M, int K, int Co, hipStream_t st);
+int r3d_pointwise_bx3_cut_launch(const void* Xc, long ldc, int pw, const float* W, long M, int K, int Co, const float* scale,
+                                 const float* shift, int act, float* Out, long ldo, int accumulate, float* stats_part,
+                                 hipStream_t st);
+extern "C" int r3d_pointwise_conv_cut_ok(long M, int K, int Co, void* stream) {
+  return r3d_pointwise_cut_ok(M, K, Co, (hipStream_t)stream) ? 1 : 0;
+}
+extern "C" int r3d_pointwise_conv_cut(const void* Xc, long ldc, int pw, const float* W, long M, int K, int Co,
+                                      const float* scale, const float* shift, int act, float* Out, long ldo, int accumulate,
+                                      float* stats_part, void* stream) {
+  R3D_REQUIRE(Xc && W && Out, "r3d_pointwise_conv_cut: null pointer");
+  R3D_REQUIRE(M > 0 && K > 0 && Co > 0 && ldo >= Co, "r3d_pointwise_conv_cut: bad shape M=%ld K=%d Co=%d ldo=%ld", M, K, Co, ldo);
+  R3D_REQUIRE(act >= 0 && act <= 2, "r3d_pointwise_conv_cut: unknown activation %d", act);
+  const int rc = r3d_pointwise_bx3_cut_launch(Xc, ldc, pw, W, M, K, Co, scale, shift, act, Out, ldo, accumulate, stats_part,
+                                              (hipStream_t)stream);
+  if (rc) return rc;
+  R3D_LAUNCH_CHECK("r3d_pointwise_conv_cut");
+  return R3D_OK;
+}
+
 static int pointwise_launch(const float* X, long ldx, const float* W, long M, int K, int Co, const float* scale,
                             const float* shift, int act, float* Out, long ldo, int accumulate, float* stats_part,
                             void* stream) {
diff --git a/r3dfsseg_amd/csrc/gemm_bx3.hip b/r3dfsseg_amd/csrc/gemm_bx3.hip
--- a/r3dfsseg_amd/csrc/gemm_bx3.hip
+++ b/r3dfsseg_amd/csrc/gemm_bx3.hip
@@ -255,9 +255,9 @@
   *reinterpret_cast<r3d_u32x4*>(d + 1024) = f.l;
 }
 
-template <int NT>
+template <int NT, bool XCUT>
 __global__ __launch_bounds__(256) __attribute__((amdgpu_waves_per_eu(3))) void r3d_pointwise_gemm_bx3p_kernel(
-    const float* __restrict__ X, long ldx, const unsigned short* __restrict__ Wp, int M, int K, int Co,
+    const float* __restrict__ X, long ldx, int xpw, const unsigned short* __restrict__ Wp, int M, int K, int Co,
     const float* __restrict__ scale, const float* __restrict__ shift, int act, float* __restrict__ Out, long ldo,
     int accumulate, float* __restrict__ stats_part) {
   constexpr int BM = 128, BN = 32 * NT;
@@ -273,18 +273,37 @@
   const long m0 = (long)tile_m * BM, mw = m0 + 32 * w;
   const int n0 = ct * BN;
   const long arows = min((long)BM, (long)M - m0);
-  const __amdgpu_buffer_rsrc_t ra = __builtin_amdgcn_make_buffer_rsrc(
-      (void*)(X + m0 * ldx), 0, (int)(((arows - 1) * ldx + K) * 4), 0x00020000);
+  const __amdgpu_buffer_rsrc_t ra =
+      XCUT ? __builtin_amdgcn_make_buffer_rsrc((void*)(reinterpret_cast<const unsigned short*>(X) + m0 * ldx), 0,
+                                               (int)(((arows - 1) * ldx + 2 * xpw + K) * 2), 0x00020000)
+           : __builtin_amdgcn_make_buffer_rsrc((void*)(X + m0 * ldx), 0, (int)(((arows - 1) * ldx + K) * 4), 0x00020000);
   const __amdgpu_buffer_rsrc_t rw = __builtin_amdgcn_make_buffer_rsrc(
       (void*)(Wp + (long)ct * ksteps * TILE), 0, ksteps * TILE * 2, 0x00020000);
-  const int oa = (int)(((32 * w + j) * ldx + 16 * g) * 4);
+  const int oa = (int)(((32 * w + j) * ldx + 16 * g) * (XCUT ? 2 : 4));
   float araw[16];
+  r3d_u32x4 acut[3][2];
   auto aload = [&](int k) {
-#pragma unroll
-    for (int q = 0; q < 4; ++q) {
-      const r3d_u32x4 v = __builtin_amdgcn_raw_buffer_load_b128(ra, oa + 16 * q, k * 4, 0);
-#pragma unroll
-      for (int i = 0; i < 4; ++i) araw[4 * q + i] = __uint_as_float(v[i]);
+    if constexpr (XCUT) {
+#pragma unroll
+      for (int p = 0; p < 3; ++p)
+#pragma unroll
+        for (int q = 0; q < 2; ++q) acut[p][q] = __builtin_amdgcn_raw_buffer_load_b128(ra, oa + 2 * p * xpw + 16 * q, k * 2, 0);
+    } else {
+#pragma unroll
+      for (int q = 0; q < 4; ++q) {
+        const r3d_u32x4 v = __builtin_amdgcn_raw_buffer_load_b128(ra, oa + 16 * q, k * 4, 0);
+#pragma unroll
+        for (int i = 0; i < 4; ++i) araw[4 * q + i] = __uint_as_float(v[i]);
+      }
+    }
+  };
+  auto afrag = [&](r3d_bx3& f0, r3d_bx3& f1) {
+    if constexpr (XCUT) {
+      f0.h = acut[0][0]; f0.m = acut[1][0]; f0.l = acut[2][0];
+      f1.h = acut[0][1]; f1.m = acut[1][1]; f1.l = acut[2][1];
+    } else {
+      f0 = r3d_bx3_split8(&araw[0]);
+      f1 = r3d_bx3_split8(&araw[8]);
     }
   };
   constexpr int H0 = (CPT + 1) / 2;
@@ -323,7 +342,8 @@
   __syncthreads();
   for (int ks = 0; ks < ksteps; ++ks) {
     const int cur = ks & 1, kn = min(ks + 1, ksteps - 1);
-    const r3d_bx3 fa0 = r3d_bx3_split8(&araw[0]), fa1 = r3d_bx3_split8(&araw[8]);
+    r3d_bx3 fa0, fa1;
+    afrag(fa0, fa1);
     aload(32 * kn);
     wload(kn, 0);
     __builtin_amdgcn_sched_barrier(0);
@@ -426,12 +446,13 @@
   }
 }
 
-template <int WM, int WN>
+template <int WM, int WN, bool ACUT, bool BCUT>
 __global__ __launch_bounds__(256) __attribute__((amdgpu_waves_per_eu(2))) void r3d_gemm_tn_bx3_kernel(
-    const float* __restrict__ A, long lda, const float* __restrict__ B, long ldb, long M, int Ca, int Cb, int tn_rows,
-    float* __restrict__ part ) {
+    const float* __restrict__ A, long lda, int apw, const float* __restrict__ B, long ldb, int bpw, long M, int Ca, int Cb,
+    int tn_rows, float* __restrict__ part ) {
   constexpr int BM = 64 * WM, BN = 64 * WN;
-  constexpr int XU = BM / 64, WU = BN / 64;
+  constexpr int XU = ACUT ? 0 : BM / 64, WU = BCUT ? 0 : BN / 64;
+  static_assert((!ACUT || BM == 128) && (!BCUT || BN == 128), "a cut operand is staged as 64 column pairs x 4 row groups");
   extern __shared__ __attribute__((aligned(16))) unsigned short gb_smem[];
   unsigned short* As = gb_smem;
   unsigned short* Bs = gb_smem + 3 * BM * GB_RS;
@@ -444,11 +465,38 @@
   const long m_beg = (long)chunk * tn_rows, m_end = min(M, m_beg + tn_rows);
   const int crows = (int)(m_end - m_beg);
   const __amdgpu_buffer_rsrc_t ra =
-      __builtin_amdgcn_make_buffer_rsrc((void*)(A + m_beg * lda), 0, (int)(((long)(crows - 1) * lda + Ca) * 4), 0x00020000);
+      ACUT ? __builtin_amdgcn_make_buffer_rsrc((void*)(reinterpret_cast<const unsigned short*>(A) + m_beg * lda), 0,
+                                               (int)(((long)(crows - 1) * lda + 2 * apw + Ca) * 2), 0x00020000)
+           : __builtin_amdgcn_make_buffer_rsrc((void*)(A + m_beg * lda), 0, (int)(((long)(crows - 1) * lda + Ca) * 4), 0x00020000);
   const __amdgpu_buffer_rsrc_t rb =
-      __builtin_amdgcn_make_buffer_rsrc((void*)(B + m_beg * ldb), 0, (int)(((long)(crows - 1) * ldb + Cb) * 4), 0x00020000);
-  const int lda4 = (int)lda * 4, ldb4 = (int)ldb * 4;
-  int ao[XU], bo[WU], amc[XU], bmc[WU];
+      BCUT ? __builtin_amdgcn_make_buffer_rsrc((void*)(reinterpret_cast<const unsigned short*>(B) + m_beg * ldb), 0,
+                                               (int)(((long)(crows - 1) * ldb + 2 * bpw + Cb) * 2), 0x00020000)
+           : __builtin_amdgcn_make_buffer_rsrc((void*)(B + m_beg * ldb), 0, (int)(((long)(crows - 1) * ldb + Cb) * 4), 0x00020000);
+  const int lda4 = (int)lda * (ACUT ? 2 : 4), ldb4 = (int)ldb * (BCUT ? 2 : 4);
+  const int cp = tid & 63, rg = tid >> 6;
+  const int aoc = 8 * rg * lda4 + 2 * min(i0 + 2 * cp, Ca - 2), boc = 8 * rg * ldb4 + 2 * min(j0 + 2 * cp, Cb - 2);
+  unsigned acr[3][8], bcr[3][8];
+  auto cut_load = [&](const __amdgpu_buffer_rsrc_t r, int off, int ld4, int pw, int mk, unsigned (&d)[3][8]) {
+#pragma unroll
+    for (int p = 0; p < 3; ++p)
+#pragma unroll
+      for (int t = 0; t < 8; ++t) d[p][t] = __builtin_amdgcn_raw_buffer_load_b32(r, off + (mk + t) * ld4 + 2 * p * pw, 0, 0);
+  };
+  auto cut_store = [&](unsigned short* __restrict__ planes, int rows, const unsigned (&d)[3][8]) {
+#pragma unroll
+    for (int p = 0; p < 3; ++p) {
+      r3d_u32x4 e, o;
+#pragma unroll
+      for (int i = 0; i < 4; ++i) {
+        e[i] = __builtin_amdgcn_perm(d[p][2 * i + 1], d[p][2 * i], 0x05040100u);
+        o[i] = __builtin_amdgcn_perm(d[p][2 * i + 1], d[p][2 * i], 0x07060302u);
+      }
+      unsigned short* q = planes + p * rows * GB_RS + 2 * cp * GB_RS + 8 * rg;
+      *reinterpret_cast<r3d_u32x4*>(q) = e;
+      *reinterpret_cast<r3d_u32x4*>(q + GB_RS) = o;
+    }
+  };
+  int ao[XU + 1], bo[WU + 1], amc[XU + 1], bmc[WU + 1];
 #pragma unroll
   for (int u = 0; u < XU; ++u) {
     const int c = tid + 256 * u;
@@ -461,8 +509,10 @@
     bmc[u] = c / BN;
     bo[u] = 8 * bmc[u] * ldb4 + 4 * min(j0 + c % BN, Cb - 1);
   }
-  float ar[XU][8], br[WU][8];
+  float ar[XU + 1][8], br[WU + 1][8];
   auto gload = [&](int mk) {
+    if constexpr (ACUT) cut_load(ra, aoc, lda4, apw, mk, acr);
+    if constexpr (BCUT) cut_load(rb, boc, ldb4, bpw, mk, bcr);
 #pragma unroll
     for (int u = 0; u < XU; ++u)
 #pragma unroll
@@ -485,6 +535,8 @@
     for (int u = 0; u < XU; ++u) { const int c = tid + 256 * u; gb_store_chunk(As, BM, c % BM, amc[u], ar[u]); }
 #pragma unroll
     for (int u = 0; u < WU; ++u) { const int c = tid + 256 * u; gb_store_chunk(Bs, BN, c % BN, bmc[u], br[u]); }
+    if constexpr (ACUT) cut_store(As, BM, acr);
+    if constexpr (BCUT) cut_store(Bs, BN, bcr);
     __syncthreads();
     gload(mk + 32);
     __builtin_amdgcn_sched_barrier(0);
@@ -552,26 +604,53 @@
   return (unsigned short*)p;
 }
 
+template <bool XCUT>
+static bool pointwise_bx3p_go(const float* X, long ldx, int xpw, const float* W, long M, int K, int Co, const float* scale,
+                              const float* shift, int act, float* Out, long ldo, int accumulate, float* stats_part,
+                              hipStream_t st) {
+  const int bnp = Co > 64 ? 128 : 64;
+  const int Cop = r3d_cdiv(Co, bnp) * bnp;
+  unsigned short* wp = wpack_scratch(st, (size_t)Cop * K * 6);
+  if (!wp) return false;
+  hipLaunchKernelGGL(r3d_w_pack_bx3_kernel, dim3(r3d_cdiv((long)Cop * (K / 8), 256)), dim3(256), 0, st, W, K, Co, bnp, wp);
+  const long tiles = (long)r3d_cdiv(M, 128) * (Cop / bnp);
+  if (bnp == 128)
+    hipLaunchKernelGGL((r3d_pointwise_gemm_bx3p_kernel<4, XCUT>), dim3((unsigned)tiles), dim3(256), 0, st, X, ldx, xpw, wp, (int)M,
+                       K, Co, scale, shift, act, Out, ldo, accumulate, stats_part);
+  else
+    hipLaunchKernelGGL((r3d_pointwise_gemm_bx3p_kernel<2, XCUT>), dim3((unsigned)tiles), dim3(256), 0, st, X, ldx, xpw, wp, (int)M,
+                       K, Co, scale, shift, act, Out, ldo, accumulate, stats_part);
+  return true;
+}
+
+bool r3d_pointwise_cut_ok(long M, int K, int Co, hipStream_t st) {
+  if (!(g_r3d_matrix_arith == 1 && (g_r3d_gemm_bx3 & 1) && (g_r3d_gemm_bx3 & 4) && K >= 32 && K % 32 == 0 && Co >= 32 &&
+        Co % 4 == 0 && M >= 256))
+    return false;
+  hipStreamCaptureStatus cs = hipStreamCaptureStatusNone;
+  if (hipStreamIsCapturing(st, &cs) != hipSuccess) return false;
+  return cs == hipStreamCaptureStatusNone || g_wpack_in_capture;
+}
+int r3d_pointwise_bx3_cut_launch(const void* Xc, long ldc, int pw, const float* W, long M, int K, int Co, const float* scale,
+                                 const float* shift, int act, float* Out, long ldo, int accumulate, float* stats_part,
+                                 hipStream_t st) {
+  R3D_REQUIRE(r3d_cut_valid(Xc, ldc, pw, K), "r3d_pointwise_conv_cut: bad cut operand (ld %ld, piece stride %d, K %d)", ldc, pw, K);
+  R3D_REQUIRE(r3d_pointwise_cut_ok(M, K, Co, st) && (ldo & 3) == 0 && ((uintptr_t)Out & 15) == 0 && ((uintptr_t)W & 15) == 0,
+              "r3d_pointwise_conv_cut: no cut-operand kernel for M=%ld K=%d Co=%d ldo=%ld here", M, K, Co, ldo);
+  R3D_REQUIRE((long)r3d_cdiv(M, 128) * r3d_cdiv(Co, 64) < 0x7fffffffL, "r3d_pointwise_conv_cut: too many tiles");
+  R3D_REQUIRE((pointwise_bx3p_go<true>((const float*)Xc, ldc, pw, W, M, K, Co, scale, shift, act, Out, ldo, accumulate,
+                                       stats_part, st)),
+              "r3d_pointwise_conv_cut: no W scratch on this stream");
+  return R3D_OK;
+}
+
 int r3d_pointwise_bx3_launch(const float* X, long ldx, const float* W, long M, int K, int Co, const float* scale,
                              const float* shift, int act, float* Out, long ldo, int accumulate, float* stats_part,
                              hipStream_t st) {
   if ((ldo & 3) != 0 || ((uintptr_t)Out & 15) != 0) return -1;
   if (!(GB_ABL & 128) && (g_r3d_gemm_bx3 & 4) && M >= 256) {
-    const int bnp = Co > 64 ? 128 : 64;
-    const int Cop = r3d_cdiv(Co, bnp) * bnp;
-    unsigned short* wp = wpack_scratch(st, (size_t)Cop * K * 6);
-    if (wp) {
-      hipLaunchKernelGGL(r3d_w_pack_bx3_kernel, dim3(r3d_cdiv((long)Cop * (K / 8), 256)), dim3(256), 0, st, W, K, Co, bnp, wp);
-      const long tiles = (long)r3d_cdiv(M, 128) * (Cop / bnp);
-      R3D_REQUIRE(tiles < 0x7fffffffL, "r3d_pointwise_conv: too many tiles");
-      if (bnp == 128)
-        hipLaunchKernelGGL((r3d_pointwise_gemm_bx3p_kernel<4>), dim3((unsigned)tiles), dim3(256), 0, st, X, ldx, wp, (int)M, K, Co,
-                           scale, shift, act, Out, ldo, accumulate, stats_part);
-      else
-        hipLaunchKernelGGL((r3d_pointwise_gemm_bx3p_kernel<2>), dim3((unsigned)tiles), dim3(256), 0, st, X, ldx, wp, (int)M, K, Co,
-                           scale, shift, act, Out, ldo, accumulate, stats_part);
-      return R3D_OK;
-    }
+    R3D_REQUIRE((long)r3d_cdiv(M, 128) * r3d_cdiv(Co, 64) < 0x7fffffffL, "r3d_pointwise_conv: too many tiles");
+    if (pointwise_bx3p_go<false>(X, ldx, 0, W, M, K, Co, scale, shift, act, Out, ldo, accumulate, stats_part, st)) return R3D_OK;
   }
   const int bn = (Co > 64 && !(GB_ABL & 64)) ? 128 : 64;
   const long tiles = (long)r3d_cdiv(M, 256) * r3d_cdiv(Co, bn);
@@ -591,21 +670,35 @@
   return Cb > 64 ? r3d_cdiv(Ca, 128) * r3d_cdiv(Cb, 128) : r3d_cdiv(Ca, 256) * r3d_cdiv(Cb, 64);
 }
 
-template <int WM, int WN>
-static int gemm_tn_bx3_go(size_t lds, int blocks, hipStream_t st, const float* A, long lda, const float* B, long ldb, long M,
-                          int Ca, int Cb, int rows, float* part) {
+template <int WM, int WN, bool ACUT = false, bool BCUT = false>
+static int gemm_tn_bx3_go(size_t lds, int blocks, hipStream_t st, const float* A, long lda, int apw, const float* B, long ldb,
+                          int bpw, long M, int Ca, int Cb, int rows, float* part) {
   static bool attr = false;
   if (!attr) {
-    R3D_REQUIRE(gb_lds_attr(r3d_gemm_tn_bx3_kernel<WM, WN>, lds) == 0, "r3d_gemm_tn: cannot reserve %zu B of LDS", lds);
+    R3D_REQUIRE((gb_lds_attr(r3d_gemm_tn_bx3_kernel<WM, WN, ACUT, BCUT>, lds) == 0), "r3d_gemm_tn: cannot reserve %zu B of LDS", lds);
     attr = true;
   }
-  hipLaunchKernelGGL((r3d_gemm_tn_bx3_kernel<WM, WN>), dim3(blocks), dim3(256), lds, st, A, lda, B, ldb, M, Ca, Cb, rows, part);
+  hipLaunchKernelGGL((r3d_gemm_tn_bx3_kernel<WM, WN, ACUT, BCUT>), dim3(blocks), dim3(256), lds, st, A, lda, apw, B, ldb, bpw, M,
+                     Ca, Cb, rows, part);
   return R3D_OK;
 }
 
 int r3d_gemm_tn_bx3_launch(const float* A, long lda, const float* B, long ldb, long M, int Ca, int Cb, int rows, int chunks,
                            float* part, hipStream_t st) {
   const int blocks = r3d_gemm_tn_bx3_tiles(Ca, Cb) * chunks;
-  if (Cb > 64) return gemm_tn_bx3_go<2, 2>(GB_LDS_22, blocks, st, A, lda, B, ldb, M, Ca, Cb, rows, part);
-  return gemm_tn_bx3_go<4, 1>(GB_LDS_41, blocks, st, A, lda, B, ldb, M, Ca, Cb, rows, part);
-}
+  if (Cb > 64) return gemm_tn_bx3_go<2, 2>(GB_LDS_22, blocks, st, A, lda, 0, B, ldb, 0, M, Ca, Cb, rows, part);
+  return gemm_tn_bx3_go<4, 1>(GB_LDS_41, blocks, st, A, lda, 0, B, ldb, 0, M, Ca, Cb, rows, part);
+}
+
+bool r3d_gemm_tn_cut_ok(int Ca, int Cb, int apw, int bpw) {
+  return r3d_gemm_tn_bx3_ok(Ca, Cb) && Cb > 64 && (!apw || Ca % 2 == 0) && (!bpw || Cb % 2 == 0);
+}
+int r3d_gemm_tn_bx3_cut_launch(const void* A, long lda, int apw, const void* B, long ldb, int bpw, long M, int Ca, int Cb,
+                               int rows, int chunks, float* part, hipStream_t st) {
+  const int blocks = r3d_gemm_tn_bx3_tiles(Ca, Cb) * chunks;
+  const float *a = (const float*)A, *b = (const float*)B;
+  if (apw && bpw) return gemm_tn_bx3_go<2, 2, true, true>(GB_LDS_22, blocks, st, a, lda, apw, b, ldb, bpw, M, Ca, Cb, rows, part);
+  if (apw) return gemm_tn_bx3_go<2, 2, true, false>(GB_LDS_22, blocks, st, a, lda, apw, b, ldb, 0, M, Ca, Cb, rows, part);
+  if (bpw) return gemm_tn_bx3_go<2, 2, false, true>(GB_LDS_22, blocks, st, a, lda, 0, b, ldb, bpw, M, Ca, Cb, rows, part);
+  return gemm_tn_bx3_go<2, 2>(GB_LDS_22, blocks, st, a, lda, 0, b, ldb, 0, M, Ca, Cb, rows, part);
+}
diff --git a/r3dfsseg_amd/csrc/train_ops.hip b/r3dfsseg_amd/csrc/train_ops.hip
--- a/r3dfsseg_amd/csrc/train_ops.hip
+++ b/r3dfsseg_amd/csrc/train_ops.hip
@@ -255,7 +255,8 @@
 #define EW_ROWS 32
 __global__ __launch_bounds__(256) void r3d_affine_act_kernel(const float* __restrict__ Z, long ldz, int M, int C, r3d_segmap sm,
                                                              const float* __restrict__ scale, const float* __restrict__ shift,
-                                                             long bn_stride, int act, float* __restrict__ Y, long ldy) {
+                                                             long bn_stride, int act, float* __restrict__ Y, long ldy,
+                                                             r3d_cut cy) {
   const int lane = threadIdx.x & 63, w = threadIdx.x >> 6;
   const int r0 = blockIdx.x * EW_ROWS + w;
   long zo[EW_ROWS / 4], yo[EW_ROWS / 4], bo[EW_ROWS / 4];
@@ -274,7 +275,10 @@
       float v = sc[u] * zv[u] + sh[u];
       if (act == 1) v = fmaxf(v, 0.f);
       else if (act == 2) v = v > 0.f ? v : 0.2f * v;
-      if (r0 + 4 * u < M) Y[yo[u] + c] = v;
+      if (r0 + 4 * u < M) {
+        if (Y) Y[yo[u] + c] = v;
+        if (cy.p) r3d_cut_store1(cy, r0 + 4 * u, c, v);
+      }
     }
   }
 }
@@ -283,7 +287,7 @@
     const float* __restrict__ Z, long ldz, const float* __restrict__ DY, long lddy, int M, int C, r3d_segmap sm,
     const float* __restrict__ scale, const float* __restrict__ shift, const float* __restrict__ mean,
     const float* __restrict__ invstd, long bn_stride, int act, const float* __restrict__ sums ,
-    double count_a, double count_b, float* __restrict__ DZ, long lddz) {
+    double count_a, double count_b, float* __restrict__ DZ, long lddz, r3d_cut cz) {
   const int lane = threadIdx.x & 63, w = threadIdx.x >> 6;
   const int r0 = blockIdx.x * EW_ROWS + w;
   constexpr int U = 4;
@@ -325,19 +329,23 @@
         if (act == 1) gg = uu > 0.f ? gg : 0.f;
         else if (act == 2) gg = uu > 0.f ? gg : 0.2f * gg;
         const float zh = (z[u] - mu[u]) * is[u];
-        if (r0 + 4 * (rr + u) < M) DZ[oo[u] + c] = sc[u] * (gg - m1[u] - zh * m2[u]);
+        if (r0 + 4 * (rr + u) < M) {
+          const float o = sc[u] * (gg - m1[u] - zh * m2[u]);
+          if (DZ) DZ[oo[u] + c] = o;
+          if (cz.p) r3d_cut_store1(cz, r0 + 4 * (rr + u), c, o);
+        }
       }
     }
   }
 }
 
 #define BA_ROWS 64
-template <int NK >
+template <int NK , bool CUT >
 __global__ __launch_bounds__(256) void r3d_bn_bwd_apply_v4_kernel(
     const float* __restrict__ Z, long ldz, const float* __restrict__ DY, long lddy, int M, int C, r3d_segmap sm,
     const float* __restrict__ scale, const float* __restrict__ shift, const float* __restrict__ mean,
     const float* __restrict__ invstd, long bn_stride, int act, const float* __restrict__ sums, double count_a, double count_b,
-    float* __restrict__ DZ, long lddz) {
+    float* __restrict__ DZ, long lddz, r3d_cut cz) {
   const int lane = threadIdx.x & 63, w = threadIdx.x >> 6;
   const int lpr = NK > 1 ? 64 : C >> 2;
   const int rpw = 64 / lpr;
@@ -401,7 +409,8 @@
           o.y = elem(z[u][kk].y, g[u][kk].y, sc[kk].y, sh[kk].y, mu[kk].y, is[kk].y, m1[kk].y, m2[kk].y);
           o.z = elem(z[u][kk].z, g[u][kk].z, sc[kk].z, sh[kk].z, mu[kk].z, is[kk].z, m1[kk].z, m2[kk].z);
           o.w = elem(z[u][kk].w, g[u][kk].w, sc[kk].w, sh[kk].w, mu[kk].w, is[kk].w, m1[kk].w, m2[kk].w);
-          *reinterpret_cast<float4*>(DZ + (long)row[u] * lddz + col0 + 256 * kk) = o;
+          if (!CUT || DZ) *reinterpret_cast<float4*>(DZ + (long)row[u] * lddz + col0 + 256 * kk) = o;
+          if (CUT) r3d_cut_store4(cz, row[u], col0 + 256 * kk, o.x, o.y, o.z, o.w);
         }
       }
     }
@@ -620,26 +629,42 @@
   return R3D_OK;
 }
 
-extern "C" int r3d_affine_act_seg(const float* Z, long ldz, long M, int C, long rows_a, long rows_b, const float* scale,
-                                  const float* shift, long bn_stride, int act, float* Y, long ldy, void* stream) {
-  R3D_REQUIRE(Z && Y && scale && shift && M > 0 && C > 0, "r3d_affine_act: bad arguments");
+static int affine_act_go(const float* Z, long ldz, long M, int C, long rows_a, long rows_b, const float* scale,
+                         const float* shift, long bn_stride, int act, float* Y, long ldy, r3d_cut cy, void* stream) {
+  R3D_REQUIRE(Z && (Y || cy.p) && scale && shift && M > 0 && C > 0, "r3d_affine_act: bad arguments");
+  R3D_REQUIRE(!cy.p || r3d_cut_valid(cy.p, cy.ld, cy.pw, C), "r3d_affine_act: bad cut output (ld %ld, piece stride %d, C %d)",
+              cy.ld, cy.pw, C);
   const r3d_segmap sm{rows_a, rows_b};
   R3D_REQUIRE(sm.covers(M), "r3d_affine_act: %ld rows are not whole segments of %ld + %ld rows", M, rows_a, rows_b);
   hipLaunchKernelGGL(r3d_affine_act_kernel, dim3(r3d_cdiv(M, EW_ROWS)), dim3(256), 0, (hipStream_t)stream, Z, ldz, (int)M, C, sm,
-                     scale, shift, bn_stride, act, Y, ldy);
+                     scale, shift, bn_stride, act, Y, ldy, cy);
   R3D_LAUNCH_CHECK("r3d_affine_act");
   return R3D_OK;
+}
+extern "C" int r3d_affine_act_seg(const float* Z, long ldz, long M, int C, long rows_a, long rows_b, const float* scale,
+                                  const float* shift, long bn_stride, int act, float* Y, long ldy, void* stream) {
+  R3D_REQUIRE(Y, "r3d_affine_act: bad arguments");
+  return affine_act_go(Z, ldz, M, C, rows_a, rows_b, scale, shift, bn_stride, act, Y, ldy, r3d_cut{nullptr, 0, 0}, stream);
+}
+extern "C" int r3d_affine_act_seg_cut(const float* Z, long ldz, long M, int C, long rows_a, long rows_b, const float* scale,
+                                      const float* shift, long bn_stride, int act, float* Y , long ldy, void* Yc,
+                                      long ldc, int pw, void* stream) {
+  R3D_REQUIRE(Yc, "r3d_affine_act_seg_cut: no cut output");
+  return affine_act_go(Z, ldz, M, C, rows_a, rows_b, scale, shift, bn_stride, act, Y, ldy, r3d_cut{(unsigned short*)Yc, ldc, pw},
+                       stream);
 }
 extern "C" int r3d_affine_act(const float* Z, long ldz, long M, int C, const float* scale, const float* shift, int act,
                               float* Y, long ldy, void* stream) {
   return r3d_affine_act_seg(Z, ldz, M, C, M, 0, scale, shift, 0, act, Y, ldy, stream);
 }
 
-extern "C" int r3d_bn_bwd_apply_seg(const float* Z, long ldz, const float* DY, long lddy, long M, int C, long rows_a,
-                                    long rows_b, const float* scale, const float* shift, const float* mean,
-                                    const float* invstd, long bn_stride, int act, const float* sums, double count_a,
-                                    double count_b, float* DZ, long lddz, void* stream) {
-  R3D_REQUIRE(Z && DY && DZ && scale && shift && mean && invstd && sums, "r3d_bn_bwd_apply: null pointer");
+static int bn_bwd_apply_go(const float* Z, long ldz, const float* DY, long lddy, long M, int C, long rows_a, long rows_b,
+                           const float* scale, const float* shift, const float* mean, const float* invstd, long bn_stride,
+                           int act, const float* sums, double count_a, double count_b, float* DZ, long lddz, r3d_cut cz,
+                           void* stream) {
+  R3D_REQUIRE(Z && DY && (DZ || cz.p) && scale && shift && mean && invstd && sums, "r3d_bn_bwd_apply: null pointer");
+  R3D_REQUIRE(!cz.p || r3d_cut_valid(cz.p, cz.ld, cz.pw, C), "r3d_bn_bwd_apply: bad cut output (ld %ld, piece stride %d, C %d)",
+              cz.ld, cz.pw, C);
   const r3d_segmap sm{rows_a, rows_b};
   R3D_REQUIRE(sm.covers(M) && count_a > 0, "r3d_bn_bwd_apply: %ld rows are not whole segments of %ld + %ld rows", M, rows_a,
               rows_b);
@@ -648,18 +673,41 @@
                     (((uintptr_t)Z | (uintptr_t)DY | (uintptr_t)DZ | (uintptr_t)scale | (uintptr_t)shift | (uintptr_t)mean |
                       (uintptr_t)invstd | (uintptr_t)sums) & 15) == 0;
   if (pow2 && al16) {
-#define BA_GO(NK)                                                                                                             \
-  hipLaunchKernelGGL(r3d_bn_bwd_apply_v4_kernel<NK>, dim3(r3d_cdiv(M, BA_ROWS)), dim3(256), 0, (hipStream_t)stream, Z, ldz, DY, \
-                     lddy, (int)M, C, sm, scale, shift, mean, invstd, bn_stride, act, sums, count_a, count_b, DZ, lddz)
-    if (C <= 256) BA_GO(1);
-    else if (C == 512) BA_GO(2);
-    else BA_GO(4);
+#define BA_GO(NK, CUT)                                                                                                        \
+  hipLaunchKernelGGL((r3d_bn_bwd_apply_v4_kernel<NK, CUT>), dim3(r3d_cdiv(M, BA_ROWS)), dim3(256), 0, (hipStream_t)stream, Z,  \
+                     ldz, DY, lddy, (int)M, C, sm, scale, shift, mean, invstd, bn_stride, act, sums, count_a, count_b, DZ,    \
+                     lddz, cz)
+    if (cz.p) {
+      if (C <= 256) BA_GO(1, true);
+      else if (C == 512) BA_GO(2, true);
+      else BA_GO(4, true);
+    } else {
+      if (C <= 256) BA_GO(1, false);
+      else if (C == 512) BA_GO(2, false);
+      else BA_GO(4, false);
+    }
 #undef BA_GO
   } else
   hipLaunchKernelGGL(r3d_bn_bwd_apply_kernel, dim3(r3d_cdiv(M, EW_ROWS)), dim3(256), 0, (hipStream_t)stream, Z, ldz, DY,
-                     lddy, (int)M, C, sm, scale, shift, mean, invstd, bn_stride, act, sums, count_a, count_b, DZ, lddz);
+                     lddy, (int)M, C, sm, scale, shift, mean, invstd, bn_stride, act, sums, count_a, count_b, DZ, lddz, cz);
   R3D_LAUNCH_CHECK("r3d_bn_bwd_apply");
   return R3D_OK;
+}
+extern "C" int r3d_bn_bwd_apply_seg(const float* Z, long ldz, const float* DY, long lddy, long M, int C, long rows_a,
+                                    long rows_b, const float* scale, const float* shift, const float* mean,
+                                    const float* invstd, long bn_stride, int act, const float* sums, double count_a,
+                                    double count_b, float* DZ, long lddz, void* stream) {
+  R3D_REQUIRE(DZ, "r3d_bn_bwd_apply: null pointer");
+  return bn_bwd_apply_go(Z, ldz, DY, lddy, M, C, rows_a, rows_b, scale, shift, mean, invstd, bn_stride, act, sums, count_a,
+                         count_b, DZ, lddz, r3d_cut{nullptr, 0, 0}, stream);
+}
+extern "C" int r3d_bn_bwd_apply_seg_cut(const float* Z, long ldz, const float* DY, long lddy, long M, int C, long rows_a,
+                                        long rows_b, const float* scale, const float* shift, const float* mean,
+                                        const float* invstd, long bn_stride, int act, const float* sums, double count_a,
+                                        double count_b, float* DZ , long lddz, void* DZc, long ldc, int pw, void* stream) {
+  R3D_REQUIRE(DZc, "r3d_bn_bwd_apply_seg_cut: no cut output");
+  return bn_bwd_apply_go(Z, ldz, DY, lddy, M, C, rows_a, rows_b, scale, shift, mean, invstd, bn_stride, act, sums, count_a,
+                         count_b, DZ, lddz, r3d_cut{(unsigned short*)DZc, ldc, pw}, stream);
 }
 extern "C" int r3d_bn_bwd_apply(const float* Z, long ldz, const float* DY, long lddy, long M, int C, const float* scale,
                                 const float* shift, const float* mean, const float* invstd, int act, const float* sums,
@@ -694,6 +742,31 @@
   return R3D_OK;
 }
 
+bool r3d_gemm_tn_cut_ok(int Ca, int Cb, int apw, int bpw);
+int r3d_gemm_tn_bx3_cut_launch(const void* A, long lda, int apw, const void* B, long ldb, int bpw, long M, int Ca, int Cb,
+                               int rows, int chunks, float* part, hipStream_t st);
+extern "C" int r3d_gemm_tn_cut_supported(int Ca, int Cb, int a_cut, int b_cut) {
+  return r3d_gemm_tn_cut_ok(Ca, Cb, a_cut ? 8 : 0, b_cut ? 8 : 0) ? 1 : 0;
+}
+extern "C" int r3d_gemm_tn_cut(const void* A, long lda, int apw, const void* B, long ldb, int bpw, long M, int Ca, int Cb,
+                               float alpha, float* out, int accumulate, float* ws, void* stream) {
+  R3D_REQUIRE(A && B && out && ws && M > 0 && Ca > 0 && Cb > 0 && apw >= 0 && bpw >= 0, "r3d_gemm_tn_cut: bad arguments");
+  R3D_REQUIRE(apw ? r3d_cut_valid(A, lda, apw, Ca) : (lda >= Ca && (lda & 3) == 0 && ((uintptr_t)A & 15) == 0),
+              "r3d_gemm_tn_cut: bad operand A (ld %ld, piece stride %d, %d columns)", lda, apw, Ca);
+  R3D_REQUIRE(bpw ? r3d_cut_valid(B, ldb, bpw, Cb) : (ldb >= Cb && (ldb & 3) == 0 && ((uintptr_t)B & 15) == 0),
+              "r3d_gemm_tn_cut: bad operand B (ld %ld, piece stride %d, %d columns)", ldb, bpw, Cb);
+  R3D_REQUIRE(r3d_gemm_tn_cut_ok(Ca, Cb, apw, bpw), "r3d_gemm_tn_cut: no cut-operand kernel for a (%d, %d) product here", Ca, Cb);
+  const int rows = tn_rows(M, Ca, Cb, true);
+  const int chunks = r3d_cdiv(M, rows);
+  hipStream_t st = (hipStream_t)stream;
+  const int rc = r3d_gemm_tn_bx3_cut_launch(A, lda, apw, B, ldb, bpw, M, Ca, Cb, rows, chunks, ws, st);
+  if (rc) return rc;
+  hipLaunchKernelGGL(r3d_chunk_reduce_kernel, dim3(r3d_cdiv((long)Ca * Cb, 256)), dim3(256), 0, st, ws, chunks,
+                     (long)Ca * Cb, alpha, out, accumulate);
+  R3D_LAUNCH_CHECK("r3d_gemm_tn_cut");
+  return R3D_OK;
+}
+
 extern "C" int r3d_add_cols(const float* src, long ld_src, float* dst, long ld_dst, long M, int C, void* stream) {
   R3D_REQUIRE(src && dst && M > 0 && C > 0, "r3d_add_cols: bad arguments");
   hipLaunchKernelGGL(r3d_add_cols_kernel, dim3(r3d_cdiv(M, 16)), dim3(256), 0, (hipStream_t)stream, src, ld_src, dst,
diff --git a/r3dfsseg_amd/train_ops.py b/r3dfsseg_amd/train_ops.py
--- a/r3dfsseg_amd/train_ops.py
+++ b/r3dfsseg_amd/train_ops.py
@@ -137,6 +137,68 @@
     return DZ
 
 
+class Cut:
+
+    def __init__(self, M, C, dev):
+        self.t = torch.empty(M, 3, C, device=dev, dtype=torch.int16)
+        self.shape = (M, C)
+        self.ld, self.pw = cut_index(0, 1, 0, C) - cut_index(0, 0, 0, C), cut_index(1, 0, 0, C) - cut_index(0, 0, 0, C)
+
+
+def cut_index(p, m, c, C):
+    return m * 3 * C + p * C + c
+
+
+CUT_DZ_COLS = (64, 128, 256, 512)
+
+
+def _cut_dz_route(X, C, M, want_dx, dx_acc):
+    lib = _lib.load()
+    Cin = X.shape[1]
+    if C not in CUT_DZ_COLS or X.stride(0) % 4 or X.data_ptr() % 16 or not lib.r3d_gemm_tn_cut_supported(C, Cin, 1, 0):
+        return False
+    if want_dx:
+        if dx_acc is not None and (dx_acc.stride(0) % 4 or dx_acc.data_ptr() % 16):
+            return False
+        return bool(lib.r3d_pointwise_conv_cut_ok(M, C, Cin, _st()))
+    return True
+
+
+def bn_bwd_apply_cut(Z, DY, bn, act, sums, counts, seg):
+    M, ldz = _rows(Z)
+    C = Z.shape[1]
+    dzc = Cut(M, C, Z.device)
+    sc, sh, mu, is_ = bn.ptrs()
+    _lib.check(_lib.load().r3d_bn_bwd_apply_seg_cut(_p(Z), ldz, _p(DY), DY.stride(0), M, C, seg.rows_a, seg.rows_b, sc, sh, mu,
+                                                    is_, bn.stride, act, _p(sums), counts[0], counts[1], None, 0, _p(dzc.t),
+                                                    dzc.ld, dzc.pw, _st()))
+    return dzc
+
+
+def gemm_tn_cut(Ac, B):
+    M, Ca = Ac.shape
+    M2, ldb = _rows(B)
+    assert M == M2
+    Cb = B.shape[1]
+    lib = _lib.load()
+    out = torch.empty(Ca, Cb, device=B.device, dtype=torch.float32)
+    ws = _f(lib.r3d_gemm_tn_ws_words(M, Ca, Cb), B.device)
+    with _timed("gemm_tn"):
+        _lib.check(lib.r3d_gemm_tn_cut(_p(Ac.t), Ac.ld, Ac.pw, _p(B), ldb, 0, M, Ca, Cb, 1.0, _p(out), 0, _p(ws), _st()))
+    return out
+
+
+def conv_cut(Xc, W, out=None, accumulate=False):
+    M, K = Xc.shape
+    Co = W.shape[0]
+    if out is None:
+        out = torch.empty(M, Co, device=W.device, dtype=torch.float32)
+    with _timed("pointwise_conv"):
+        _lib.check(_lib.load().r3d_pointwise_conv_cut(_p(Xc.t), Xc.ld, Xc.pw, _p(W), M, K, Co, None, None, 0, _p(out),
+                                                      out.stride(0), 1 if accumulate else 0, None, _st()))
+    return out
+
+
 def gemm_tn(A, B):
     M, lda = _rows(A)
     M2, ldb = _rows(B)
@@ -192,14 +254,22 @@
     C = W2d.shape[0]
     M = z.shape[0]
     sums = colstats(z, C, seg, mode=1, DY=dY, bn=bn, act=act)
-    dz = bn_bwd_apply(z, dY, bn, act, sums, seg.counts(), seg)
-    dW = gemm_tn(dz, X)
+    cut = _cut_dz_route(X, C, M, want_dx, dx_acc)
+    if cut:
+        dz = bn_bwd_apply_cut(z, dY, bn, act, sums, seg.counts(), seg)
+        dW = gemm_tn_cut(dz, X)
+    else:
+        dz = bn_bwd_apply(z, dY, bn, act, sums, seg.counts(), seg)
+        dW = gemm_tn(dz, X)
     tot = sums.sum(0) if seg.n_seg > 1 else sums[0]
     dbias = torch.zeros(C, device=z.device, dtype=torch.float32)
     dX = None
     if want_dx:
         Wt = W2d.t().contiguous()
-        if dx_acc is not None:
+        if cut:
+            dX = conv_cut(dz, Wt, out=dx_acc, accumulate=dx_acc is not None)
+            dX = None if dx_acc is not None else dX
+        elif dx_acc is not None:
             conv_acc(dz, Wt, dx_acc)
         else:
             dX = ops.pointwise_conv(dz, Wt)
```
